# LemonATsu/DANBO-pytorch

Measured on AMD Instinct MI355X. Metric: ray-samples/sec at 512x512x64 samples, higher is better.
Workload: dtype f32 (fp16x2-split MFMA products, fp32 accumulate); 1 GPU; H36M danbo_base network, 512x512 rays x (48 coarse + 16 importance) samples, 1 pose / 1 camera per rank, cylinder near/far, exact in-volume culling; rays=262144, samples_per_ray=64, parallelism=rays-dp1

## Files before the change

### danbo-pytorch_amd/core/hip_ops.py

```python
import contextlib
import ctypes
import gc

import torch

from . import _hip
from ._hip import call as _call, ptr as _p, stream as _stream
from .utils.skeleton_utils import SMPLSkeleton

J = _hip.C.DANBO_J
VOL = _hip.C.DANBO_VOL
FEAT = _hip.C.DANBO_FEAT
RAY_FLAT_VMAX = _hip.C.DANBO_RAY_FLAT_VMAX
H_STRIDE = _hip.C.DANBO_H_STRIDE
MLP_PACKED_FLOATS = _hip.C.DANBO_MLP_PACKED_FLOATS
ASSIGN16_PACKED_BYTES = _hip.C.DANBO_ASSIGN16_PACKED_BYTES
MLP16_PACKED_BYTES = _hip.C.DANBO_MLP16_PACKED_BYTES
ANERF_ENC_FLOATS = _hip.C.DANBO_ANERF_ENC_FLOATS
LINEAR16_ENC_K = _hip.C.DANBO_LINEAR16_ENC_K
TRUNK_PACKED_BYTES = _hip.C.DANBO_TRUNK_PACKED_BYTES
TRUNK_PE_WIDTH = _hip.C.DANBO_TRUNK_PE_WIDTH
VIEW_W = 128


def _on_device(*named, f32=False, dim=None, required=False):
    for t, name in named:
        ok = not required if t is None else t.is_cuda and (not f32 or t.dtype == torch.float32) and (dim is None or t.dim() == dim)
        if not ok:
            what = ("%d-D " % dim if dim else "") + ("float32 " if f32 else "")
            raise RuntimeError(f"{name}: expected a {what}CUDA/HIP tensor -- libdanbo_hip has no CPU fallback")


def _f32(t, name):
    if t is None:
        return None
    _on_device((t, name))
    if t.dtype != torch.float32:
        t = t.float()
    return t.contiguous()


def cam_index(cam_idx):
    return None if cam_idx is None else cam_idx.reshape(-1).to(torch.int64).contiguous()


def _ptr_array(tensors):
    arr = (ctypes.c_void_p * len(tensors))()
    for i, t in enumerate(tensors):
        arr[i] = t.data_ptr()
    return arr


def pose_volumes(bones, gw, L_graph=5):
    bones = _f32(bones, "bones")
    G = bones.shape[0]
    W = gw["w1"].shape[-1]
    scratch = torch.empty(3 * G * J * W, device=bones.device, dtype=torch.float32)
    vol = torch.empty(G, J, VOL, device=bones.device, dtype=torch.float32)
    _call("danbo_pose_volumes_fwd", _p(bones), G, L_graph, W,
          _p(gw["w0"]), _p(gw["adjw0"]), _p(gw["b0"]), _p(gw["w1"]), _p(gw["adjw1"]), _p(gw["b1"]),
          _p(gw["w2"]), _p(gw["b2"]), _p(gw["w3"]), _p(gw["b3"]), _p(scratch), _p(vol), _stream())
    return vol


def near_far_cylinder(rays_o, rays_d, cyl, near0=0.0, far0=1.0, chunk=4096, near_in=None, far_in=None):
    rays_o, rays_d, cyl = _f32(rays_o, "rays_o"), _f32(rays_d, "rays_d"), _f32(cyl, "cyl")
    near_in, far_in = _f32(near_in, "near_in"), _f32(far_in, "far_in")
    R, G = rays_o.shape[0], cyl.shape[0]
    nchunk = (R + chunk - 1) // chunk
    scratch = torch.empty(nchunk * 8, device=rays_o.device, dtype=torch.float32)
    near = torch.empty(R, device=rays_o.device, dtype=torch.float32)
    far = torch.empty_like(near)
    _call("danbo_near_far_cylinder", _p(rays_o), _p(rays_d), _p(cyl), R, G, float(near0), float(far0),
          _p(near_in), _p(far_in), int(chunk), _p(scratch), _p(near), _p(far), _stream())
    return near, far


def near_far_boxes(rays_o, rays_d, skts, align, axis_scale, near, far):
    R, G = rays_o.shape[0], skts.shape[0]
    _call("danbo_near_far_boxes", _p(_f32(rays_o, "rays_o")), _p(_f32(rays_d, "rays_d")), _p(_f32(skts, "skts")),
          _p(_f32(align, "align")), _p(_f32(axis_scale, "axis_scale")), R, G, _p(near), _p(far), _stream())
    return near, far


def coarse_samples(near, far, S, t_rand=None):
    R = near.shape[0]
    z = torch.empty(R, S, device=near.device, dtype=torch.float32)
    _call("danbo_coarse_samples", _p(near), _p(far), R, S, _p(_f32(t_rand, "t_rand")), _p(z), _stream())
    return z


@contextlib.contextmanager
def capture(graph):
    gc.collect()
    was_on = gc.isenabled()
    gc.disable()
    try:
        with torch.cuda.graph(graph):
            yield
    finally:
        if was_on:
            gc.enable()


def per_pose(x, G):
    return x if x.shape[0] == G else x[::max(x.shape[0] // G, 1)].contiguous()


def dw16(layers, M, device, count=None, slices=8):
    L = (_hip.DanboDwLayer * len(layers))(*layers)
    scratch = torch.empty(_hip.lib().danbo_dw16_scratch_floats(L, len(layers), slices), device=device)
    _call("danbo_dw16", L, len(layers), M, _p(count), slices, _p(scratch), _stream())


class Geometry:

    def __init__(self, rays_o, rays_d, skts, align, axis_scale, z=None, pts=None, ray_mask=None):
        self.rays_o = _f32(rays_o, "rays_o")
        self.rays_d = _f32(rays_d, "rays_d")
        self.skts = _f32(skts, "skts")
        self.align = _f32(align, "align")
        self.axis_scale = _f32(axis_scale, "axis_scale")
        self.z = _f32(z, "z")
        self.pts = _f32(pts, "pts")
        assert (self.z is None) != (self.pts is None)
        self.R = self.rays_o.shape[0]
        self.G = self.skts.shape[0]
        self.S = self.z.shape[1] if self.z is not None else self.pts.shape[1]
        self.M = self.R * self.S
        self.device = self.rays_o.device
        self.ray_mask = ray_mask if self.z is not None else None

    def head(self):
        return (_p(self.rays_o), _p(self.rays_d), _p(self.z), _p(self.pts), self.R, self.S, self.G,
                _p(self.skts), _p(self.align), _p(self.axis_scale))


def bone_cull(geo, compact=True, cnt=None):
    bits = torch.empty(geo.M, device=geo.device, dtype=torch.int32)
    lst = None
    if compact:
        lst = torch.empty(geo.M, device=geo.device, dtype=torch.int32)
        if cnt is None:
            cnt = torch.zeros(1, device=geo.device, dtype=torch.int32)
        assert cnt.dtype == torch.int32 and cnt.numel() == 1 and cnt.is_contiguous()
    else:
        cnt = None
    rm = tuple(geo.ray_mask) if geo.ray_mask is not None else (None, None, None)
    flat = rm[3] if len(rm) > 3 else None
    _call("danbo_bone_cull", *geo.head(), _p(rm[0]), _p(rm[1]), _p(rm[2]), _p(flat), _p(bits), _p(lst), _p(cnt), _stream())
    return bits, lst, cnt


def bone_cull_rays(geo, flat, bounds=None, cnt=None, rays_per_wg=0):
    assert geo.z is not None and geo.ray_mask is not None and geo.z.is_contiguous()
    bits = torch.empty(geo.M, device=geo.device, dtype=torch.int32)
    lst = torch.empty(geo.M, device=geo.device, dtype=torch.int32)
    if cnt is None:
        cnt = torch.zeros(1, device=geo.device, dtype=torch.int32)
    assert cnt.dtype == torch.int32 and cnt.numel() == 1 and cnt.is_contiguous()
    near, far = (None, None) if bounds is None else (_f32(b, "bounds").reshape(-1) for b in bounds)
    assert near is None or (near.shape[0] == geo.R and far.shape[0] == geo.R)
    rm = tuple(geo.ray_mask)
    _call("danbo_bone_cull_rays", *_ray_list(flat), _p(rm[0]), _p(rm[1]), _p(rm[2]), _p(geo.rays_o), _p(geo.rays_d), geo.R, geo.S,
          geo.G, _p(geo.skts), _p(geo.align), _p(geo.axis_scale), _p(near), _p(far), _p(geo.z), int(rays_per_wg), _p(bits), _p(lst),
          _p(cnt), _stream())
    return bits, lst, cnt


def ray_bone_mask(rays_o, rays_d, skts, align, axis_scale, t_lo, t_hi, want_flat=False):
    rays_o, rays_d, skts = _f32(rays_o, "rays_o"), _f32(rays_d, "rays_d"), _f32(skts, "skts")
    t_lo, t_hi = _f32(t_lo, "t_lo").reshape(-1), _f32(t_hi, "t_hi").reshape(-1)
    R, G = rays_o.shape[0], skts.shape[0]
    assert t_lo.shape[0] == R and t_hi.shape[0] == R
    mask = torch.empty(R, device=rays_o.device, dtype=torch.int32)
    flat = torch.empty(R, device=rays_o.device, dtype=torch.int32) if want_flat else None
    _call("danbo_ray_bone_mask", _p(rays_o), _p(rays_d), _p(t_lo), _p(t_hi), R, G, _p(skts), _p(_f32(align, "align")),
          _p(_f32(axis_scale, "axis_scale")), _p(mask), _p(flat), _stream())
    return (mask, t_lo, t_hi, flat) if want_flat else (mask, t_lo, t_hi)


def group_rows(bits, lst, cnt):
    _call("danbo_group_rows", _p(bits), _p(lst), _p(cnt), lst.shape[0], _stream())
    return lst


def bone_gather(geo, volumes, lst=None, cnt=None, n=None):
    n = geo.M if n is None else n
    out = torch.empty(n, J, FEAT, device=geo.device, dtype=torch.float32)
    _call("danbo_bone_gather_fwd", *geo.head(), _p(volumes), _p(lst), _p(cnt), n, _p(out), _stream())
    return out


def assign_blend(part_feat, bits, aw, lst=None, cnt=None, n=None, want_confd=False):
    n = part_feat.shape[0] if n is None else n
    h = torch.empty(n, H_STRIDE, device=part_feat.device, dtype=torch.float32)
    confd = torch.empty(n, J, device=part_feat.device, dtype=torch.float32) if want_confd else None
    _call("danbo_assign_blend_fwd", _p(part_feat), _p(bits), _p(lst), _p(cnt), n,
          _p(aw["w0"]), _p(aw["adjw"]), _p(aw["b0"]), _p(aw["w1"]), _p(aw["b1"]), _p(aw["w2"]), _p(aw["b2"]),
          _p(h), _p(confd), _stream())
    return h, confd


def gather_assign_blend(geo, volumes, bits, aw, lst=None, cnt=None, n=None, want_confd=False):
    n = geo.M if n is None else n
    h = torch.empty(n, H_STRIDE, device=geo.device, dtype=torch.float32)
    confd = torch.empty(n, J, device=geo.device, dtype=torch.float32) if want_confd else None
    _call("danbo_gather_assign_blend_fwd", *geo.head(), _p(volumes), _p(bits), _p(lst), _p(cnt), n,
          _p(aw["w0"]), _p(aw["adjw"]), _p(aw["b0"]), _p(aw["w1"]), _p(aw["b1"]), _p(aw["w2"]), _p(aw["b2"]),
          _p(h), _p(confd), _stream())
    return h, confd


_ADJ_CHECKED = set()


def check_smpl_adjacency(adj):
    key = (adj.data_ptr(), adj._version)
    if key in _ADJ_CHECKED:
        return
    want = torch.eye(J)
    for i, p_ in enumerate(SMPLSkeleton.joint_trees.tolist()):
        if i != p_:
            want[i, p_] = want[p_, i] = 1.0
    if not torch.equal((adj.detach().reshape(J, J) != 0).cpu(), want != 0):
        raise NotImplementedError("the assignment net's adjacency is not the SMPL tree: the fast K2 kernel (k_assign16) has that "
                                  "tree compiled in -- use mlp_mode='fp32' (k_assign_blend reads the adjacency it is given)")
    _ADJ_CHECKED.add(key)


def assign16_pack(aw):
    packed = torch.empty(ASSIGN16_PACKED_BYTES, device=aw["w0"].device, dtype=torch.uint8)
    _call("danbo_assign16_pack", _p(aw["w0"]), _p(aw["adjw"]), _p(aw["w1"]), _p(packed), _stream())
    return packed


_TICKETS = {}


def _ticket(device):
    if torch.cuda.is_current_stream_capturing():
        return torch.zeros(1, device=device, dtype=torch.int32)
    key = (device, torch.cuda.current_stream(device).cuda_stream)
    t = _TICKETS.get(key)
    if t is None:
        t = _TICKETS[key] = torch.zeros(1, device=device, dtype=torch.int32)
    return t


def gather_assign_blend16(geo, volumes, bits, aw, packed16, lst=None, cnt=None, n=None, want_confd=False):
    n = geo.M if n is None else n
    h = torch.empty(n, H_STRIDE, device=geo.device, dtype=torch.float32)
    confd = torch.empty(n, J, device=geo.device, dtype=torch.float32) if want_confd else None
    _call("danbo_gather_assign_blend16_fwd", *geo.head(), _p(volumes), _p(bits), _p(lst), _p(cnt), n, _p(packed16),
          _p(aw["b0"]), _p(aw["b1"]), _p(aw["w2"]), _p(aw["b2"]), _p(h), _p(confd), _p(_ticket(geo.device)), _stream())
    return h, confd


def mlp_pack(pts_w, feature_w, views_w):
    dev = feature_w.device
    Cv = views_w.shape[1] - 256
    packed = torch.empty(MLP_PACKED_FLOATS, device=dev, dtype=torch.float32)
    wrt = torch.empty(max(Cv, 1), VIEW_W, device=dev, dtype=torch.float32)
    pts_w = [_f32(w, "pts_w") for w in pts_w]
    _call("danbo_mlp_pack", _ptr_array(pts_w), _p(_f32(feature_w, "feature_w")), _p(_f32(views_w, "views_w")), Cv,
          _p(packed), _p(wrt), _stream())
    return packed, wrt


def view_consts(rays_d, skts, ray_mode, normalise, L_view, framecodes, mean_code, cam_idx, wrt, views_b,
                rgb_w, rgb_b, empty_consts=None, rgb_order=0, code_table=None, ray_list=None, ray_count=None):
    rays_d = _f32(rays_d, "rays_d")
    R, G = rays_d.shape[0], skts.shape[0]
    Cf = 0 if mean_code is None else mean_code.shape[0]
    n_codes = 0 if framecodes is None else framecodes.shape[0]
    cview = torch.empty(R, VIEW_W, device=rays_d.device, dtype=torch.float32)
    raw_empty = torch.empty(R, 4, device=rays_d.device, dtype=torch.float32) if empty_consts is not None else None
    cam_idx = cam_index(cam_idx)
    _call("danbo_view_consts", _p(rays_d), _p(_f32(skts, "skts")), R, G, int(ray_mode), int(normalise), int(L_view),
          _p(framecodes), n_codes, Cf, _p(mean_code), _p(cam_idx), _p(wrt), _p(views_b), _p(rgb_w), _p(rgb_b),
          _p(empty_consts), int(rgb_order), _p(code_table), _p(ray_list), _p(ray_count), _p(cview), _p(raw_empty), _stream())
    return cview, raw_empty


def view_code_table(framecodes, mean_code, L_view, wrt, views_b):
    n_codes, Cf = framecodes.shape
    table = torch.empty(n_codes + 1, VIEW_W, device=framecodes.device, dtype=torch.float32)
    _call("danbo_view_code_table", _p(framecodes), _p(mean_code), n_codes, Cf, int(L_view), _p(wrt), _p(views_b),
          _p(table), _stream())
    return table


def pe_mlp(h, S, packed, pts_b, alpha_w, alpha_b, feature_b, cview, rgb_w, rgb_b, raw_out,
           lst=None, cnt=None, n=None, aux=False):
    n = h.shape[0] if n is None else n
    aux_out = torch.empty(n, VIEW_W + 1, device=h.device, dtype=torch.float32) if aux else None
    _call("danbo_pe_mlp_fwd", _p(h), _p(lst), _p(cnt), n, S, _p(packed), _ptr_array(pts_b), _p(alpha_w), _p(alpha_b),
          _p(feature_b), _p(cview), _p(rgb_w), _p(rgb_b), _p(raw_out), _p(aux_out), _stream())
    return aux_out


def mlp16_pack(pts_w, feature_w, feature_b, views_w, views_b, form=16):
    dev = feature_w.device
    Cv = views_w.shape[1] - 256
    packed = torch.empty(MLP16_PACKED_BYTES, device=dev, dtype=torch.uint8)
    vb = torch.empty(VIEW_W, device=dev, dtype=torch.float32)
    pts_w = [_f32(w, "pts_w") for w in pts_w]
    _call({16: "danbo_mlp16_pack", 32: "danbo_mlp32_pack"}[form], _ptr_array(pts_w), _p(_f32(feature_w, "feature_w")), _p(_f32(feature_b, "feature_b")),
          _p(_f32(views_w, "views_w")), _p(_f32(views_b, "views_b")), Cv, _p(packed), _p(vb), _stream())
    return packed, vb


def pe_mlp16(h, S, packed16, pts_b, alpha_w, alpha_b, cview, rgb_w, rgb_b, raw_out,
             lst=None, cnt=None, n=None, aux=False, form=16):
    n = h.shape[0] if n is None else n
    aux_out = torch.empty(n, VIEW_W + 1, device=h.device, dtype=torch.float32) if aux else None
    _call({16: "danbo_pe_mlp16_fwd", 32: "danbo_pe_mlp32_fwd"}[form], _p(h), _p(lst), _p(cnt), n, S, _p(packed16), _ptr_array(pts_b), _p(alpha_w),
          _p(alpha_b), _p(cview), _p(rgb_w), _p(rgb_b), _p(raw_out), _p(aux_out), _stream())
    return aux_out


def fill_raw(raw_empty, S):
    R = raw_empty.shape[0]
    raw = torch.empty(R, S, 4, device=raw_empty.device, dtype=torch.float32)
    _call("danbo_fill_raw", _p(raw_empty), R, S, _p(raw), _stream())
    return raw


RELU = ("relu", 0.0)
_ACT_TYPES = {"relu": _hip.C.DANBO_DENSITY_RELU, "softplus": _hip.C.DANBO_DENSITY_SOFTPLUS}


def density_act(fn):
    if fn is None:
        return RELU
    if isinstance(fn, tuple) and len(fn) == 2 and fn[0] in _ACT_TYPES:
        return (fn[0], float(fn[1]) if fn[0] == "softplus" else 0.0)
    kind = getattr(fn, "density_kind", None)
    if kind == "softplus":
        return ("softplus", float(fn.softplus_shift))
    if kind == "relu" or fn is torch.nn.functional.relu or fn is torch.relu or getattr(fn, "__name__", "") == "relu":
        return RELU
    raise NotImplementedError("density activation: only relu and softplus (raycasters.get_density_fn) are implemented in the "
                              "composite kernels")


def _act_args(act):
    kind, shift = density_act(act)
    return _ACT_TYPES[kind], float(shift)


def _ray_outputs(R, S, Sf, dev, flat=None, want_weights=True, merged=False):
    n = S + Sf if merged else S
    if flat is not None:
        out = dict(flat["out" if merged else "out0"])
        assert out["alpha"].shape == (R, n)
        return out
    f = lambda *shape: torch.empty(*shape, device=dev, dtype=torch.float32)
    return dict(rgb_map=f(R, 3), disp_map=f(R), acc_map=f(R), weights=f(R, n) if want_weights else None, alpha=f(R, n))


def _ray_list(flat):
    return (None, None) if flat is None else (_p(flat["ray_list"]), _p(flat["ray_count"]))


def composite(raw, z, rays_d, B=1.0, noise=None, bits=None, raw_empty=None, flat=None, act=None):
    a_type, a_shift = _act_args(act)
    assert a_type == 0 or flat is None, "rays of constants (flat=) do not exist under softplus"
    raw, z, rays_d = _f32(raw, "raw"), _f32(z, "z"), _f32(rays_d, "rays_d")
    R, S = z.shape
    out = _ray_outputs(R, S, 0, raw.device, flat)
    assert out["weights"] is not None and out["weights"].shape == (R, S)
    _call("danbo_composite_rays_fwd_act", _p(raw), _p(_f32(raw_empty, "raw_empty")), _p(bits), _p(z), _p(rays_d), R, S, float(B),
          _p(_f32(noise, "noise")), _p(out["rgb_map"]), _p(out["disp_map"]), _p(out["acc_map"]), _p(out["weights"]), _p(out["alpha"]),
          *_ray_list(flat), a_type, a_shift, _stream())
    return out


def importance_samples(z, weights, Sf, u=None, flat=None, two_net=False):
    R, S = z.shape
    dev = z.device
    zs = torch.empty(R, S + Sf, device=dev, dtype=torch.float32)
    idx = torch.empty(R, S + Sf, device=dev, dtype=torch.int32)
    zf = flat["z_fine"] if flat is not None else torch.empty(R, Sf, device=dev, dtype=torch.float32)
    assert zf.shape == (R, Sf)
    _call("danbo_importance_samples_pdf", _p(_f32(z, "z")), _p(_f32(weights, "weights")), R, S, Sf, _p(_f32(u, "u")),
          int(bool(two_net)), _p(zf), _p(zs), _p(idx), *_ray_list(flat), _stream())
    return zs, zf, idx


def flat_rays(t_lo, ray_flat, S, Sf, want_weights=False, rows_later=False, cnt=None):
    t_lo = _f32(t_lo, "t_lo").reshape(-1)
    R, dev = t_lo.shape[0], t_lo.device
    assert ray_flat.dtype == torch.int32 and ray_flat.shape[0] == R
    out0 = _ray_outputs(R, S, Sf, dev, want_weights=want_weights)
    out = _ray_outputs(R, S, Sf, dev, merged=True)
    zf = torch.empty(R, Sf, device=dev, dtype=torch.float32)
    lst = torch.empty(R, device=dev, dtype=torch.int32)
    if cnt is None:
        cnt = torch.zeros(1, device=dev, dtype=torch.int32)
    assert cnt.dtype == torch.int32 and cnt.numel() == 1
    def launch(parts):
        _call("danbo_flat_rays", _p(t_lo), _p(ray_flat), R, int(S), int(Sf), _p(out0["rgb_map"]), _p(out0["disp_map"]),
              _p(out0["acc_map"]), _p(out0["weights"]), _p(out0["alpha"]), _p(zf), _p(out["rgb_map"]), _p(out["disp_map"]),
              _p(out["acc_map"]), _p(out["weights"]), _p(out["alpha"]), _p(lst), _p(cnt), parts, _stream())
    launch(1 if rows_later else 3)
    res = dict(out0=out0, out=out, z_fine=zf, ray_list=lst, ray_count=cnt)
    if rows_later:
        res["rows"] = lambda: launch(2)
    return res


def composite_importance(raw, z, rays_d, Sf, B=1.0, noise=None, u=None, bits=None, raw_empty=None, want_weights=True,
                         flat=None, two_net=False, act=None):
    a_type, a_shift = _act_args(act)
    assert a_type == 0 or flat is None, "rays of constants (flat=) do not exist under softplus"
    raw, z, rays_d = _f32(raw, "raw"), _f32(z, "z"), _f32(rays_d, "rays_d")
    R, S = z.shape
    dev = raw.device
    out0 = _ray_outputs(R, S, Sf, dev, flat, want_weights)
    zf = flat["z_fine"] if flat is not None else torch.empty(R, Sf, device=dev, dtype=torch.float32)
    assert zf.shape == (R, Sf)
    zs = torch.empty(R, S + Sf, device=dev, dtype=torch.float32)
    idx = torch.empty(R, S + Sf, device=dev, dtype=torch.int32)
    _call("danbo_composite_importance_pdf_fwd_act", _p(raw), _p(_f32(raw_empty, "raw_empty")), _p(bits), _p(z), _p(rays_d), R, S,
          int(Sf), float(B), _p(_f32(noise, "noise")), _p(_f32(u, "u")), int(bool(two_net)), _p(out0["rgb_map"]), _p(out0["disp_map"]),
          _p(out0["acc_map"]), _p(out0["weights"]), _p(out0["alpha"]), _p(zf), _p(zs), _p(idx), *_ray_list(flat), a_type, a_shift,
          _stream())
    return out0, zs, zf, idx


def composite_merged(raw_a, raw_b, idx, z_sorted, rays_d, B=1.0, noise=None, bits_a=None, bits_b=None, raw_empty=None,
                     want_raw=False, flat=None, act=None):
    a_type, a_shift = _act_args(act)
    assert a_type == 0 or flat is None, "rays of constants (flat=) do not exist under softplus"
    raw_a, raw_b, rays_d = _f32(raw_a, "raw_a"), _f32(raw_b, "raw_b"), _f32(rays_d, "rays_d")
    R, S = raw_a.shape[:2]
    Sf = raw_b.shape[1]
    assert flat is None or not want_raw
    out = _ray_outputs(R, S, Sf, raw_a.device, flat, merged=True)
    rs = torch.empty(R, S + Sf, 4, device=raw_a.device, dtype=torch.float32) if want_raw else None
    _call("danbo_composite_merged_fwd_act", _p(raw_a), _p(raw_b), _p(_f32(raw_empty, "raw_empty")), _p(bits_a), _p(bits_b),
          _p(idx), _p(_f32(z_sorted, "z_sorted")), _p(rays_d), R, S, Sf, float(B), _p(_f32(noise, "noise")), _p(out["rgb_map"]),
          _p(out["disp_map"]), _p(out["acc_map"]), _p(out["weights"]), _p(out["alpha"]), _p(rs), *_ray_list(flat), a_type, a_shift,
          _stream())
    if want_raw:
        out["raw_sorted"] = rs
    return out


def random_draws(state, n_uniform, n_normal, normal_std=1.0):
    assert state.dtype == torch.int64 and state.numel() == 3 and state.is_cuda
    dev = state.device
    u = torch.empty(n_uniform, device=dev, dtype=torch.float32) if n_uniform else None
    nz = torch.empty(n_normal, device=dev, dtype=torch.float32) if n_normal else None
    _call("danbo_random_draws", _p(state), int(n_uniform), _p(u), int(n_normal), float(normal_std), _p(nz), _stream())
    return u, nz


def row_span(t):
    assert t.element_size() in (4, 8)
    k = t.element_size() // 4
    if t.dim() == 0:
        t = t.reshape(1)
    inner = t[0] if t.shape[0] > 0 else t
    if not (t.shape[0] > 0 and inner.is_contiguous() and t.stride(0) >= 0):
        t = t.contiguous()
        inner = t[0]
    return t, t.shape[0], inner.numel() * k, t.stride(0) * k


def gather_rows(dst, items):
    assert dst.is_contiguous() and dst.element_size() == 4 and len(items) <= _hip.MAX_ROW_SPANS
    spans = (_hip.DanboRowSpan * len(items))()
    keep = []
    for i, (t, off) in enumerate(items):
        t, rows, words, stride = row_span(t)
        assert off + rows * words <= dst.numel()
        keep.append(t)
        spans[i] = _hip.DanboRowSpan(src=t.data_ptr(), dst_word=int(off), src_row_stride_words=int(stride), rows=int(rows),
                                     row_words=int(words))
    _call("danbo_gather_rows", spans, len(items), _p(dst), _stream())
    return dst


def merge_samples(a, b, idx):
    R, S = a.shape[:2]
    Sf = b.shape[1]
    C = a[0, 0].numel()
    out = torch.empty((R, S + Sf) + tuple(a.shape[2:]), device=a.device, dtype=torch.float32)
    _call("danbo_merge_samples", _p(_f32(a, "a")), _p(_f32(b, "b")), _p(idx), R, S, Sf, C, _p(out), _stream())
    return out


PART_MODES = {"confd": 0, "entropy": 1}
_PALETTES = {}


def part_palette(device):
    device = torch.device(device)
    t = _PALETTES.get(device)
    if t is None:
        from .networks.misc import joint_colours
        t = joint_colours(device).contiguous()
        if device.type != "cuda" or not torch.cuda.is_current_stream_capturing():
            _PALETTES[device] = t
    return t


def part_colors(confd, mode, rgb, lst=None, cnt=None, n=None, bits=None, valid_only=False):
    if mode not in PART_MODES:
        raise ValueError(f"part_colors: mode must be one of {sorted(PART_MODES)}, not {mode!r}")
    _on_device((confd, "confd"), (rgb, "rgb"), (lst, "list"), (cnt, "count"), (bits, "valid_bits"))
    if confd.dtype != torch.float32 or confd.dim() != 2 or confd.shape[1] != J or not confd.is_contiguous():
        raise ValueError("part_colors: confd must be a contiguous [rows, 24] float32 tensor")
    if rgb.dtype != torch.float32 or not rgb.is_contiguous() or rgb.shape[-1] != 3:
        raise ValueError("part_colors: rgb must be a contiguous [..., 3] float32 tensor")
    if valid_only and bits is None:
        raise ValueError("part_colors: valid_only needs the in-volume words")
    n = confd.shape[0] if n is None else int(n)
    if n > confd.shape[0] or (lst is None and n > rgb.numel() // 3) or (lst is not None and n > lst.numel()):
        raise ValueError("part_colors: more rows than confd / list / rgb hold")
    pal = part_palette(confd.device) if mode == "confd" else None
    _call("danbo_part_colors_fwd", _p(confd), _p(bits), _p(lst), _p(cnt), n, PART_MODES[mode], 1 if valid_only else 0, _p(pal),
          _p(rgb), _stream())
    return rgb


def composite_colors(rgb_a, weights, rgb_b=None, idx=None, bits_a=None, bits_b=None, flat=None, out=None):
    _on_device((rgb_a, "rgb_a"), (weights, "weights"), (rgb_b, "rgb_b"), (idx, "sorted_idx"), (out, "out"))
    rgb_a, rgb_b, weights = _f32(rgb_a, "rgb_a"), _f32(rgb_b, "rgb_b"), _f32(weights, "weights")
    R, S = rgb_a.shape[:2]
    Sf = 0 if rgb_b is None else rgb_b.shape[1]
    if tuple(weights.shape) != (R, S + Sf) or (idx is None) != (rgb_b is None) or (idx is not None and tuple(idx.shape) != (R, S + Sf)):
        raise ValueError("composite_colors: weights / sorted_idx must be [R, S + Sf]; sorted_idx and rgb_b come together")
    if out is None:
        out = torch.empty(R, 3, device=rgb_a.device, dtype=torch.float32)
    assert out.dtype == torch.float32 and tuple(out.shape) == (R, 3) and out.is_contiguous()
    _call("danbo_composite_colors_fwd", _p(rgb_a), _p(rgb_b), _p(bits_a), _p(bits_b), _p(idx), _p(weights), R, S, Sf,
          *_ray_list(flat), _p(out), _stream())
    return out


def _anerf_grid(rays_o, rays_d, skts, z, pts, nrows, width, out):
    skts = _f32(skts, "skts")
    if pts is not None:
        geo = (None, None, None, _f32(pts, "pts"))
    else:
        geo = (_f32(rays_o, "rays_o"), _f32(rays_d, "rays_d"), _f32(z, "z"), None)
    grid = geo[3] if pts is not None else geo[2]
    if out is None:
        out = (torch.empty(nrows, width, device=grid.device, dtype=torch.float32),
               torch.empty(nrows, J, device=grid.device, dtype=torch.float32))
    return geo, skts, grid.shape[0], grid.shape[1], out[0][:nrows], out[1][:nrows]


def anerf_encode(rays_o, rays_d, skts, align, cutoff, tau, L, row0, nrows, z=None, pts=None, out=None):
    geo, skts, R, S, x0, w = _anerf_grid(rays_o, rays_d, skts, z, pts, nrows, (1 + 2 * L) * J + 3 * J, out)
    _call("danbo_anerf_encode_fwd", *map(_p, geo), R, S, skts.shape[0], _p(skts), _p(_f32(align, "align")),
          _p(_f32(cutoff, "cutoff")), float(tau), int(L), int(row0), int(nrows), _p(x0), _p(w), _stream())
    return x0, w


def anerf_encode_compact(rays_o, rays_d, skts, align, cutoff, tau, row0, nrows, z=None, pts=None, out=None):
    geo, skts, R, S, table, w = _anerf_grid(rays_o, rays_d, skts, z, pts, nrows, ANERF_ENC_FLOATS, out)
    _call("danbo_anerf_encode_compact", *map(_p, geo), R, S, skts.shape[0], _p(skts), _p(_f32(align, "align")),
          _p(_f32(cutoff, "cutoff")), float(tau), int(row0), int(nrows), _p(table), _p(w), _stream())
    return table, w


def anerf_view_pe(rays_d, skts, L):
    rays_d, skts = _f32(rays_d, "rays_d"), _f32(skts, "skts")
    R, G = rays_d.shape[0], skts.shape[0]
    E = torch.empty(R, (1 + 2 * L) * 3 * J, device=rays_d.device, dtype=torch.float32)
    _call("danbo_anerf_view_pe_fwd", _p(rays_d), _p(skts), R, G, int(L), _p(E), _stream())
    return E


def transform_batch(vecs, skt, rot_only=False):
    _on_device((vecs, "transform_batch pts"), (skt, "transform_batch skt"), f32=True)
    N, S = vecs.shape[:2]
    G, J = skt.shape[0], skt.shape[-3]
    if vecs.shape[-1] != 3 or skt.shape[-2:] != (4, 4) or G < 1 or N % G:
        raise ValueError(f"transform_batch: pts {tuple(vecs.shape)}, skt {tuple(skt.shape)}")
    vecs, skt = vecs.contiguous(), skt.contiguous()
    out = torch.empty(N, S, J, 3, device=vecs.device, dtype=torch.float32)
    _call("danbo_transform_batch_pts", _p(vecs), _p(skt), N, S, J, N // G, 1 if rot_only else 0, _p(out), _stream())
    return out


def optcodes(codes, idx, mode):
    _on_device((codes, "optcodes codes"), f32=True)
    _on_device((idx, "optcodes idx"))
    idx = idx.reshape(idx.shape[0], -1).to(torch.float32).contiguous()
    codes = codes.contiguous()
    out = torch.empty(idx.shape[0], codes.shape[1], device=codes.device, dtype=torch.float32)
    _call("danbo_optcodes_fwd", _p(codes), codes.shape[0], codes.shape[1], _p(idx), idx.shape[1], idx.shape[0], int(mode), _p(out), _stream())
    return out


def small_matmul(a, b, bias=None, out=None):
    _on_device((a, "small_matmul a"), (b, "small_matmul b"), f32=True, dim=2)
    M, K = a.shape
    K2, N = b.shape
    if K != K2:
        raise ValueError(f"small_matmul: {tuple(a.shape)} @ {tuple(b.shape)}")
    if out is None:
        out = torch.empty(M, N, device=a.device, dtype=torch.float32)
    if bias is not None:
        bias = _f32(bias, "bias")
    _call("danbo_small_matmul", _p(a), a.stride(0), a.stride(1), _p(b), b.stride(0), b.stride(1), _p(bias), M, N, K, _p(out), out.stride(0),
          _stream())
    return out


def anerf_view_wj(views_w, col0, L):
    views_w = _f32(views_w, "views_w")
    VW, ld = views_w.shape
    wj = torch.empty(J, 3 * (1 + 2 * L), VW, device=views_w.device, dtype=torch.float32)
    _call("danbo_anerf_view_wj_pack", _p(views_w), ld, int(col0), VW, int(L), _p(wj), _stream())
    return wj


def anerf_view_consts(rays_d, skts, L, wj, out=None):
    rays_d, skts, wj = _f32(rays_d, "rays_d"), _f32(skts, "skts"), _f32(wj, "wj")
    R, G, VW = rays_d.shape[0], skts.shape[0], wj.shape[2]
    if wj.shape[0] != J or wj.shape[1] != 3 * (1 + 2 * L):
        raise ValueError(f"wj {tuple(wj.shape)} for L = {L}")
    C = out if out is not None else torch.empty(J, R, VW, device=rays_d.device, dtype=torch.float32)
    _call("danbo_anerf_view_consts_fwd", _p(rays_d), _p(skts), R, G, int(L), _p(wj), VW, _p(C), _stream())
    return C


def anerf_view_consts_bwd(rays_d, skts, L, dC, g_views_w, col0):
    rays_d, skts, dC = _f32(rays_d, "rays_d"), _f32(skts, "skts"), _f32(dC, "dC")
    R, G, VW = rays_d.shape[0], skts.shape[0], dC.shape[2]
    g_views_w = _f32(g_views_w, "g_views_w")
    n = _hip.lib().danbo_anerf_view_consts_bwd_scratch_floats(R, int(L), VW)
    scratch = torch.empty(n, device=rays_d.device, dtype=torch.float32)
    _call("danbo_anerf_view_consts_bwd", _p(rays_d), _p(skts), R, G, int(L), _p(dC), VW, _p(g_views_w), g_views_w.shape[1], int(col0),
          _p(scratch), _stream())
    return g_views_w


def _rows(t, name):
    _on_device((t, name), f32=True)
    if t.dim() == 1:
        t = t.unsqueeze(1)
    if t.stride(1) != 1:
        t = t.contiguous()
    return t, t.stride(0)


def anerf_color(featv, w, C, table, cam_idx, ray0, nrays, S, rgb_w, rgb_b, alpha, raw_out):
    VW = featv.shape[1]
    R_total = C.shape[1]
    cam_idx = cam_index(cam_idx)
    if cam_idx is not None and not cam_idx.is_cuda:
        raise RuntimeError("cam_idx: expected a CUDA/HIP tensor")
    featv, ldf = _rows(featv, "featv")
    alpha, lda = _rows(alpha, "alpha")
    _call("danbo_anerf_color_fwd", _p(featv), ldf, _p(_f32(w, "w")), _p(_f32(C, "C")), _p(_f32(table, "table")),
          _p(cam_idx), table.shape[0] - 1, R_total, int(ray0), int(nrays), int(S), VW, _p(_f32(rgb_w, "rgb_w")),
          _p(_f32(rgb_b, "rgb_b")), _p(alpha), lda, _p(raw_out), _stream())
    return raw_out


def linear16_color(h, packed, shape, bias, w, C, table, cam_idx, ray0, S, rgb_w, rgb_b, raw_out):
    N, K1, K2 = shape
    if not isinstance(h, FragBuffer) or h.C != K1 or K2:
        raise ValueError("linear16_color: h must be the FragBuffer the layer was packed for")
    VW, M = N - 1, h.M
    cam_idx = cam_index(cam_idx)
    _call("danbo_linear16_fwd_color", _p(h.data), K1, _p(packed), _p(_f32(bias, "bias")), VW, M, _p(_f32(w, "w")), _p(_f32(C, "C")),
          _p(_f32(table, "table")), _p(cam_idx), table.shape[0] - 1, C.shape[1], int(ray0), int(S), _p(_f32(rgb_w, "rgb_w")),
          _p(_f32(rgb_b, "rgb_b")), _p(raw_out), _stream())
    return raw_out


def linear16_pack(weight, K1=None, transposed=False, frag_in=(False, False)):
    w = _f32(weight, "weight")
    N, K = (w.shape[1], w.shape[0]) if transposed else w.shape
    K1 = K if K1 is None else int(K1)
    nbytes = _hip.lib().danbo_linear16_packed_bytes(N, K1, K - K1)
    if nbytes < 0:
        raise ValueError(f"linear16: unsupported layer shape N={N}, K={K}")
    packed = torch.empty(nbytes, dtype=torch.uint8, device=w.device)
    sn, sk = (1, w.stride(0)) if transposed else (w.stride(0), 1)
    fr = (1 if frag_in[0] else 0) | (2 if frag_in[1] else 0)
    _call("danbo_linear16_pack_frag", _p(w), sn, sk, N, K1, K - K1, fr, _p(packed), _stream())
    return packed, (N, K1, K - K1)


def linear16_pack_enc(weight, L, frag_second=True):
    w = _f32(weight, "weight")
    N, K = w.shape
    K2 = K - (24 * (1 + 2 * L) + 72)
    if K2 < 0 or K2 % 32:
        raise ValueError(f"linear16_pack_enc: {K} columns do not hold the {24 * (1 + 2 * L) + 72} density inputs (+ a multiple of 32)")
    nbytes = _hip.lib().danbo_linear16_packed_bytes(N, LINEAR16_ENC_K, K2)
    if nbytes < 0:
        raise ValueError(f"linear16: unsupported layer shape N={N}, K={K}")
    packed = torch.empty(nbytes, dtype=torch.uint8, device=w.device)
    _call("danbo_linear16_pack_enc", _p(w), w.stride(0), 1, N, int(L), K2, 2 if (K2 > 0 and frag_second) else 0, _p(packed), _stream())
    return packed, (N, LINEAR16_ENC_K, K2)


def linear16_enc(table, packed, shape, L, bias=None, relu=False, x2=None, out=None, count=None):
    N, K1, K2 = shape
    M = table.shape[0]
    if K1 != LINEAR16_ENC_K or table.shape[1] != ANERF_ENC_FLOATS or not table.is_contiguous() or not isinstance(out, FragBuffer):
        raise ValueError("linear16_enc: table must be [M, 144] contiguous, out a FragBuffer, the layer packed by linear16_pack_enc")
    if (K2 > 0) != (x2 is not None) or (x2 is not None and (not isinstance(x2, FragBuffer) or x2.M != M or x2.C != K2)):
        raise ValueError("linear16_enc: x2 must be the FragBuffer the layer was packed for")
    if out.M != M or out.C != N:
        raise ValueError("linear16_enc: out shape")
    _call("danbo_linear16_fwd_enc", _p(table), int(L), _p(x2.data) if x2 is not None else None, K2, _p(packed), _p(_f32(bias, "bias")), N,
          1 if relu else 0, _p(out.data), M, _p(count), _stream())
    return out


class FragBuffer:

    def __init__(self, rows, C, device, storage=None):
        if C % 32:
            raise ValueError("FragBuffer: the width must be a multiple of 32")
        self.M, self.C = int(rows), int(C)
        n = (self.M + 127) // 128 * 128 * self.C
        if storage is not None and storage.numel() < n:
            raise ValueError("FragBuffer: storage too small")
        self.data = torch.empty(n, device=device, dtype=torch.float32) if storage is None else storage

    def rows(self):
        G = (self.M + 127) // 128 * 8
        t = self.data[:G * 16 * self.C].view(G, self.C // 32, 2, 4, 16, 4).permute(0, 4, 1, 2, 3, 5)
        return t.reshape(G * 16, self.C)[:self.M]

    @staticmethod
    def from_rows(x):
        M, C = x.shape
        fb = FragBuffer(M, C, x.device)
        G = (M + 127) // 128 * 8
        pad = torch.zeros(G * 16, C, device=x.device, dtype=torch.float32)
        pad[:M] = x
        fb.data[:G * 16 * C] = pad.view(G, 16, C // 32, 2, 4, 4).permute(0, 2, 3, 4, 1, 5).reshape(-1)
        return fb


def _aligned_rows(t, name):
    t, ld = _rows(t, name)
    K = t.shape[1]
    if ld % 4 == 0 and ld >= (K + 3) // 4 * 4 and t.data_ptr() % 16 == 0:
        return t, ld
    buf = torch.zeros(t.shape[0], (K + 3) // 4 * 4, device=t.device, dtype=torch.float32)
    buf[:, :K] = t
    return buf[:, :K], buf.stride(0)


def _linear16_out(out, M, N, device):
    if out is None:
        out = torch.empty(M, (N + 3) // 4 * 4, device=device, dtype=torch.float32)[:, :N]
    y, ldy = _rows(out, "out")
    if y.data_ptr() != out.data_ptr() or tuple(y.shape) != (M, N) or ldy % 4 or y.data_ptr() % 16:
        raise ValueError("linear16: out must be a [M, N] float32 matrix, unit column stride, rows 16-byte aligned")
    return out, y, ldy


def linear16(x1, packed, shape, bias=None, relu=False, x2=None, out=None, count=None):
    N, K1, K2 = shape
    fr = (1 if isinstance(x1, FragBuffer) else 0) | (2 if isinstance(x2, FragBuffer) else 0) | (4 if isinstance(out, FragBuffer) else 0)
    if fr:
        return _linear16_frag(x1, packed, shape, bias, relu, x2, out, count, fr)
    if x1.shape[1] != K1 or (K2 > 0) != (x2 is not None):
        raise ValueError(f"linear16: inputs do not match the packed layer ({K1} + {K2} columns)")
    x1, ld1 = _aligned_rows(x1, "x1")
    M = x1.shape[0]
    ld2 = 0
    if x2 is not None:
        if tuple(x2.shape) != (M, K2):
            raise ValueError("linear16: x2 shape")
        x2, ld2 = _aligned_rows(x2, "x2")
    out, y, ldy = _linear16_out(out, M, N, x1.device)
    _call("danbo_linear16_fwd", _p(x1), ld1, K1, _p(x2), ld2, K2, _p(packed), _p(_f32(bias, "bias")), N, 1 if relu else 0,
          _p(y), ldy, M, _p(count), _stream())
    return out


def _linear16_frag(x1, packed, shape, bias, relu, x2, out, count, fr):
    N, K1, K2 = shape
    if fr not in (1, 4, 5, 6) or (fr == 1 and N > 256):
        raise ValueError("linear16: unsupported combination of fragment-order inputs / output")
    if (K2 > 0) != (x2 is not None):
        raise ValueError(f"linear16: inputs do not match the packed layer ({K1} + {K2} columns)")

    def operand(x, K, name):
        if isinstance(x, FragBuffer):
            if x.C != K:
                raise ValueError(f"linear16: {name} has {x.C} columns, the packed layer wants {K}")
            return x.data, 0, x.M
        if x.shape[1] != K:
            raise ValueError(f"linear16: {name} has {x.shape[1]} columns, the packed layer wants {K}")
        t, ld = _aligned_rows(x, name)
        return t, ld, t.shape[0]
    a1, ld1, M = operand(x1, K1, "x1")
    a2, ld2 = None, 0
    if x2 is not None:
        a2, ld2, M2 = operand(x2, K2, "x2")
        if M2 != M:
            raise ValueError("linear16: x2 rows")
    if isinstance(out, FragBuffer):
        if out.C != N or out.M != M:
            raise ValueError("linear16: fragment-order out does not match [rows, N]")
        y, ldy = out.data, 0
    else:
        out, y, ldy = _linear16_out(out, M, N, a1.device)
    _call("danbo_linear16_fwd_frag", _p(a1), ld1, K1, _p(a2), ld2, K2, _p(packed), _p(_f32(bias, "bias")), N, 1 if relu else 0,
          _p(y), ldy, M, _p(count), fr, _stream())
    return out


def marching_cubes(sigma, iso, floor=float("-inf"), scale=1.0, offset=(0.0, 0.0, 0.0), normals=False):
    _on_device((sigma, "sigma"))
    if sigma.dtype != torch.float32 or sigma.dim() != 3:
        raise ValueError("marching_cubes: sigma must be a [nx, ny, nz] float32 grid")
    if sigma.stride(2) != 1:
        raise ValueError("marching_cubes: the innermost stride of sigma must be 1")
    nx, ny, nz = sigma.shape
    grid = (_p(sigma), nx, ny, nz, sigma.stride(0), sigma.stride(1), float(floor), float(iso))
    n_bytes = _hip.lib().danbo_mesh_workspace_bytes(nx, ny, nz)
    if n_bytes == 0:
        raise _hip.HipError(f"marching_cubes: unsupported grid {nx} x {ny} x {nz} (each dimension 2 .. 1024, fewer than 2^31 points)")
    ws = torch.empty(n_bytes, device=sigma.device, dtype=torch.uint8)
    counts = torch.empty(2, device=sigma.device, dtype=torch.int32)
    _call("danbo_mesh_count", *grid, _p(ws), _p(counts), _stream())
    V, T = counts.tolist()
    if max(V, T) >= 2 ** 31 - 1:
        raise _hip.HipError("marching_cubes: the surface has 2^31 or more vertices or triangles")
    verts = torch.empty(V, 3, device=sigma.device, dtype=torch.float32)
    faces = torch.empty(T, 3, device=sigma.device, dtype=torch.int32)
    if V > 0:
        ox, oy, oz = (float(x) for x in offset)
        _call("danbo_mesh_extract", *grid, _p(ws), float(scale), ox, oy, oz, _p(verts), V, _p(faces), T, _stream())
    if not normals:
        return verts, faces
    nrm = torch.empty(V, 3, device=sigma.device, dtype=torch.float32)
    if V > 0:
        _call("danbo_mesh_normals", *grid, _p(ws), _p(nrm), V, _stream())
    return verts, faces, nrm


_rc = _hip.header("danbo_raster.h").C
RASTER_MODES = {"color": _rc.DANBO_RASTER_COLOR, "normal": _rc.DANBO_RASTER_NORMAL, "flat": _rc.DANBO_RASTER_FLAT}


def rasterize_mesh(verts, faces, attr=None, mode="normal", views=None, half_extent=0.6, size=(512, 512), background=(1.0, 1.0, 1.0),
                   want=("rgb",)):
    _on_device((verts, "verts"), (faces, "faces"), (views, "views"), required=True)
    if mode not in RASTER_MODES:
        raise ValueError(f"rasterize_mesh: mode must be one of {sorted(RASTER_MODES)}, not {mode!r}")
    if verts.dim() != 2 or verts.shape[1] != 3 or verts.dtype != torch.float32:
        raise ValueError("rasterize_mesh: verts must be a [V, 3] float32 tensor")
    if faces.dim() != 2 or faces.shape[1] != 3 or faces.dtype != torch.int32:
        raise ValueError("rasterize_mesh: faces must be a [T, 3] int32 tensor")
    if views.dtype != torch.float32 or views.numel() == 0 or views.numel() % 12 or tuple(views.shape[1:]) not in ((3, 4), (12,)):
        raise ValueError("rasterize_mesh: views must be a [n, 3, 4] or [n, 12] float32 tensor, n >= 1")
    want = tuple(want)
    if not want or any(w not in ("rgb", "depth", "tri_id") for w in want):
        raise ValueError("rasterize_mesh: want names at least one of 'rgb', 'depth', 'tri_id'")
    V, n = verts.shape[0], views.shape[0]
    H, W = (int(x) for x in size)
    if mode == "flat":
        attr = None
    else:
        if attr is None:
            raise ValueError(f"rasterize_mesh: mode {mode!r} needs attr [V, 3]")
        _on_device((attr, "attr"))
        if attr.dtype != torch.float32 or tuple(attr.shape) != (V, 3):
            raise ValueError(f"rasterize_mesh: attr must be a [{V}, 3] float32 tensor")
        attr = attr.contiguous() if V else attr.new_zeros(1, 3)
    n_bytes = _hip.lib().danbo_raster_workspace_bytes(V, H, W)
    if n_bytes == 0:
        raise _hip.HipError(f"rasterize_mesh: unsupported size {H} x {W} (height and width 1 .. 4096)")
    dev = verts.device
    verts, faces, views = verts.contiguous(), faces.contiguous(), views.contiguous()
    ws = torch.empty(n_bytes, device=dev, dtype=torch.uint8)
    bg = torch.tensor([float(x) for x in background], device=dev, dtype=torch.float32)
    if bg.numel() != 3:
        raise ValueError("rasterize_mesh: background is three numbers")
    out = {}
    if "rgb" in want:
        out["rgb"] = torch.empty(n, H, W, 3, device=dev, dtype=torch.float32)
    if "depth" in want:
        out["depth"] = torch.empty(n, H, W, device=dev, dtype=torch.float32)
    if "tri_id" in want:
        out["tri_id"] = torch.empty(n, H, W, device=dev, dtype=torch.int32)
    _call("danbo_raster_mesh", _p(verts) if V else None, V, _p(faces) if faces.shape[0] else None, faces.shape[0], _p(attr),
          RASTER_MODES[mode], _p(views), n, float(half_extent), H, W, _p(bg), _p(ws), _p(out.get("rgb")), _p(out.get("depth")),
          _p(out.get("tri_id")), _stream())
    return out


METRICS_WIN = 11
_METRIC_WINDOWS = {}
_METRIC_WORKSPACES = {}


def metrics_window(device):
    key = str(device)
    if key not in _METRIC_WINDOWS:
        from .utils.evaluation_helpers import _gauss
        _METRIC_WINDOWS[key] = _gauss(METRICS_WIN).to(device=device, dtype=torch.float32).contiguous()
    return _METRIC_WINDOWS[key]


def image_metrics(pred, gt, mask_a=None, mask_b=None, boxes=None, want_map=False):
    _on_device((pred, "pred"), (gt, "gt"), (mask_a, "mask_a"), (mask_b, "mask_b"), (boxes, "boxes"))
    if pred.dim() != 4 or pred.shape[-1] != 3 or pred.shape != gt.shape:
        raise ValueError("image_metrics: pred and gt must be [N, H, W, 3] tensors of one shape")
    pred, gt = _f32(pred, "pred"), _f32(gt, "gt")
    pred, gt = (t.clone() if t.data_ptr() % 16 else t for t in (pred, gt))
    N, H, W = pred.shape[:3]
    dev = pred.device

    def mask(m, name):
        if m is None:
            return None
        if m.numel() != N * H * W:
            raise ValueError(f"image_metrics: {name} must be [N, H, W] (or [N, H, W, 1])")
        return _f32(m, name).reshape(N, H, W)
    mask_a, mask_b = mask(mask_a, "mask_a"), mask(mask_b, "mask_b")
    if boxes is not None:
        if boxes.dtype != torch.int32 or tuple(boxes.shape) != (N, 4):
            raise ValueError("image_metrics: boxes must be an [N, 4] int32 tensor")
        boxes = boxes.contiguous()
    n_bytes = _hip.lib().danbo_image_metrics_workspace_bytes(N, H, W)
    if n_bytes == 0:
        raise _hip.HipError(f"image_metrics: unsupported size {N} x {H} x {W} (height and width 1 .. 4096)")
    key = (str(dev), n_bytes, torch.cuda.current_stream().cuda_stream)
    if key not in _METRIC_WORKSPACES:
        _METRIC_WORKSPACES[key] = torch.empty(n_bytes, device=dev, dtype=torch.uint8)
    sums = torch.empty(N, 8, device=dev, dtype=torch.float32)
    ssim = torch.zeros(N, H, W, 3, device=dev, dtype=torch.float32) if want_map else None
    _call("danbo_image_metrics", _p(pred), _p(gt), _p(mask_a), _p(mask_b), _p(boxes), N, H, W, _p(metrics_window(dev)), METRICS_WIN,
          _p(_METRIC_WORKSPACES[key]), _p(sums), _p(ssim), _stream())
    return dict(sums=sums, ssim_map=ssim)
```

### danbo-pytorch_amd/core/render_engine.py

```python
import ctypes

import torch

from . import _hip
from . import hip_ops as ops


class RenderEngine:
    fuse_resample = False

    def _key(self):
        return tuple((k, v.data_ptr(), v._version) for k, v in sorted(self.p.items()))

    def _sampling(self, N_samples, N_importance):
        cfg = self.cfg
        return (N_samples or cfg["N_samples"], N_importance or cfg["N_importance"], cfg["density_scale"],
                ops.density_act(cfg.get("density_act")))

    @staticmethod
    def frame_result(out, out0):
        return dict(rgb_map=out["rgb_map"], disp_map=out["disp_map"], acc_map=out["acc_map"], alpha=out["alpha"],
                    T_i=out["weights"], rgb0=out0["rgb_map"], disp0=out0["disp_map"], acc0=out0["acc_map"],
                    alpha0=out0["alpha"])

    def _network_pass(self, rays_o, rays_d, skts, bones, cam_idx, z, bounds, dense, lazy, tag):
        raise NotImplementedError

    @staticmethod
    def _part_mode(part_map):
        if part_map not in (None, "confd", "entropy"):
            raise ValueError(f"part_map must be None, 'confd' or 'entropy', not {part_map!r}")
        return part_map

    def _part_exact_culled(self, act):
        return act[0] == "relu" and bool(getattr(self, "empty_density_le0", False))

    @staticmethod
    def _part_colors(ex, n_samples, mode, valid_only, dense):
        confd = ex["confd_rows"]
        R = ex["valid_bits"].numel() // n_samples
        rgb = torch.empty(R, n_samples, 3, device=confd.device, dtype=torch.float32)
        ops.part_colors(confd, mode, rgb, ex["list"], ex["count"], bits=ex["valid_bits"], valid_only=valid_only)
        return rgb, (None if dense else ex["valid_bits"])

    def render_two_net(self, fine, rays_o, rays_d, skts, bones, cyls, cam_idx=None, N_samples=None, N_importance=None,
                       chunk=4096, near_far=None, dense=False, keep=False, part_map=None, part_valid_only=False):
        S, Sf, B, act = self._sampling(N_samples, N_importance)
        self.refresh()
        fine.refresh()
        part = self._part_mode(part_map)
        if part and not (self._part_exact_culled(act) and fine._part_exact_culled(act)):
            dense = True
        lazy = not dense and not keep
        pkw = dict(want_confd=True) if part else {}
        near, far = self.near_far(rays_o, rays_d, cyls, skts, 0.0, 1.0, chunk) if near_far is None else near_far
        z = ops.coarse_samples(near, far, S)
        raw, bits, empty, ex = self._network_pass(rays_o, rays_d, skts, bones, cam_idx, z, (near, far), dense, lazy, "coarse", **pkw)
        if self.fuse_resample and S <= 64 and Sf <= 64:
            out0, z_all, z_fine, order = ops.composite_importance(raw, z, rays_d, Sf, B, bits=bits, raw_empty=empty,
                                                                  want_weights=keep or bool(part), two_net=True, act=act)
        else:
            out0 = ops.composite(raw, z, rays_d, B, bits=bits, raw_empty=empty, act=act)
            z_all, z_fine, order = ops.importance_samples(z, out0["weights"], Sf, two_net=True)
        raw_f, bits_f, empty_f, ex_f = fine._network_pass(rays_o, rays_d, skts, bones, cam_idx, z_all, (near, far), dense, lazy, "fine",
                                                          **pkw)
        out = ops.composite(raw_f, z_all, rays_d, B, bits=bits_f, raw_empty=empty_f, act=act)
        pex, pex_f = ex.pop("part", None), ex_f.pop("part", None)
        if part:
            col, cb = self._part_colors(pex, S, part, part_valid_only, dense)
            ops.composite_colors(col, out0["weights"], bits_a=cb, out=out0["rgb_map"])
            col_f, cb_f = self._part_colors(pex_f, S + Sf, part, part_valid_only, dense)
            ops.composite_colors(col_f, out["weights"], bits_a=cb_f, out=out["rgb_map"])
        ret = self.frame_result(out, out0)
        if keep and part:
            ret.update(confd_coarse=pex["confd_rows"], confd_fine=pex_f["confd_rows"], list_coarse=pex["list"],
                       list_fine=pex_f["list"])
        if keep:
            ret.update(near=near, far=far, z_coarse=z, raw_coarse=raw, weights_coarse=out0["weights"], z_fine=z_fine,
                       z_sorted=z_all, sorted_idxs=order, raw_fine=raw_f, **ex, **ex_f)
        return ret


class DanboEngine(RenderEngine):
    fuse_resample = True

    def __init__(self, cfg, params, align, buffers=None, mlp_mode="f16split"):
        self.cfg = cfg
        self.p = params
        self.align = align.float().contiguous()
        self._packed_key = None
        self.packed = self.wrt = self.empty_consts = None
        self.mean_code = None
        self.profile = None
        self.skip_flat_rays = True
        self.mlp_form = 32
        assert mlp_mode in ("f16split", "fp32")
        self.mlp_mode = mlp_mode
        self.group_rows = False
        self.cull_listed_rays = True

    def refresh(self):
        key = self._key()
        if key == self._packed_key and getattr(self, "_built_mode", None) == (self.mlp_mode, self.mlp_form):
            return
        p = self.p
        dev = p["alpha_linear.weight"].device
        q = self._equalized(p) if self.mlp_mode == "f16split" else p
        self.pts_w = [q[f"pts_linears.{i}.weight"] for i in range(8)]
        self.pts_b = [q[f"pts_linears.{i}.bias"].contiguous() for i in range(8)]
        self.packed, self.wrt = ops.mlp_pack(self.pts_w, q["feature_linear.weight"], q["views_linears.0.weight"])
        self.packed16, self.views_b16 = ops.mlp16_pack(self.pts_w, q["feature_linear.weight"],
                                                       q["feature_linear.bias"], q["views_linears.0.weight"],
                                                       q["views_linears.0.bias"], form=self.mlp_form)
        self.alpha_w = q["alpha_linear.weight"].reshape(-1).contiguous()
        self.alpha_b = q["alpha_linear.bias"].contiguous()
        self.feature_b = q["feature_linear.bias"].contiguous()
        self.views_b = q["views_linears.0.bias"].contiguous()
        self.rgb_w = q["rgb_linear.weight"].contiguous()
        self.rgb_b = q["rgb_linear.bias"].contiguous()
        self.view_scale = q.get("_view_scale", torch.ones((), device=dev))
        g = "graph_net.layers."
        self.gw = dict(
            w0=p[g + "0.lin.weight"].contiguous(), adjw0=(p[g + "0.adj_w"] * p[g + "0.adj"])[0].contiguous(),
            b0=p[g + "0.bias"].contiguous(),
            w1=p[g + "1.lin.weight"].contiguous(), adjw1=(p[g + "1.adj_w"] * p[g + "1.adj"])[0].contiguous(),
            b1=p[g + "1.bias"].contiguous(),
            w2=p[g + "2.weight"].contiguous(), b2=p[g + "2.bias"].reshape(24, -1).contiguous(),
            w3=p[g + "3.weight"].contiguous(), b3=p[g + "3.bias"].reshape(24, -1).contiguous())
        a = "prob_linears.layers."
        self.aw = dict(
            w0=p[a + "0.lin.weight"].contiguous(), adjw=(p[a + "0.adj_w"] * p[a + "0.adj"])[0].contiguous(),
            b0=p[a + "0.bias"].contiguous(), w1=p[a + "1.weight"].contiguous(),
            b1=p[a + "1.bias"].reshape(24, -1).contiguous(), w2=p[a + "2.weight"].reshape(24, -1).contiguous(),
            b2=p[a + "2.bias"].reshape(-1).contiguous())
        if self.mlp_mode == "f16split":
            ops.check_smpl_adjacency(p[a + "0.adj"])
        self.assign16 = ops.assign16_pack(self.aw)
        self.axis_scale = p["graph_net.axis_scale"].contiguous()
        if self.cfg["use_framecode"]:
            self.framecodes = p["framecodes.codes.weight"].contiguous()
            self.mean_code = self.framecodes.mean(0).contiguous()
            vb = self.views_b16 if self.mlp_mode == "f16split" else self.views_b
            self.code_table = ops.view_code_table(self.framecodes, self.mean_code, self.cfg["multires_views"],
                                                  self.wrt, vb)
        else:
            self.framecodes = self.mean_code = self.code_table = None
        h0 = torch.zeros(1, ops.H_STRIDE, device=dev)
        scratch_raw = torch.empty(1, 4, device=dev)
        self.empty_consts = self._mlp(h0, 1, None, scratch_raw, aux=True).reshape(-1).contiguous()
        self.flat_rays_ok = self._flat_rays_ok()
        self._built_mode = (self.mlp_mode, self.mlp_form)
        self._packed_key = key

    def _flat_rays_ok(self):
        cfg = self.cfg
        ec = self.empty_consts
        if self.mlp_mode != "f16split":
            self.empty_density_le0 = bool((ec[128] / float(cfg["density_scale"]) <= 0).item())
            return False
        Cpe = 3 * (1 + 2 * cfg["multires_views"])
        vmax = 1.0 if cfg["view_type"] == "relray" else ops.RAY_FLAT_VMAX
        a_max = self.wrt[:Cpe].abs().sum(0) * vmax
        if self.code_table is not None:
            a_max = a_max + self.code_table.abs().max(0).values
        elif self.wrt.shape[0] > Cpe:
            self.empty_density_le0 = bool((ec[128] / float(cfg["density_scale"]) <= 0).item())
            return False
        else:
            a_max = a_max + self.views_b16.abs()
        hidden = ec[:128].abs() + a_max
        logit = ((self.rgb_w.abs() * hidden[None, :]).sum(-1) + self.rgb_b.abs()).max()
        le0 = ec[128] / float(cfg["density_scale"]) <= 0
        self.empty_density_le0, ok = torch.stack([le0, le0 & (logit < 1e30)]).tolist()
        return ok

    @staticmethod
    def _equalized(p):
        q = dict(p)
        one = torch.ones((), device=p["alpha_linear.weight"].device)
        tiny = torch.finfo(torch.float32).tiny

        def pow2(x):
            return torch.exp2(torch.clamp(torch.round(torch.log2(torch.clamp(x, min=tiny))), -100, 100))

        def factor(w_eff, b):
            gain = torch.sqrt((w_eff.double() ** 2).sum(1).mean()).float() * 0.7
            r = pow2(1.0 / torch.clamp(gain, min=tiny))
            cap = torch.exp2(torch.clamp(torch.floor(torch.log2(1024.0 / torch.clamp(b.abs().max(), min=tiny))), -100, 100))
            return torch.minimum(r, cap)

        r_prev = one
        n_in = p["pts_linears.0.weight"].shape[1]
        for l in range(8):
            w, b = p[f"pts_linears.{l}.weight"], p[f"pts_linears.{l}.bias"]
            if l == 0:
                w_eff = w
            elif w.shape[1] > p["pts_linears.1.weight"].shape[1]:
                w_eff = torch.cat([w[:, :n_in], w[:, n_in:] / r_prev], 1)
            else:
                w_eff = w / r_prev
            r = factor(w_eff, b)
            q[f"pts_linears.{l}.weight"], q[f"pts_linears.{l}.bias"] = (w_eff * r).contiguous(), (b * r).contiguous()
            r_prev = r
        q["alpha_linear.weight"] = (p["alpha_linear.weight"] / r_prev).contiguous()
        q["feature_linear.weight"] = (p["feature_linear.weight"] / r_prev).contiguous()
        wv, bv = p["views_linears.0.weight"], p["views_linears.0.bias"]
        rv = factor(wv, bv)
        q["views_linears.0.weight"], q["views_linears.0.bias"] = (wv * rv).contiguous(), (bv * rv).contiguous()
        q["rgb_linear.weight"] = (p["rgb_linear.weight"] / rv).contiguous()
        q["_view_scale"] = rv
        return q

    def _mlp(self, h, S, cview, raw, lst=None, cnt=None, n=None, aux=False):
        if self.mlp_mode == "f16split":
            return ops.pe_mlp16(h, S, self.packed16, self.pts_b, self.alpha_w, self.alpha_b, cview,
                                self.rgb_w, self.rgb_b, raw, lst, cnt, n, aux, form=self.mlp_form)
        return ops.pe_mlp(h, S, self.packed, self.pts_b, self.alpha_w, self.alpha_b, self.feature_b, cview,
                          self.rgb_w, self.rgb_b, raw, lst, cnt, n, aux)

    def volumes(self, bones):
        self.refresh()
        return ops.pose_volumes(bones, self.gw, self.cfg["multires_graph"])

    def view_constants(self, rays_d, skts, cam_idx, ray_list=None, ray_count=None):
        self.refresh()
        cfg = self.cfg
        ray_mode = {"world": 0, "root_local": 1}[cfg["ray_tr_type"]]
        normalise = 1 if cfg["view_type"] == "relray" else 0
        return ops.view_consts(rays_d, skts, ray_mode, normalise, cfg["multires_views"], self.framecodes,
                               self.mean_code, cam_idx, self.wrt,
                               self.views_b16 if self.mlp_mode == "f16split" else self.views_b, self.rgb_w,
                               self.rgb_b, self.empty_consts, {16: 1, 32: 2}[self.mlp_form] if self.mlp_mode == "f16split" else 0,
                               self.code_table, ray_list, ray_count)

    def forward_samples(self, rays_o, rays_d, skts, bones, cam_idx=None, z=None, pts=None, dense=False,
                        want_confd=False, volumes=None, view=None, fill=True, ray_mask=None, count=None, listed=None):
        self.refresh()
        geo = ops.Geometry(rays_o, rays_d, skts, self.align, self.axis_scale, z=z, pts=pts, ray_mask=ray_mask)
        vols = self.volumes(bones) if volumes is None else volumes
        cview, raw_empty = self.view_constants(geo.rays_d, geo.skts, cam_idx) if view is None else view
        S = geo.S
        if listed is not None:
            assert not dense and pts is None
            bits, lst, cnt = ops.bone_cull_rays(geo, listed[0], listed[1], cnt=count)
        else:
            bits, lst, cnt = ops.bone_cull(geo, compact=not dense, cnt=count)
        if lst is not None and self.mlp_mode == "f16split" and self.group_rows:
            ops.group_rows(bits, lst, cnt)
        if self.mlp_mode == "f16split":
            h, confd = ops.gather_assign_blend16(geo, vols, bits, self.aw, self.assign16, lst, cnt, geo.M, want_confd)
        else:
            h, confd = ops.gather_assign_blend(geo, vols, bits, self.aw, lst, cnt, geo.M, want_confd)
        raw = ops.fill_raw(raw_empty, S) if fill or dense else torch.empty(geo.R, S, 4, device=raw_empty.device)
        if self.profile is not None:
            e0, e1 = torch.cuda.Event(enable_timing=True), torch.cuda.Event(enable_timing=True)
            e0.record()
        self._mlp(h, S, cview, raw, lst, cnt, geo.M)
        if self.profile is not None:
            e1.record()
            self.profile.setdefault("k_pe_mlp", []).append((e0, e1, cnt if cnt is not None else geo.M))
        extras = dict(valid_bits=bits, list=lst, count=cnt, confd_rows=confd, h_rows=h, volumes=vols)
        return raw, extras

    def density(self, pts, skts, bones, netchunk=1024 * 64):
        self.refresh()
        M = pts.shape[0]
        out = torch.empty(M, 1, device=pts.device, dtype=torch.float32)
        vols = self.volumes(bones)
        for a in range(0, M, netchunk):
            p = pts[a:a + netchunk].contiguous()
            n = p.shape[0]
            dummy = torch.zeros(n, 3, device=pts.device)
            raw_empty = torch.zeros(n, 4, device=pts.device)
            raw_empty[:, 3] = self.empty_consts[128]
            cview = torch.zeros(n, ops.VIEW_W, device=pts.device)
            raw, _ = self.forward_samples(dummy, dummy, skts, bones, pts=p, volumes=vols, view=(cview, raw_empty))
            out[a:a + n] = raw[..., 3:4].reshape(n, 1)
        return out

    def colors(self, pts, dirs, skts, bones, cam_idx=None, netchunk=1024 * 64):
        self.refresh()
        pts, dirs = pts.reshape(-1, 1, 3), dirs.reshape(-1, 3)
        M = pts.shape[0]
        out = torch.empty(M, 3, device=pts.device, dtype=torch.float32)
        vols = self.volumes(bones)
        cam = ops.cam_index(cam_idx)
        for a in range(0, M, netchunk):
            p, d = pts[a:a + netchunk].contiguous(), dirs[a:a + netchunk].contiguous()
            raw, _ = self.forward_samples(torch.zeros_like(d), d, skts, bones, None if cam is None else cam[a:a + netchunk], pts=p,
                                          volumes=vols)
            out[a:a + p.shape[0]] = torch.sigmoid(raw[:, 0, :3])
        return out

    def render_frame_c(self, rays_o, rays_d, skts, bones, cyls, cam_idx=None, N_samples=None, N_importance=None, chunk=4096):
        assert self.mlp_mode == "f16split" and self.mlp_form == 32
        self.refresh()
        cfg = self.cfg
        S, Sf, _, act = self._sampling(N_samples, N_importance)
        f32 = lambda t: None if t is None else t.float().contiguous()
        rays_o, rays_d, skts, bones, cyls = (f32(t) for t in (rays_o, rays_d, skts, bones, cyls))
        cam = ops.cam_index(cam_idx) if cfg["use_framecode"] else None
        R, G, dev = rays_o.shape[0], skts.shape[0], rays_o.device
        gw, aw = self.gw, self.aw
        m = _hip.DanboModel()
        for k in ("w0", "adjw0", "b0", "w1", "adjw1", "b1", "w2", "b2", "w3", "b3"):
            setattr(m, "g_" + k, gw[k].data_ptr())
        m.L_graph, m.graph_width = cfg["multires_graph"], gw["w1"].shape[-1]
        m.align, m.axis_scale, m.assign16 = self.align.data_ptr(), self.axis_scale.data_ptr(), self.assign16.data_ptr()
        m.a_b0, m.a_b1, m.a_w2, m.a_b2 = (aw[k].data_ptr() for k in ("b0", "b1", "w2", "b2"))
        m.mlp16 = self.packed16.data_ptr()
        for i in range(8):
            m.pts_b[i] = self.pts_b[i].data_ptr()
        m.alpha_w, m.alpha_b, m.rgb_w, m.rgb_b = (t.data_ptr() for t in (self.alpha_w, self.alpha_b, self.rgb_w, self.rgb_b))
        m.views_w_ray_t, m.views_b_eff, m.empty_consts = self.wrt.data_ptr(), self.views_b16.data_ptr(), self.empty_consts.data_ptr()
        if self.framecodes is not None:
            m.framecodes, m.mean_code, m.code_table = (t.data_ptr() for t in (self.framecodes, self.mean_code, self.code_table))
            m.n_codes, m.code_size = self.framecodes.shape
        m.L_view = cfg["multires_views"]
        m.ray_mode, m.normalise = {"world": 0, "root_local": 1}[cfg["ray_tr_type"]], 1 if cfg["view_type"] == "relray" else 0
        m.density_scale, m.use_volume_near_far = float(cfg["density_scale"]), int(bool(cfg["use_volume_near_far"]))
        m.flat_rays_ok = int(self.flat_rays_ok and self.skip_flat_rays)
        r = _hip.DanboRays(rays_o=rays_o.data_ptr(), rays_d=rays_d.data_ptr(), skts=skts.data_ptr(), bones=bones.data_ptr(),
                           cyls=cyls.data_ptr(), cam_idx=None if cam is None else cam.data_ptr(), near_in=None, far_in=None,
                           R=R, G=G, chunk=int(chunk))
        shapes = dict(rgb_map=(R, 3), disp_map=(R,), acc_map=(R,), alpha=(R, S + Sf), weights=(R, S + Sf), rgb0=(R, 3),
                      disp0=(R,), acc0=(R,), alpha0=(R, S))
        out = {k: torch.empty(v, device=dev, dtype=torch.float32) for k, v in shapes.items()}
        o = _hip.DanboFrameOut(**{k: v.data_ptr() for k, v in out.items()})
        nbytes = _hip.lib().danbo_render_frame_workspace(R, G, S, Sf, int(chunk), m.graph_width)
        ws = torch.empty(nbytes, device=dev, dtype=torch.uint8)
        ops._call("danbo_render_frame_act", ctypes.byref(m), ctypes.byref(r), S, Sf, ctypes.byref(o), _hip.ptr(ws), nbytes,
                  *ops._act_args(act), ops._stream())
        out["T_i"] = out.pop("weights")
        return out

    def near_far(self, rays_o, rays_d, cyls, skts, near0=0.0, far0=1.0, chunk=4096):
        self.refresh()
        near, far = ops.near_far_cylinder(rays_o, rays_d, cyls, near0, far0, chunk)
        if self.cfg["use_volume_near_far"]:
            ops.near_far_boxes(rays_o, rays_d, skts, self.align, self.axis_scale, near, far)
        return near, far

    def render(self, rays_o, rays_d, skts, bones, cyls, cam_idx=None, N_samples=None, N_importance=None,
               chunk=4096, near_far=None, dense=False, keep=False, part_map=None, part_valid_only=False):
        S, Sf, B, act = self._sampling(N_samples, N_importance)
        self.refresh()
        part = self._part_mode(part_map)
        if part and not self._part_exact_culled(act):
            dense = True
        fused = S <= 64 and Sf <= 64
        lazy = not dense and not keep
        flat_mode = (lazy and (fused or (S <= 256 and Sf <= 64)) and self.skip_flat_rays and self.flat_rays_ok
                     and act[0] == "relu")
        near, far = self.near_far(rays_o, rays_d, cyls, skts, 0.0, 1.0, chunk) if near_far is None else near_far
        listed_cull = flat_mode and self.cull_listed_rays and not part and skts.shape[0] == 1
        z = torch.empty(rays_o.shape[0], S, device=rays_o.device, dtype=torch.float32) if listed_cull else ops.coarse_samples(near, far, S)
        ray_mask = None if dense else ops.ray_bone_mask(rays_o, rays_d, skts, self.align, self.axis_scale, near, far,
                                                        want_flat=flat_mode)
        counts = torch.zeros(3, device=rays_o.device, dtype=torch.int32)
        flat = None
        vols = self.volumes(bones)
        if flat_mode:
            flat = ops.flat_rays(ray_mask[1], ray_mask[3], S, Sf, want_weights=not fused or bool(part), cnt=counts[2:3])
            view = self.view_constants(rays_d, skts, cam_idx, flat["ray_list"], flat["ray_count"])
        else:
            view = self.view_constants(rays_d, skts, cam_idx)
        if ray_mask is not None:
            ray_mask = ray_mask[:3]
        raw, ex = self.forward_samples(rays_o, rays_d, skts, bones, cam_idx, z=z, dense=dense, volumes=vols, view=view,
                                       fill=not lazy, ray_mask=ray_mask, count=counts[0:1], want_confd=bool(part),
                                       listed=(flat, (near, far)) if listed_cull else None)
        if fused:
            out0, z_all, z_fine, order = ops.composite_importance(
                raw, z, rays_d, Sf, B, bits=ex["valid_bits"] if lazy else None, raw_empty=view[1] if lazy else None,
                want_weights=keep or bool(part), flat=flat, act=act)
        else:
            out0 = ops.composite(raw, z, rays_d, B, bits=ex["valid_bits"] if lazy else None, raw_empty=view[1] if lazy else None,
                                 flat=flat, act=act)
            z_all, z_fine, order = ops.importance_samples(z, out0["weights"], Sf, flat=flat)
        raw_f, ex_f = self.forward_samples(rays_o, rays_d, skts, bones, cam_idx, z=z_fine, dense=dense,
                                           volumes=vols, view=view, fill=not lazy,
                                           ray_mask=ray_mask, count=counts[1:2], want_confd=bool(part),
                                           listed=(flat, None) if listed_cull else None)
        out = ops.composite_merged(raw, raw_f, order, z_all, rays_d, B, bits_a=ex["valid_bits"] if lazy else None,
                                   bits_b=ex_f["valid_bits"] if lazy else None, raw_empty=view[1] if lazy else None,
                                   want_raw=keep, flat=flat, act=act)
        if part:
            col, cb = self._part_colors(ex, S, part, part_valid_only, dense)
            col_f, cb_f = self._part_colors(ex_f, Sf, part, part_valid_only, dense)
            ops.composite_colors(col, out0["weights"], bits_a=cb, flat=flat, out=out0["rgb_map"])
            ops.composite_colors(col, out["weights"], col_f, order, cb, cb_f, flat=flat, out=out["rgb_map"])
        ret = self.frame_result(out, out0)
        if keep:
            ret.update(near=near, far=far, z_coarse=z, raw_coarse=raw, weights_coarse=out0["weights"], z_fine=z_fine,
                       z_sorted=z_all, sorted_idxs=order, raw_fine=raw_f, raw_sorted=out.get("raw_sorted"),
                       count_coarse=ex["count"], count_fine=ex_f["count"], valid_bits=ex["valid_bits"])
            if part:
                ret.update(confd_coarse=ex["confd_rows"], confd_fine=ex_f["confd_rows"], list_coarse=ex["list"],
                           list_fine=ex_f["list"], valid_bits_fine=ex_f["valid_bits"])
        return ret

    def _network_pass(self, rays_o, rays_d, skts, bones, cam_idx, z, bounds, dense, lazy, tag, want_confd=False):
        mask = None if dense else ops.ray_bone_mask(rays_o, rays_d, skts, self.align, self.axis_scale, *bounds)
        view = self.view_constants(rays_d, skts, cam_idx)
        raw, ex = self.forward_samples(rays_o, rays_d, skts, bones, cam_idx, z=z, dense=dense, volumes=self.volumes(bones), view=view,
                                       fill=not lazy, ray_mask=mask, want_confd=want_confd)
        bits, empty = (ex["valid_bits"], view[1]) if lazy else (None, None)
        extras = {"count_" + tag: ex["count"], "valid_bits" + ("_fine" if tag == "fine" else ""): ex["valid_bits"]}
        if want_confd:
            extras["part"] = ex
        return raw, bits, empty, extras
```

### danbo-pytorch_amd/csrc/k_frame.hip

```cpp
#include "common.hpp"
#include "../../include/danbo_cull.h"

using namespace danbo;

namespace {
struct FrameBuffers {
    float *near, *far, *cyl_scratch, *z, *vol_scratch, *volumes, *cview, *raw_empty, *h, *raw_a, *raw_b, *z_fine, *z_sorted, *weights0;
    uint32_t *bits_a, *bits_b, *ray_mask, *ray_flat;
    int32_t *list, *count, *order, *ray_list;
};

FrameBuffers carve(Carver& c, int R, int G, int S, int Sf, int chunk, int Wg) {
    FrameBuffers b;
    const size_t M = (size_t)R * S, Mf = (size_t)R * Sf;
    b.near = c.take<float>(R);
    b.far = c.take<float>(R);
    b.cyl_scratch = c.take<float>(8 * (size_t)((R + chunk - 1) / chunk));
    b.z = c.take<float>(M);
    b.vol_scratch = c.take<float>(3 * (size_t)G * 24 * Wg);
    b.volumes = c.take<float>((size_t)G * 24 * 240);
    b.cview = c.take<float>((size_t)R * 128);
    b.raw_empty = c.take<float>((size_t)R * 4);
    b.ray_mask = c.take<uint32_t>(R);
    b.ray_flat = c.take<uint32_t>(R);
    b.ray_list = c.take<int32_t>(R);
    b.bits_a = c.take<uint32_t>(M);
    b.bits_b = c.take<uint32_t>(Mf);
    b.list = c.take<int32_t>(M);
    b.count = c.take<int32_t>(4);
    b.h = c.take<float>((M > Mf ? M : Mf) * 16);
    b.raw_a = c.take<float>(M * 4);
    b.raw_b = c.take<float>(Mf * 4);
    b.z_fine = c.take<float>(Mf);
    b.z_sorted = c.take<float>(M + Mf);
    b.order = c.take<int32_t>(M + Mf);
    if (Mf > M) b.list = c.take<int32_t>(Mf);
    b.weights0 = (S <= 64 && Sf <= 64) ? nullptr : c.take<float>(M);
    return b;
}
}

extern "C" size_t danbo_render_frame_workspace(int R, int G, int S, int Sf, int chunk, int graph_width) {
    if (R < 1 || G < 1 || S < 1 || Sf < 1 || chunk < 1 || graph_width < 1) return 0;
    Carver c;
    carve(c, R, G, S, Sf, chunk, graph_width);
    return c.used + 256;
}

static int render_frame_impl(const DanboModel* m, const DanboRays* r, int S, int Sf, const DanboFrameOut* o, void* workspace,
                             size_t workspace_bytes, int act, float shift, void* stream) {
    DANBO_CHECK_ARG(m && r && o && workspace && S >= 3 && S <= 256 && Sf >= 1 && Sf <= 64);
    DANBO_CHECK_ARG(r->R >= 1 && r->G >= 1 && r->R % r->G == 0 && r->chunk >= 1);
    DANBO_CHECK_ARG(r->rays_o && r->rays_d && r->skts && r->bones && r->cyls);
    DANBO_CHECK_ARG(o->rgb_map && o->disp_map && o->acc_map && o->alpha && o->weights && o->rgb0 && o->disp0 && o->acc0 && o->alpha0);
    const int R = r->R, G = r->G;
    const bool flat_rays = m->flat_rays_ok != 0 && act == DANBO_DENSITY_RELU;
    DANBO_CHECK_ARG(workspace_bytes >= danbo_render_frame_workspace(R, G, S, Sf, r->chunk, m->graph_width));
    Carver c(workspace);
    const FrameBuffers b = carve(c, R, G, S, Sf, r->chunk, m->graph_width);
    hipStream_t st = (hipStream_t)stream;

    DANBO_TRY(danbo_near_far_cylinder(r->rays_o, r->rays_d, r->cyls, R, G, 0.f, 1.f, r->near_in, r->far_in, r->chunk, b.cyl_scratch,
                                      b.near, b.far, stream));
    if (m->use_volume_near_far)
        DANBO_TRY(danbo_near_far_boxes(r->rays_o, r->rays_d, r->skts, m->align, m->axis_scale, R, G, b.near, b.far, stream));
    const bool listed_cull = flat_rays && G == 1;
    if (!listed_cull) DANBO_TRY(danbo_coarse_samples(b.near, b.far, R, S, nullptr, b.z, stream));
    DANBO_TRY(danbo_ray_bone_mask(r->rays_o, r->rays_d, b.near, b.far, R, G, r->skts, m->align, m->axis_scale, b.ray_mask,
                                  flat_rays ? b.ray_flat : nullptr, stream));
    DANBO_TRY(danbo_pose_volumes_fwd(r->bones, G, m->L_graph, m->graph_width, m->g_w0, m->g_adjw0, m->g_b0, m->g_w1, m->g_adjw1, m->g_b1,
                                     m->g_w2, m->g_b2, m->g_w3, m->g_b3, b.vol_scratch, b.volumes, stream));
    zero_words(b.count, 4, nullptr, 0, st);
    auto view_consts = [&](const int32_t* ray_list, const int32_t* ray_count) -> int {
        return danbo_view_consts(r->rays_d, r->skts, R, G, m->ray_mode, m->normalise, m->L_view, m->framecodes, m->n_codes, m->code_size,
                                 m->mean_code, r->cam_idx, m->views_w_ray_t, m->views_b_eff, m->rgb_w, m->rgb_b, m->empty_consts, 2,
                                 m->code_table, ray_list, ray_count, b.cview, b.raw_empty, stream);
    };
    const int32_t *ray_list = nullptr, *ray_count = nullptr;
    if (flat_rays) {
        DANBO_TRY(danbo_flat_rays(b.near, b.ray_flat, R, S, Sf, o->rgb0, o->disp0, o->acc0, b.weights0, o->alpha0, b.z_fine, o->rgb_map,
                                  o->disp_map, o->acc_map, o->weights, o->alpha, b.ray_list, b.count + 3, 3, stream));
        ray_list = b.ray_list;
        ray_count = b.count + 3;
    }
    DANBO_TRY(view_consts(ray_list, ray_count));
    auto cull = [&](float* zz, int s, uint32_t* bits, int32_t* count) -> int {
        if (listed_cull) {
            const bool coarse = zz == b.z;
            return danbo_bone_cull_rays(ray_list, ray_count, b.ray_mask, b.near, b.far, r->rays_o, r->rays_d, R, s, G, r->skts, m->align,
                                        m->axis_scale, coarse ? b.near : nullptr, coarse ? b.far : nullptr, zz, 0, bits, b.list, count,
                                        stream);
        }
        DANBO_TRY(danbo_bone_cull(r->rays_o, r->rays_d, zz, nullptr, R, s, G, r->skts, m->align, m->axis_scale, b.ray_mask, b.near, b.far,
                                  nullptr, bits, b.list, count, stream));
        return 0;
    };
    auto network = [&](const float* zz, int s, uint32_t* bits, int32_t* count, float* raw) -> int {
        DANBO_TRY(danbo_gather_assign_blend16_fwd(r->rays_o, r->rays_d, zz, nullptr, R, s, G, r->skts, m->align, m->axis_scale, b.volumes,
                                                  bits, b.list, count, R * s, m->assign16, m->a_b0, m->a_b1, m->a_w2, m->a_b2, b.h,
                                                  nullptr, reinterpret_cast<uint32_t*>(b.count + 2), stream));
        return danbo_pe_mlp32_fwd(b.h, b.list, count, R * s, s, m->mlp16, m->pts_b, m->alpha_w, m->alpha_b, b.cview, m->rgb_w,
                                  m->rgb_b, raw, nullptr, stream);
    };
    DANBO_TRY(cull(b.z, S, b.bits_a, b.count));
    DANBO_TRY(network(b.z, S, b.bits_a, b.count, b.raw_a));
    if (S <= 64) {
        DANBO_TRY(danbo_composite_importance_pdf_fwd_act(b.raw_a, b.raw_empty, b.bits_a, b.z, r->rays_d, R, S, Sf, m->density_scale, nullptr,
                                                         nullptr, 0, o->rgb0, o->disp0, o->acc0, nullptr, o->alpha0, b.z_fine, b.z_sorted,
                                                         b.order, ray_list, ray_count, act, shift, stream));
    } else {
        DANBO_TRY(danbo_composite_rays_fwd_act(b.raw_a, b.raw_empty, b.bits_a, b.z, r->rays_d, R, S, m->density_scale, nullptr, o->rgb0,
                                               o->disp0, o->acc0, b.weights0, o->alpha0, ray_list, ray_count, act, shift, stream));
        DANBO_TRY(danbo_importance_samples_rays(b.z, b.weights0, R, S, Sf, nullptr, b.z_fine, b.z_sorted, b.order, ray_list, ray_count,
                                                stream));
    }
    DANBO_TRY(cull(b.z_fine, Sf, b.bits_b, b.count + 1));
    DANBO_TRY(network(b.z_fine, Sf, b.bits_b, b.count + 1, b.raw_b));
    return danbo_composite_merged_fwd_act(b.raw_a, b.raw_b, b.raw_empty, b.bits_a, b.bits_b, b.order, b.z_sorted, r->rays_d, R, S, Sf,
                                          m->density_scale, nullptr, o->rgb_map, o->disp_map, o->acc_map, o->weights, o->alpha, nullptr,
                                          ray_list, ray_count, act, shift, stream);
}

extern "C" int danbo_render_frame(const DanboModel* m, const DanboRays* r, int S, int Sf, const DanboFrameOut* o, void* workspace,
                                  size_t workspace_bytes, void* stream) {
    return render_frame_impl(m, r, S, Sf, o, workspace, workspace_bytes, DANBO_DENSITY_RELU, 0.f, stream);
}

extern "C" int danbo_render_frame_act(const DanboModel* m, const DanboRays* r, int S, int Sf, const DanboFrameOut* o, void* workspace,
                                      size_t workspace_bytes, int act, float shift, void* stream) {
    DANBO_CHECK_DENSITY_ACT(act, shift);
    return render_frame_impl(m, r, S, Sf, o, workspace, workspace_bytes, act, act == DANBO_DENSITY_SOFTPLUS ? shift : 0.f, stream);
}
```

### danbo-pytorch_amd/csrc/k_sample.hip

```cpp
#include "common.hpp"
#include "cull_math.hpp"

namespace danbo {

__global__ __launch_bounds__(256) DANBO_NO_PK_F32 void k_cylinder_pass1(const float* __restrict__ rays_o,
                                                        const float* __restrict__ rays_d,
                                                        const float* __restrict__ cyl, int R, int G,
                                                        float near0, float far0,
                                                        const float* __restrict__ near_in,
                                                        const float* __restrict__ far_in, int chunk,
                                                        double* __restrict__ acc,
                                                        float* __restrict__ near_out,
                                                        float* __restrict__ far_out) {
    const int rays_per_pose = R / G;
    for (int r0 = blockIdx.x * blockDim.x; r0 < R; r0 += gridDim.x * blockDim.x) {
        const int r = r0 + threadIdx.x;
        const bool act = r < R;
        const int rc = act ? r : R - 1;
        const int g = min(rc / rays_per_pose, G - 1);
        float o[3] = {rays_o[3 * rc], rays_o[3 * rc + 1], rays_o[3 * rc + 2]};
        float d[3] = {rays_d[3 * rc], rays_d[3 * rc + 1], rays_d[3 * rc + 2]};
        float c[3] = {cyl[5 * g], cyl[5 * g + 1], cyl[5 * g + 2]};
        float nr, fr;
        const bool hit = cylinder_bounds(o, d, c, near_in ? near_in[rc] : near0, far_in ? far_in[rc] : far0, &nr, &fr) && act;
        if (act) {
            near_out[r] = nr;
            far_out[r] = fr;
        }
        const int ck = rc / chunk;
        const int ck0 = __shfl(ck, 0, 64);
        const bool uniform = __all(ck == ck0);
        double sn = hit ? (double)nr : 0.0, sf = hit ? (double)fr : 0.0, sc = hit ? 1.0 : 0.0;
        if (uniform) {
#pragma unroll
            for (int off = 32; off > 0; off >>= 1) {
                sn += __shfl_xor(sn, off, 64);
                sf += __shfl_xor(sf, off, 64);
                sc += __shfl_xor(sc, off, 64);
            }
            if ((threadIdx.x & 63) == 0 && sc > 0.0) {
                double* a = acc + 4 * ck;
                atomicAdd(a + 0, sn);
                atomicAdd(a + 1, sf);
                atomicAdd(a + 2, sc);
            }
        } else if (hit) {
            double* a = acc + 4 * ck;
            atomicAdd(a + 0, sn);
            atomicAdd(a + 1, sf);
            atomicAdd(a + 2, 1.0);
        }
    }
}

__global__ __launch_bounds__(256) void k_cylinder_pass2(int R, float near0, float far0,
                                                        const float* __restrict__ near_in,
                                                        const float* __restrict__ far_in, int chunk,
                                                        const double* __restrict__ acc,
                                                        float* __restrict__ near_out,
                                                        float* __restrict__ far_out) {
    for (int r = blockIdx.x * blockDim.x + threadIdx.x; r < R; r += gridDim.x * blockDim.x) {
        const float nr = near_out[r];
        if (nr != nr) {
            const double* a = acc + 4 * (r / chunk);
            const double cnt = a[2];
            near_out[r] = cnt > 0.0 ? (float)(a[0] / cnt) : (near_in ? near_in[r] : near0);
            far_out[r] = cnt > 0.0 ? (float)(a[1] / cnt) : (far_in ? far_in[r] : far0);
        }
    }
}

constexpr int CYL_BLOCK = 1024, CYL_FUSED_MAX = 16 * CYL_BLOCK;
__global__ __launch_bounds__(CYL_BLOCK) DANBO_NO_PK_F32 void k_cylinder_chunk(const float* __restrict__ rays_o, const float* __restrict__ rays_d,
                                                              const float* __restrict__ cyl, int R, int G, float near0, float far0,
                                                              const float* __restrict__ near_in, const float* __restrict__ far_in,
                                                              int chunk, float* __restrict__ near_out, float* __restrict__ far_out) {
    __shared__ double s_part[CYL_BLOCK / 64][3];
    __shared__ double s_sum[3];
    const int rays_per_pose = R / G;
    const int r_begin = blockIdx.x * chunk, r_end = min(r_begin + chunk, R);
    constexpr int PER = CYL_FUSED_MAX / CYL_BLOCK;
    float nr[PER], fr[PER];
    double sn = 0.0, sf = 0.0, sc = 0.0;
#pragma unroll
    for (int k = 0; k < PER; ++k) {
        const int r = r_begin + k * CYL_BLOCK + (int)threadIdx.x;
        nr[k] = 0.f; fr[k] = 0.f;
        if (r < r_end) {
            const int g = min(r / rays_per_pose, G - 1);
            const float o[3] = {rays_o[3 * r], rays_o[3 * r + 1], rays_o[3 * r + 2]};
            const float d[3] = {rays_d[3 * r], rays_d[3 * r + 1], rays_d[3 * r + 2]};
            const float c[3] = {cyl[5 * g], cyl[5 * g + 1], cyl[5 * g + 2]};
            if (cylinder_bounds(o, d, c, near_in ? near_in[r] : near0, far_in ? far_in[r] : far0, &nr[k], &fr[k])) {
                sn += (double)nr[k]; sf += (double)fr[k]; sc += 1.0;
            }
        }
    }
#pragma unroll
    for (int off = 32; off > 0; off >>= 1) {
        sn += __shfl_xor(sn, off, 64);
        sf += __shfl_xor(sf, off, 64);
        sc += __shfl_xor(sc, off, 64);
    }
    if ((threadIdx.x & 63) == 0) { s_part[threadIdx.x >> 6][0] = sn; s_part[threadIdx.x >> 6][1] = sf; s_part[threadIdx.x >> 6][2] = sc; }
    __syncthreads();
    if (threadIdx.x < 3) {
        double t = 0.0;
        for (int w = 0; w < CYL_BLOCK / 64; ++w) t += s_part[w][threadIdx.x];
        s_sum[threadIdx.x] = t;
    }
    __syncthreads();
    const double cnt = s_sum[2];
#pragma unroll
    for (int k = 0; k < PER; ++k) {
        const int r = r_begin + k * CYL_BLOCK + (int)threadIdx.x;
        if (r < r_end) {
            float n = nr[k], f = fr[k];
            if (n != n) {
                n = cnt > 0.0 ? (float)(s_sum[0] / cnt) : (near_in ? near_in[r] : near0);
                f = cnt > 0.0 ? (float)(s_sum[1] / cnt) : (far_in ? far_in[r] : far0);
            }
            near_out[r] = n;
            far_out[r] = f;
        }
    }
}

__global__ __launch_bounds__(256) void k_box_bounds(const float* __restrict__ rays_o,
                                                    const float* __restrict__ rays_d,
                                                    const float* __restrict__ skts,
                                                    const float* __restrict__ align,
                                                    const float* __restrict__ axis_scale, int R, int G,
                                                    float* __restrict__ near_io, float* __restrict__ far_io) {
    __shared__ float s_align[J * 16];
    __shared__ float s_scale[J * 3];
    for (int i = threadIdx.x; i < J * 16; i += blockDim.x) s_align[i] = align[i];
    for (int i = threadIdx.x; i < J * 3; i += blockDim.x) s_scale[i] = fabsf(axis_scale[i]);
    __syncthreads();
    const int rays_per_pose = R / G;
    const int j = threadIdx.x & 31;
    const long slots = ((long)gridDim.x * blockDim.x) >> 5;
    for (long r0 = ((long)blockIdx.x * blockDim.x + threadIdx.x) >> 5; r0 < ((R + 1) & ~1L); r0 += slots) {
        const int r = (int)(r0 < R ? r0 : R - 1);
        const int g = min(r / rays_per_pose, G - 1);
        float lo = 100000.0f, hi = -100000.0f;
        bool ok = false;
        if (j < J && r0 < R) {
            const float o[3] = {rays_o[3 * r], rays_o[3 * r + 1], rays_o[3 * r + 2]};
            const float d[3] = {rays_d[3 * r], rays_d[3 * r + 1], rays_d[3 * r + 2]};
            float sk[12];
            const float* src = skts + ((size_t)g * J + j) * 16;
#pragma unroll
            for (int i = 0; i < 12; ++i) sk[i] = src[i];
            float l_, h_;
            ok = bone_box_steps(sk, s_align + 16 * j, s_scale + 3 * j, o, d, &l_, &h_);
            if (ok) { lo = l_; hi = h_; }
        }
        int any = ok ? 1 : 0;
#pragma unroll
        for (int off = 16; off > 0; off >>= 1) {
            lo = fminf(lo, __shfl_xor(lo, off, 64));
            hi = fmaxf(hi, __shfl_xor(hi, off, 64));
            any |= __shfl_xor(any, off, 64);
        }
        if (j == 0 && r0 < R && any) {
            near_io[r] = lo;
            far_io[r] = hi;
        }
    }
}

__global__ __launch_bounds__(256) void k_coarse_samples4(const float* __restrict__ nr, const float* __restrict__ fr,
                                                         int R, int S, const float* __restrict__ t_rand,
                                                         float4* __restrict__ z) {
    const unsigned S4 = (unsigned)S / 4u;
    const unsigned M4 = (unsigned)R * S4;
    for (unsigned q = blockIdx.x * blockDim.x + threadIdx.x; q < M4; q += gridDim.x * blockDim.x) {
        const unsigned r = q / S4;
        const int s0 = 4 * (int)(q - r * S4);
        const float n_ = nr[r], f_ = fr[r];
        const long m = 4L * q;
        float4 v;
        v.x = coarse_sample(n_, f_, s0, S, t_rand, m);
        v.y = coarse_sample(n_, f_, s0 + 1, S, t_rand, m + 1);
        v.z = coarse_sample(n_, f_, s0 + 2, S, t_rand, m + 2);
        v.w = coarse_sample(n_, f_, s0 + 3, S, t_rand, m + 3);
        z[q] = v;
    }
}

__global__ __launch_bounds__(256) void k_coarse_samples(const float* __restrict__ nr, const float* __restrict__ fr,
                                                        int R, int S, const float* __restrict__ t_rand,
                                                        float* __restrict__ z) {
    const long M = (long)R * S;
    const bool small = M <= 0x7fffffffL;
    for (long m = (long)blockIdx.x * blockDim.x + threadIdx.x; m < M; m += (long)gridDim.x * blockDim.x) {
        int r, s;
        if (small) {
            r = (int)((unsigned)m / (unsigned)S);
            s = (int)((unsigned)m - (unsigned)r * (unsigned)S);
        } else {
            r = (int)(m / S);
            s = (int)(m % S);
        }
        z[m] = coarse_sample(nr[r], fr[r], s, S, t_rand, m);
    }
}


__device__ __forceinline__ bool segment_misses_bone(const float* sk, const float* al, const float* sc ,
                                                    const float* o, const float* d, float zl, float zh) {
    float ol[3], dl[3], t[3];
    bone_local(sk, al, o, ol);
    for (int k = 0; k < 3; ++k) t[k] = sk[4 * k] * d[0] + sk[4 * k + 1] * d[1] + sk[4 * k + 2] * d[2];
    for (int k = 0; k < 3; ++k) dl[k] = al[4 * k] * t[0] + al[4 * k + 1] * t[1] + al[4 * k + 2] * t[2];
    const float pad = 1e-4f * fmaxf(fabsf(zl), fabsf(zh)) + 1e-5f;
    float tmin = zl - pad, tmax = zh + pad;
    bool miss = false;
    for (int k = 0; k < 3; ++k) {
        const float s = sc[k] * 1.001f + 1e-4f;
        if (fabsf(dl[k]) < 1e-12f) {
            miss = miss || fabsf(ol[k]) > s;
        } else {
            const float inv = 1.0f / dl[k];
            const float t1 = (-s - ol[k]) * inv, t2 = (s - ol[k]) * inv;
            tmin = fmaxf(tmin, fminf(t1, t2));
            tmax = fminf(tmax, fmaxf(t1, t2));
        }
    }
    return miss || tmin > tmax;
}

constexpr float RAY_FLAT_VMAX = DANBO_RAY_FLAT_VMAX;

template <bool POSES_IN_LDS>
__global__ __launch_bounds__(256) void k_ray_bone_mask(const float* __restrict__ rays_o, const float* __restrict__ rays_d,
                                                       const float* __restrict__ t_lo, const float* __restrict__ t_hi,
                                                       const float* __restrict__ skts, const float* __restrict__ align,
                                                       const float* __restrict__ axis_scale, int R, int G,
                                                       uint32_t* __restrict__ ray_mask, uint32_t* __restrict__ ray_flat) {
    extern __shared__ __attribute__((aligned(16))) float smem[];
    float* s_align = smem;
    float* s_scale = smem + J * 16;
    float* s_skt = smem + J * 16 + J * 4;
    const int rays_per_pose = R / G;
    const int r_a = blockIdx.x * 256, r_b = min(r_a + 255, R - 1);
    const int g0 = min(r_a / rays_per_pose, G - 1), g1 = min(r_b / rays_per_pose, G - 1);
    const int r = min(r_a + (int)threadIdx.x, R - 1);
    const float o[3] = {rays_o[3 * r], rays_o[3 * r + 1], rays_o[3 * r + 2]};
    const float d[3] = {rays_d[3 * r], rays_d[3 * r + 1], rays_d[3 * r + 2]};
    const float zl = t_lo[r], zh = t_hi[r];
    stage_bone_tables<256>(align, axis_scale, s_align, s_scale, 0.f);
    if (POSES_IN_LDS)
        for (int i = threadIdx.x; i < (g1 - g0 + 1) * J * 16; i += 256) s_skt[i] = skts[(size_t)g0 * J * 16 + i];
    __syncthreads();
    const int g = min(r / rays_per_pose, G - 1);
    uint32_t bits = 0u;
    if (POSES_IN_LDS) {
        const float* sk = s_skt + (size_t)(g - g0) * J * 16;
#pragma unroll 2
        for (int j = 0; j < J; ++j)
            bits |= segment_misses_bone(sk + 16 * j, s_align + 16 * j, s_scale + 4 * j, o, d, zl, zh) ? 0u : 1u << j;
    } else {
        for (int j = 0; j < J; ++j) {
            float sk[12];
            const float* src = skts + ((size_t)g * J + j) * 16;
#pragma unroll
            for (int i = 0; i < 12; ++i) sk[i] = src[i];
            bits |= segment_misses_bone(sk, s_align + 16 * j, s_scale + 4 * j, o, d, zl, zh) ? 0u : 1u << j;
        }
    }
    if (r_a + (int)threadIdx.x < R) {
        ray_mask[r] = bits;
        if (ray_flat != nullptr) {
            const float dn = norm3_torch(d[0], d[1], d[2]);
            const float span = mul_rn(add_rn(sub_rn(zh, zl), mul_rn(1e-3f, fmaxf(fabsf(zl), fabsf(zh)))), dn);
            const float tail = mul_rn(1e10f, dn);
            const float* m0 = POSES_IN_LDS ? s_skt + (size_t)(g - g0) * J * 16 : skts + (size_t)g * J * 16;
            float msum = 0.f;
            for (int a = 0; a < 3; ++a)
                for (int k = 0; k < 3; ++k) msum = add_rn(msum, fabsf(m0[4 * a + k]));
            const float vin = mul_rn(dn, fmaxf(1.0f, msum));
            const bool fin = zl <= zh && sub_rn(span, span) == 0.f && sub_rn(tail, tail) == 0.f && vin <= RAY_FLAT_VMAX;
            ray_flat[r] = (bits == 0u && fin) ? 1u : 0u;
        }
    }
}

constexpr int CULL_BLOCK = 256;
constexpr int CULL_SPT = 4;
constexpr int CULL_MAX_RAYS = 130;

__global__ __launch_bounds__(CULL_BLOCK) void k_bone_cull(const float* __restrict__ rays_o,
                                                          const float* __restrict__ rays_d,
                                                          const float* __restrict__ z,
                                                          const float* __restrict__ pts, int R, int S, int G,
                                                          const float* __restrict__ skts,
                                                          const float* __restrict__ align,
                                                          const float* __restrict__ axis_scale, int np_lds,
                                                          const uint32_t* __restrict__ ray_mask,
                                                          const float* __restrict__ t_lo, const float* __restrict__ t_hi,
                                                          uint32_t* __restrict__ ray_flat,
                                                          uint32_t* __restrict__ valid_bits,
                                                          int32_t* __restrict__ list, int32_t* __restrict__ count) {
    extern __shared__ __attribute__((aligned(16))) float smem[];
    float* s_align = smem;
    float* s_scale = smem + J * 16;
    float* s_skt = smem + J * 16 + J * 4;
    __shared__ float s_zlo[CULL_MAX_RAYS], s_zhi[CULL_MAX_RAYS];
    __shared__ uint32_t s_mask[CULL_MAX_RAYS];

    const long M = (long)R * S;
    const long spp = (long)(R / G) * S;
    const long base = (long)blockIdx.x * (CULL_BLOCK * CULL_SPT);
    const long last = min(base + CULL_BLOCK * CULL_SPT, M) - 1;
    const int g0 = pose_of_sample(base, spp, G), g1 = pose_of_sample(last, spp, G);

    const int lane = threadIdx.x & 63;
    const int r_first = (int)(base / S), r_last = (int)(last / S);
    const int off0 = (int)(base - (long)r_first * S);
    const int rays_per_pose = R / G;
    const float inv_S = 1.0f / (float)S;
    auto pose_of = [&](int r) { return G == 1 ? 0 : min(r / rays_per_pose, G - 1); };
    const int nrays = r_last - r_first + 1;
    const bool prefilter = pts == nullptr && ray_mask == nullptr && nrays <= CULL_MAX_RAYS;
    float zreg[CULL_SPT];
    if (pts == nullptr) {
#pragma unroll
        for (int k = 0; k < CULL_SPT; ++k) zreg[k] = z[min(base + k * CULL_BLOCK + threadIdx.x, M - 1)];
    }
    uint32_t pre[CULL_SPT];
    if (ray_mask != nullptr) {
        bool any = false;
#pragma unroll
        for (int k = 0; k < CULL_SPT; ++k) {
            pre[k] = 0u;
            if (base + k * CULL_BLOCK + threadIdx.x < M) {
                const int r = r_first + ray_of_local(off0 + k * CULL_BLOCK + threadIdx.x, S, inv_S);
                const float lo = t_lo[r], hi = t_hi[r];
                const float slack = mask_slack(lo, hi);
                const bool inside = zreg[k] >= lo - slack && zreg[k] <= hi + slack;
                pre[k] = inside ? ray_mask[r] : (1u << J) - 1u;
                if (!inside && ray_flat != nullptr) ray_flat[r] = 0u;
            }
            any = any || pre[k] != 0u;
        }
        if (!__syncthreads_or(any ? 1 : 0)) {
#pragma unroll
            for (int k = 0; k < CULL_SPT; ++k)
                if (base + k * CULL_BLOCK + threadIdx.x < M) valid_bits[base + k * CULL_BLOCK + threadIdx.x] = 0u;
            return;
        }
    }
    stage_bone_tables<CULL_BLOCK>(align, axis_scale, s_align, s_scale, 0.f);
    const int npose = g1 - g0 + 1;
    for (int i = threadIdx.x; i < npose * J * 16; i += CULL_BLOCK) s_skt[i] = skts[(size_t)g0 * J * 16 + i];
    __syncthreads();

    if (prefilter) {
        int* s_lo = reinterpret_cast<int*>(s_zlo);
        int* s_hi = reinterpret_cast<int*>(s_zhi);
        for (int i = threadIdx.x; i < nrays; i += CULL_BLOCK) { s_lo[i] = INT_MAX; s_hi[i] = INT_MIN; s_mask[i] = 0u; }
        __syncthreads();
        auto ordered = [](float f) { const int b = __builtin_bit_cast(int, f); return b >= 0 ? b : (int)(0x80000000u - (unsigned)b); };
        auto unordered = [](int o) { return __builtin_bit_cast(float, o >= 0 ? o : (int)(0x80000000u - (unsigned)o)); };
#pragma unroll
        for (int k = 0; k < CULL_SPT; ++k) {
            if (base + k * CULL_BLOCK + threadIdx.x < M) {
                const int i = ray_of_local(off0 + k * CULL_BLOCK + threadIdx.x, S, inv_S);
                const int oz = ordered(zreg[k]);
                atomicMin(&s_lo[i], oz);
                atomicMax(&s_hi[i], oz);
            }
        }
        __syncthreads();
        for (int i = threadIdx.x; i < nrays; i += CULL_BLOCK) {
            const float lo = unordered(s_lo[i]), hi = unordered(s_hi[i]);
            s_zlo[i] = lo; s_zhi[i] = hi;
        }
        __syncthreads();
        for (int q = threadIdx.x; q < nrays * J; q += CULL_BLOCK) {
            const int i = q / J, j = q % J, r = r_first + i;
            const int g = pose_of(r);
            const float* sk = s_skt + (g - g0) * J * 16 + 16 * j;
            const float* al = s_align + 16 * j;
            const float o[3] = {rays_o[3 * r], rays_o[3 * r + 1], rays_o[3 * r + 2]};
            const float d[3] = {rays_d[3 * r], rays_d[3 * r + 1], rays_d[3 * r + 2]};
            const bool miss = segment_misses_bone(sk, al, s_scale + 4 * j, o, d, s_zlo[i], s_zhi[i]);
            if (!miss) atomicOr(&s_mask[i], 1u << j);
        }
        __syncthreads();
    }
    uint32_t bits4[CULL_SPT];
#pragma unroll
    for (int pr = 0; pr < CULL_SPT / 2; ++pr) {
        const long ma = base + (2 * pr) * CULL_BLOCK + threadIdx.x;
        const long mb = ma + CULL_BLOCK;
        const long mac = min(ma, M - 1), mbc = min(mb, M - 1);
        const int lia = (int)(mac - base) + off0, lib = (int)(mbc - base) + off0;
        const int ra = r_first + ray_of_local(lia, S, inv_S), rb = r_first + ray_of_local(lib, S, inv_S);
        float pa[3], pb[3];
        if (pts != nullptr) {
            pa[0] = pts[3 * mac]; pa[1] = pts[3 * mac + 1]; pa[2] = pts[3 * mac + 2];
            pb[0] = pts[3 * mbc]; pb[1] = pts[3 * mbc + 1]; pb[2] = pts[3 * mbc + 2];
        } else {
            const float oa[3] = {rays_o[3 * ra], rays_o[3 * ra + 1], rays_o[3 * ra + 2]};
            const float da[3] = {rays_d[3 * ra], rays_d[3 * ra + 1], rays_d[3 * ra + 2]};
            const float ob[3] = {rays_o[3 * rb], rays_o[3 * rb + 1], rays_o[3 * rb + 2]};
            const float db[3] = {rays_d[3 * rb], rays_d[3 * rb + 1], rays_d[3 * rb + 2]};
            sample_point(oa, da, ma < M ? zreg[2 * pr] : z[M - 1], pa);
            sample_point(ob, db, mb < M ? zreg[2 * pr + 1] : z[M - 1], pb);
        }
        const int ga = pose_of(ra), gb = pose_of(rb);
        uint32_t ba = 0, bb = 0;
        uint32_t need = (1u << J) - 1u;
        if (ray_mask != nullptr) {
            need = wave_or(pre[2 * pr] | pre[2 * pr + 1]);
        } else if (prefilter) {
            uint32_t mine = s_mask[ra - r_first] | s_mask[rb - r_first];
            need = wave_or(mine);
        }
        if (__builtin_amdgcn_readfirstlane((int)__all(ga == gb))) {
            const v2f px = {pa[0], pb[0]}, py = {pa[1], pb[1]}, pz = {pa[2], pb[2]};
            const float* sk = s_skt + (ga - g0) * J * 16;
            in_volume_pk(sk, s_align, s_scale, need, px, py, pz, ba, bb);
        } else {
            const float* ska = s_skt + (ga - g0) * J * 16;
            const float* skb = s_skt + (gb - g0) * J * 16;
            for (int j = 0; j < J; ++j) {
                float pt[3];
                bone_local(ska + 16 * j, s_align + 16 * j, pa, pt);
                ba |= (in_volume(pt, s_scale + 4 * j) ? 1u : 0u) << j;
                bone_local(skb + 16 * j, s_align + 16 * j, pb, pt);
                bb |= (in_volume(pt, s_scale + 4 * j) ? 1u : 0u) << j;
            }
        }
        bits4[2 * pr] = ma < M ? ba : 0u;
        bits4[2 * pr + 1] = mb < M ? bb : 0u;
        if (ma < M) valid_bits[ma] = ba;
        if (mb < M) valid_bits[mb] = bb;
    }
    if (list != nullptr) {
        __shared__ int s_cnt[CULL_SPT * (CULL_BLOCK / 64)];
        __shared__ int s_base;
        const int wave = threadIdx.x >> 6;
        unsigned long long ball[CULL_SPT];
#pragma unroll
        for (int it = 0; it < CULL_SPT; ++it) {
            ball[it] = __ballot(bits4[it] != 0);
            if (lane == 0) s_cnt[it * (CULL_BLOCK / 64) + wave] = __popcll(ball[it]);
        }
        __syncthreads();
        if (threadIdx.x == 0) {
            int run = 0;
            for (int i = 0; i < CULL_SPT * (CULL_BLOCK / 64); ++i) { const int c = s_cnt[i]; s_cnt[i] = run; run += c; }
            s_base = run > 0 ? atomicAdd(count, run) : 0;
        }
        __syncthreads();
#pragma unroll
        for (int it = 0; it < CULL_SPT; ++it) {
            if (bits4[it] != 0) {
                const long m = base + it * CULL_BLOCK + threadIdx.x;
                list[s_base + s_cnt[it * (CULL_BLOCK / 64) + wave] + __popcll(ball[it] & ((1ull << lane) - 1ull))] = (int32_t)m;
            }
        }
    }
}

constexpr int GATHER_TS = 16;
constexpr int GATHER_BLOCK = GATHER_TS * J;

__global__ __launch_bounds__(GATHER_BLOCK) void k_bone_gather(const float* __restrict__ rays_o,
                                                              const float* __restrict__ rays_d,
                                                              const float* __restrict__ z,
                                                              const float* __restrict__ pts, int R, int S, int G,
                                                              const float* __restrict__ skts,
                                                              const float* __restrict__ align,
                                                              const float* __restrict__ axis_scale,
                                                              const float* __restrict__ volumes,
                                                              const int32_t* __restrict__ list,
                                                              const int32_t* __restrict__ count, int n_cap,
                                                              float* __restrict__ part_feat) {
    __shared__ __attribute__((aligned(16))) float s_vol[J * VOL];
    __shared__ __attribute__((aligned(16))) float s_out[GATHER_TS * J * FEAT];
    __shared__ __attribute__((aligned(16))) float s_skt[J * 16];
    __shared__ __attribute__((aligned(16))) float s_align[J * 16];
    __shared__ float s_scale[J * 4];

    const int n = resolve_count(count, n_cap);
    const int ntiles = (n + GATHER_TS - 1) / GATHER_TS;
    const long spp = (long)(R / G) * S;
    const int tid = threadIdx.x;
    const int sl = tid / J, j = tid % J;

    stage_bone_tables<GATHER_BLOCK>(align, axis_scale, s_align, s_scale, 1.f);
    int g_lds = -1;

    for (int tile = blockIdx.x; tile < ntiles; tile += gridDim.x) {
        const int row0 = tile * GATHER_TS;
        const int first = list ? list[row0] : row0;
        const int g_tile = pose_of_sample(first, spp, G);
        __syncthreads();
        if (g_tile != g_lds) {
            const float4* src = reinterpret_cast<const float4*>(volumes + (size_t)g_tile * J * VOL);
            float4* dst = reinterpret_cast<float4*>(s_vol);
            for (int i = tid; i < J * VOL / 4; i += GATHER_BLOCK) dst[i] = src[i];
            for (int i = tid; i < J * 16; i += GATHER_BLOCK) s_skt[i] = skts[(size_t)g_tile * J * 16 + i];
            g_lds = g_tile;
        }
        __syncthreads();
        const int row = row0 + sl;
        float* o_ = s_out + (sl * J + j) * FEAT;
        if (row < n) {
            const long m = list ? list[row] : row;
            const int g = pose_of_sample(m, spp, G);
            float p[3], pt[3], f[FEAT];
            point_of_sample(rays_o, rays_d, z, pts, m, S, p);
            if (g == g_lds) {
                bone_local(s_skt + 16 * j, s_align + 16 * j, p, pt);
                gather_bone_features(s_vol + j * VOL, pt, s_scale + 4 * j, f);
            } else {
                float sk[12];
                const float* src = skts + ((size_t)g * J + j) * 16;
#pragma unroll
                for (int i = 0; i < 12; ++i) sk[i] = src[i];
                bone_local(sk, s_align + 16 * j, p, pt);
                gather_bone_features(volumes + ((size_t)g * J + j) * VOL, pt, s_scale + 4 * j, f);
            }
#pragma unroll
            for (int k = 0; k < FEAT; ++k) o_[k] = f[k];
        } else {
#pragma unroll
            for (int k = 0; k < FEAT; ++k) o_[k] = 0.f;
        }
        __syncthreads();
        const int rows_here = min(GATHER_TS, n - row0);
        const int nvec = rows_here * (J * FEAT / 4);
        f32x4* dst = reinterpret_cast<f32x4*>(part_feat + (size_t)row0 * J * FEAT);
        const f32x4* src = reinterpret_cast<const f32x4*>(s_out);
        for (int i = tid; i < nvec; i += GATHER_BLOCK) __builtin_nontemporal_store(src[i], dst + i);
    }
}

__global__ __launch_bounds__(256) void k_fill_raw(const float4* __restrict__ raw_empty, int R, int S,
                                                  float4* __restrict__ raw) {
    const long M = (long)R * S;
    for (long m = (long)blockIdx.x * blockDim.x + threadIdx.x; m < M; m += (long)gridDim.x * blockDim.x)
        raw[m] = raw_empty[m / S];
}

__global__ __launch_bounds__(256) void k_merge_samples(const float* __restrict__ a, const float* __restrict__ b,
                                                       const int32_t* __restrict__ idx, int R, int S, int Sf, int C,
                                                       float* __restrict__ out) {
    const int St = S + Sf;
    const long N = (long)R * St;
    for (long i = (long)blockIdx.x * blockDim.x + threadIdx.x; i < N; i += (long)gridDim.x * blockDim.x) {
        const int r = (int)(i / St);
        const int src = min(max(idx[i], 0), St - 1);
        const float* s = src < S ? a + ((size_t)r * S + src) * C : b + ((size_t)r * Sf + (src - S)) * C;
        float* o = out + (size_t)i * C;
        if (C == 4) {
            *reinterpret_cast<float4*>(o) = *reinterpret_cast<const float4*>(s);
        } else {
            for (int c = 0; c < C; ++c) o[c] = s[c];
        }
    }
}

struct CompositeState {
    float carry, sr, sg, sb, sd, sa;
};

__device__ __forceinline__ int scattered_ray(long g, unsigned scatter, int R) {
    return (int)((unsigned long long)g * scatter % (unsigned)R);
}

template <int DA>
__device__ __forceinline__ float composite_chunk(CompositeState& st, const float4 rw, float zs, float gap, float dn,
                                                 float B, bool has_noise, float nz, bool act, int lane, float& al, float shift) {
    const float dist = mul_rn(gap, dn);
    float sig = div_rn(rw.w, B);
    if (has_noise) sig = add_rn(sig, nz);
    sig = density_act<DA>(sig, shift);
    al = sub_rn(1.0f, expf(-mul_rn(sig, dist)));
    if (!act) al = 0.f;
    const float t = act ? add_rn(sub_rn(1.0f, al), 1e-10f) : 1.0f;
    const float p = wave_scan_mul(t);
    float excl = __shfl_up(p, 1, 64);
    if (lane == 0) excl = 1.0f;
    const float T = mul_rn(st.carry, excl);
    st.carry = mul_rn(st.carry, __builtin_bit_cast(float, __builtin_amdgcn_readlane(__builtin_bit_cast(int, p), 63)));
    const float w = mul_rn(al, T);
    const float cr = rgb_of_logit(rw.x);
    const float cg = rgb_of_logit(rw.y);
    const float cb = rgb_of_logit(rw.z);
    st.sr += wave_total(w * cr);
    st.sg += wave_total(w * cg);
    st.sb += wave_total(w * cb);
    st.sd += wave_total(w * zs);
    st.sa += wave_total(w);
    return w;
}

__device__ __forceinline__ void composite_finish(const CompositeState& st, int r, float* __restrict__ rgb_map,
                                                 float* __restrict__ disp, float* __restrict__ acc_out) {
    rgb_map[3 * r] = st.sr;
    rgb_map[3 * r + 1] = st.sg;
    rgb_map[3 * r + 2] = st.sb;
    disp[r] = disp_of(st.sd, st.sa);
    acc_out[r] = fminf(st.sa, 1.0f);
}

__device__ __forceinline__ float ray_norm(const float* __restrict__ rays_d, int r) {
    const float dx = rays_d[3 * r], dy = rays_d[3 * r + 1], dz_ = rays_d[3 * r + 2];
    return norm3_torch(dx, dy, dz_);
}

template <int DA>
__global__ __launch_bounds__(256) void k_composite(const float4* __restrict__ raw, const float4* __restrict__ raw_empty,
                                                   const uint32_t* __restrict__ bits, const float* __restrict__ z,
                                                   const float* __restrict__ rays_d, int R, int S, float B, float shift,
                                                   const float* __restrict__ noise, float* __restrict__ rgb_map,
                                                   float* __restrict__ disp, float* __restrict__ acc_out,
                                                   float* __restrict__ weights, float* __restrict__ alpha_out,
                                                   const int32_t* __restrict__ ray_list, const int32_t* __restrict__ ray_count) {
    const int lane = threadIdx.x & 63;
    const int wave = (blockIdx.x * blockDim.x + threadIdx.x) >> 6;
    const int nwaves = (gridDim.x * blockDim.x) >> 6;
    const int n = ray_list ? min(max(*ray_count, 0), R) : R;
    for (int i = wave; i < n; i += nwaves) {
        const int r = ray_list ? min(max(ray_list[i], 0), R - 1) : i;
        const float dn = ray_norm(rays_d, r);
        const float4 re = bits ? raw_empty[r] : float4{0.f, 0.f, 0.f, 0.f};
        CompositeState st = {1.0f, 0.f, 0.f, 0.f, 0.f, 0.f};
        for (int c0 = 0; c0 < S; c0 += 64) {
            const int s = c0 + lane;
            const bool act = s < S;
            const size_t m = (size_t)r * S + (act ? s : S - 1);
            const float zs = z[m];
            const float gap = (s + 1 < S) ? sub_rn(z[m + 1], zs) : 1e10f;
            float4 rw = re;
            if (bits == nullptr || bits[m] != 0u) rw = raw[m];
            float al;
            const float w = composite_chunk<DA>(st, rw, zs, gap, dn, B, noise != nullptr, noise ? noise[m] : 0.f, act, lane, al, shift);
            if (act) {
                if (weights) weights[m] = w;
                if (alpha_out) alpha_out[m] = al;
            }
        }
        if (lane == 0) composite_finish(st, r, rgb_map, disp, acc_out);
    }
}

#define DANBO_MERGED_PARAMS                                                                                                      \
    const float4 *__restrict__ raw_a, const float4 *__restrict__ raw_b, const float4 *__restrict__ raw_empty,                    \
        const uint32_t *__restrict__ bits_a, const uint32_t *__restrict__ bits_b, const int32_t *__restrict__ sorted_idx,        \
        const float *__restrict__ z, const float *__restrict__ rays_d, int R, int S, int Sf, float B,                            \
        const float *__restrict__ noise, float *__restrict__ rgb_map, float *__restrict__ disp, float *__restrict__ acc_out,     \
        float *__restrict__ weights, float *__restrict__ alpha_out, float4 *__restrict__ raw_sorted,                             \
        const int32_t *__restrict__ ray_list, const int32_t *__restrict__ ray_count, unsigned scatter
__global__ __launch_bounds__(256) __attribute__((amdgpu_waves_per_eu(8, 8))) void k_composite_merged(DANBO_MERGED_PARAMS) {
    constexpr int DA = DENSITY_RELU;
    const float shift = 0.f;
#include "composite_merged_body.inc"
}
__global__ __launch_bounds__(256) __attribute__((amdgpu_waves_per_eu(8, 8))) void k_composite_merged_softplus(DANBO_MERGED_PARAMS,
                                                                                                              float shift) {
    constexpr int DA = DENSITY_SOFTPLUS;
#include "composite_merged_body.inc"
}
#undef DANBO_MERGED_PARAMS

template <bool TWO>
__global__ __launch_bounds__(64) void k_importance(const float* __restrict__ z, const float* __restrict__ weights,
                                                   int R, int S, int Sf, const float* __restrict__ u,
                                                   float* __restrict__ z_fine, float* __restrict__ z_sorted,
                                                   int32_t* __restrict__ sorted_idx) {
    for (int r = blockIdx.x * blockDim.x + threadIdx.x; r < R; r += gridDim.x * blockDim.x) {
        float* cdf = reinterpret_cast<float*>(sorted_idx + (size_t)r * (S + Sf));
        const float* zr = z + (size_t)r * S;
        float* zf = z_fine + (size_t)r * Sf;
        float* zs = z_sorted + (size_t)r * (S + Sf);
        int32_t* si = sorted_idx + (size_t)r * (S + Sf);
        importance_ray<TWO>(zr, weights + (size_t)r * S, S, Sf, u ? u + (size_t)r * Sf : nullptr, cdf, zf, zs, si);
        bool ascending = true;
        for (int i = 0; i + 1 < S; ++i) ascending = ascending && zr[i + 1] >= zr[i];
        if (u != nullptr || !ascending) {
            for (int i = 0; i < S; ++i) {
                int rank = 0;
                for (int k = 0; k < Sf; ++k) rank += zf[k] < zr[i];
                for (int q = 0; q < S; ++q) rank += sorts_before(zr[q], q, zr[i], i);
                zs[rank] = zr[i];
                si[rank] = i;
            }
            for (int k = 0; k < Sf; ++k) {
                int rank = 0;
                for (int i = 0; i < S; ++i) rank += zr[i] <= zf[k];
                for (int q = 0; q < Sf; ++q) rank += sorts_before(zf[q], q, zf[k], k);
                zs[rank] = zf[k];
                si[rank] = S + k;
            }
        }
    }
}

template <bool DET, bool TWO = false>
__device__ __forceinline__ void importance_wave(float zi, float wi, int r, int S, int Sf, const float* __restrict__ u,
                                                int lane, float* __restrict__ z_fine, float* __restrict__ z_sorted,
                                                int32_t* __restrict__ sorted_idx) {
    const int nb = S - 2, ncdf = S - 1;
    const bool cact = lane < S;
    const float w1 = __shfl_down(wi, 1, 64), w2 = __shfl_down(wi, 2, 64);
    const float z1 = __shfl_down(zi, 1, 64);
    float dw = 0.f;
    if (lane < nb) dw = pdf_weight<TWO>(wi, w1, w2);
    const float sum = wave_total(dw);
    const float inc = wave_scan_add(div_rn(dw, sum));
    float cdf = __shfl_up(inc, 1, 64);
    if (lane == 0) cdf = 0.f;
    const float bin = mul_rn(0.5f, add_rn(z1, zi));
    const bool fact = lane < Sf;
    const float uk = DET ? linspace01(fact ? lane : 0, Sf) : (fact ? u[(size_t)r * Sf + lane] : 0.f);
    int lo = 0, hi = ncdf;
#pragma unroll
    for (int it = 0; it < 7; ++it) {
        const int mid = (lo + hi) >> 1;
        const float cm = __shfl(cdf, mid < ncdf ? mid : ncdf - 1, 64);
        if (lo < hi) {
            if (cm > uk) hi = mid; else lo = mid + 1;
        }
    }
    const int below = cdf_below(lo), above = cdf_above(lo, ncdf);
    const float c0 = __shfl(cdf, below, 64), c1 = __shfl(cdf, above, 64);
    const float b0 = __shfl(bin, below, 64), b1 = __shfl(bin, above, 64);
    float denom = sub_rn(c1, c0);
    if (denom < 1e-5f) denom = 1.0f;
    const float t = div_rn(sub_rn(uk, c0), denom);
    const float zf = fact ? add_rn(b0, mul_rn(t, sub_rn(b1, b0))) : INFINITY;
    if (fact) z_fine[(size_t)r * Sf + lane] = zf;
    int rank_c = lane, rank_f = lane;
    const bool ascending = __all(!(lane < S - 1) || z1 >= zi);
    if (DET && ascending) {
        int l0 = 0, h0 = Sf, l1 = 0, h1 = S;
#pragma unroll
        for (int it = 0; it < 7; ++it) {
            const int m0 = (l0 + h0) >> 1, m1 = (l1 + h1) >> 1;
            const float f = __shfl(zf, m0 < 63 ? m0 : 63, 64);
            const float c = __shfl(zi, m1 < 63 ? m1 : 63, 64);
            if (l0 < h0) { if (f < zi) l0 = m0 + 1; else h0 = m0; }
            if (l1 < h1) { if (c <= zf) l1 = m1 + 1; else h1 = m1; }
        }
        rank_c += l0;
        rank_f += l1;
    } else {
        rank_c = 0;
        rank_f = 0;
        for (int k = 0; k < Sf; ++k) {
            const float zk = __shfl(zf, k, 64);
            rank_c += zk < zi;
            rank_f += sorts_before(zk, k, zf, lane);
        }
        if (ascending) rank_c += lane;
        for (int i = 0; i < S; ++i) {
            const float zc = __shfl(zi, i, 64);
            rank_f += zc <= zf;
            if (!ascending) rank_c += sorts_before(zc, i, zi, lane);
        }
    }
    const size_t o = (size_t)r * (S + Sf);
    if (cact) { z_sorted[o + rank_c] = zi; sorted_idx[o + rank_c] = lane; }
    if (fact) { z_sorted[o + rank_f] = zf; sorted_idx[o + rank_f] = S + lane; }
}

template <bool DET, bool TWO = false>
__global__ __launch_bounds__(256) void k_importance_wave(const float* __restrict__ z, const float* __restrict__ weights,
                                                         int R, int S, int Sf, const float* __restrict__ u,
                                                         float* __restrict__ z_fine, float* __restrict__ z_sorted,
                                                         int32_t* __restrict__ sorted_idx) {
    const int lane = threadIdx.x & 63;
    const int wave = (blockIdx.x * blockDim.x + threadIdx.x) >> 6;
    const int nwaves = (gridDim.x * blockDim.x) >> 6;
    for (int r = wave; r < R; r += nwaves) {
        const bool cact = lane < S;
        const float zi = cact ? z[(size_t)r * S + lane] : INFINITY;
        const float wi = cact ? weights[(size_t)r * S + lane] : 0.f;
        importance_wave<DET, TWO>(zi, wi, r, S, Sf, u, lane, z_fine, z_sorted, sorted_idx);
    }
}

constexpr int IMPB_MAX_S = 256;
template <bool DET, bool TWO = false>
__global__ __launch_bounds__(256) void k_importance_wave_long(const float* __restrict__ z, const float* __restrict__ weights,
                                                              int R, int S, int Sf, const float* __restrict__ u,
                                                              float* __restrict__ z_fine, float* __restrict__ z_sorted,
                                                              int32_t* __restrict__ sorted_idx, unsigned scatter,
                                                              const int32_t* __restrict__ ray_list,
                                                              const int32_t* __restrict__ ray_count) {
    __shared__ float s_all[4][3 * IMPB_MAX_S + 64];
    const int lane = threadIdx.x & 63, wv = threadIdx.x >> 6;
    float* s_z = s_all[wv];
    float* s_w = s_z + IMPB_MAX_S;
    float* s_b = s_w + IMPB_MAX_S;
    float* s_f = s_b + IMPB_MAX_S;
    const int wave = (blockIdx.x * blockDim.x + threadIdx.x) >> 6;
    const int nwaves = (gridDim.x * blockDim.x) >> 6;
    const int nb = S - 2, ncdf = S - 1;
    const int nchunk = (S + 63) >> 6;
    const int n = ray_list ? min(max(*ray_count, 0), R) : R;
    for (int i = wave; i < n; i += nwaves) {
        const int r = ray_list ? min(max(ray_list[i], 0), R - 1) : scattered_ray(i, scatter, R);
        const size_t o = (size_t)r * S;
        for (int c = 0; c < nchunk; ++c) {
            const int s0 = 64 * c + lane;
            if (s0 < S) { s_z[s0] = z[o + s0]; s_w[s0] = weights[o + s0]; }
        }
        float sum = 0.f;
        float dwv[IMPB_MAX_S / 64];
        bool asc = true;
#pragma unroll
        for (int c = 0; c < IMPB_MAX_S / 64; ++c) {
            const int s0 = 64 * c + lane;
            float dw = 0.f;
            if (c < nchunk && s0 < nb) {
                const float w0 = s_w[s0], w1 = s_w[s0 + 1], w2 = s_w[s0 + 2];
                dw = pdf_weight<TWO>(w0, w1, w2);
            }
            dwv[c] = dw;
            if (c < nchunk) {
                sum = add_rn(sum, wave_total(dw));
                if (s0 + 1 < S) {
                    const float z0 = s_z[s0], z1 = s_z[s0 + 1];
                    s_b[s0] = mul_rn(0.5f, add_rn(z1, z0));
                    asc = asc && z1 >= z0;
                }
            }
        }
        const bool ascending = __all(asc);
        float carry = 0.f;
#pragma unroll
        for (int c = 0; c < IMPB_MAX_S / 64; ++c) {
            if (c < nchunk) {
                const int s0 = 64 * c + lane;
                const float inc = add_rn(carry, wave_scan_add(div_rn(dwv[c], sum)));
                if (s0 < nb) s_w[s0 + 1] = inc;
                carry = __builtin_bit_cast(float, __builtin_amdgcn_readlane(__builtin_bit_cast(int, inc), 63));
            }
        }
        if (lane == 0) s_w[0] = 0.f;
        const bool fact = lane < Sf;
        const float uk = DET ? linspace01(fact ? lane : 0, Sf) : (fact ? u[(size_t)r * Sf + lane] : 0.f);
        int lo = 0, hi = ncdf;
#pragma unroll
        for (int it = 0; it < 9; ++it) {
            const int mid = (lo + hi) >> 1;
            const float cm = s_w[mid < ncdf ? mid : ncdf - 1];
            if (lo < hi) {
                if (cm > uk) hi = mid; else lo = mid + 1;
            }
        }
        const int below = cdf_below(lo), above = cdf_above(lo, ncdf);
        const float c0 = s_w[below], c1 = s_w[above];
        const float b0 = s_b[below], b1 = s_b[above];
        float denom = sub_rn(c1, c0);
        if (denom < 1e-5f) denom = 1.0f;
        const float t = div_rn(sub_rn(uk, c0), denom);
        const float zf = fact ? add_rn(b0, mul_rn(t, sub_rn(b1, b0))) : INFINITY;
        if (fact) z_fine[(size_t)r * Sf + lane] = zf;
        s_f[lane] = zf;
        const size_t oo = (size_t)r * (S + Sf);
        if (DET && ascending) {
            int l1 = 0, h1 = S;
#pragma unroll
            for (int it = 0; it < 9; ++it) {
                const int m1 = (l1 + h1) >> 1;
                const float cz = s_z[m1 < S ? m1 : S - 1];
                if (l1 < h1) { if (cz <= zf) l1 = m1 + 1; else h1 = m1; }
            }
            if (fact) { z_sorted[oo + lane + l1] = zf; sorted_idx[oo + lane + l1] = S + lane; }
            for (int c = 0; c < nchunk; ++c) {
                const int s0 = 64 * c + lane;
                const float zi = s_z[s0 < S ? s0 : S - 1];
                int l0 = 0, h0 = Sf;
#pragma unroll
                for (int it = 0; it < 7; ++it) {
                    const int m0 = (l0 + h0) >> 1;
                    const float fz = s_f[m0 < 63 ? m0 : 63];
                    if (l0 < h0) { if (fz < zi) l0 = m0 + 1; else h0 = m0; }
                }
                if (s0 < S) { z_sorted[oo + s0 + l0] = zi; sorted_idx[oo + s0 + l0] = s0; }
            }
        } else {
            int rank_f = 0;
            for (int k = 0; k < Sf; ++k) {
                const float zk = s_f[k];
                rank_f += (zk < zf) || (zk == zf && k < lane);
            }
            for (int q = 0; q < S; ++q) rank_f += s_z[q] <= zf;
            if (fact) { z_sorted[oo + rank_f] = zf; sorted_idx[oo + rank_f] = S + lane; }
            for (int c = 0; c < nchunk; ++c) {
                const int s0 = 64 * c + lane;
                const float zi = s_z[s0 < S ? s0 : S - 1];
                int rank_c = 0;
                for (int k = 0; k < Sf; ++k) rank_c += s_f[k] < zi;
                if (ascending) rank_c += s0;
                else
                    for (int q = 0; q < S; ++q) { const float zq = s_z[q]; rank_c += (zq < zi) || (zq == zi && q < s0); }
                if (s0 < S) { z_sorted[oo + rank_c] = zi; sorted_idx[oo + rank_c] = s0; }
            }
        }
    }
}

template <bool DET, bool TWO = false, int DA = DENSITY_RELU>
__global__ __launch_bounds__(256) __attribute__((amdgpu_waves_per_eu(8, 8))) void k_composite_importance(const float4* __restrict__ raw,
                                                              const float4* __restrict__ raw_empty,
                                                              const uint32_t* __restrict__ bits,
                                                              const float* __restrict__ z, const float* __restrict__ rays_d,
                                                              int R, int S, int Sf, float B, const float* __restrict__ noise,
                                                              const float* __restrict__ u, float* __restrict__ rgb_map,
                                                              float* __restrict__ disp, float* __restrict__ acc_out,
                                                              float* __restrict__ weights, float* __restrict__ alpha_out,
                                                              float* __restrict__ z_fine, float* __restrict__ z_sorted,
                                                              int32_t* __restrict__ sorted_idx,
                                                              const int32_t* __restrict__ ray_list,
                                                              const int32_t* __restrict__ ray_count, unsigned scatter, float shift) {
    const int lane = threadIdx.x & 63;
    const int wave = (blockIdx.x * blockDim.x + threadIdx.x) >> 6;
    const int nwaves = (gridDim.x * blockDim.x) >> 6;
    const bool act = lane < S;
    struct RayIn { uint32_t word; float zs, z1, dn; float4 re; };
    auto fetch = [&](int r) {
        RayIn in;
        const size_t m = (size_t)r * S + (act ? lane : S - 1);
        in.word = bits ? bits[m] : 1u;
        in.zs = z[m];
        in.z1 = (lane + 1 < S) ? z[m + 1] : 0.f;
        in.dn = ray_norm(rays_d, r);
        in.re = bits ? raw_empty[r] : float4{0.f, 0.f, 0.f, 0.f};
        return in;
    };
    const int n = ray_list ? min(max(*ray_count, 0), R) : R;
    auto ray_at = [&](int i) { return i < n ? (ray_list ? min(max(ray_list[i], 0), R - 1) : scattered_ray(i, scatter, R)) : -1; };
    int r = ray_at(wave), r_nxt = ray_at(wave + nwaves);
    if (r < 0) return;
    RayIn cur = fetch(r);
    for (int i = wave; i < n; i += nwaves) {
        CompositeState st = {1.0f, 0.f, 0.f, 0.f, 0.f, 0.f};
        const size_t m = (size_t)r * S + (act ? lane : S - 1);
        float4 rw = cur.re;
        if (cur.word != 0u) rw = raw[m];
        const int r_n = r_nxt >= 0 ? r_nxt : r;
        const RayIn nxt = fetch(r_n);
        const int r_nn = ray_at(i + 2 * nwaves);
        const float zs = cur.zs;
        const float gap = (lane + 1 < S) ? sub_rn(cur.z1, zs) : 1e10f;
        float al, w;
        bool flat = false;
        if constexpr (DA == DENSITY_RELU) {
            const float dist = mul_rn(gap, cur.dn);
            const float rgb_sum = add_rn(add_rn(cur.re.x, cur.re.y), cur.re.z);
            flat = bits != nullptr && noise == nullptr && !(div_rn(cur.re.w, B) > 0.f) && sub_rn(rgb_sum, rgb_sum) == 0.f &&
                   __all(cur.word == 0u && sub_rn(dist, dist) == 0.f);
        }
        if (flat) {
            al = 0.f;
            w = 0.f;
            st.sr = st.sg = st.sb = st.sd = st.sa = 0.f;
        } else {
            w = composite_chunk<DA>(st, rw, zs, gap, cur.dn, B, noise != nullptr, noise ? noise[m] : 0.f, act, lane, al, shift);
        }
        if (act) {
            if (weights) weights[m] = w;
            if (alpha_out) alpha_out[m] = al;
        }
        if (lane == 0) composite_finish(st, r, rgb_map, disp, acc_out);
        importance_wave<DET, TWO>(act ? zs : INFINITY, act ? w : 0.f, r, S, Sf, u, lane, z_fine, z_sorted, sorted_idx);
        cur = nxt; r = r_n; r_nxt = r_nn;
    }
}

constexpr int FLAT_BLOCK = 256;
__global__ __launch_bounds__(FLAT_BLOCK) void k_flat_rays(const float* __restrict__ t_lo,
                                                          const uint32_t* __restrict__ ray_flat, int R, int S, int Sf,
                                                          float* __restrict__ rgb0, float* __restrict__ disp0, float* __restrict__ acc0,
                                                          float* __restrict__ weights0, float* __restrict__ alpha0,
                                                          float* __restrict__ z_fine, float* __restrict__ rgb_map,
                                                          float* __restrict__ disp, float* __restrict__ acc_out,
                                                          float* __restrict__ weights, float* __restrict__ alpha_out,
                                                          int32_t* __restrict__ ray_list, int32_t* __restrict__ ray_count,
                                                          int parts) {
    __shared__ int s_cnt[FLAT_BLOCK / 64];
    __shared__ int s_base;
    const int lane = threadIdx.x & 63, wave = threadIdx.x >> 6;
    const int St = S + Sf;
    const int r = blockIdx.x * FLAT_BLOCK + threadIdx.x;
    const bool flat = r < R && ray_flat[r] != 0u;
    const float lo = flat ? t_lo[r] : 0.f;
    if (flat && (parts & 1)) {
        rgb0[3 * r] = 0.f; rgb0[3 * r + 1] = 0.f; rgb0[3 * r + 2] = 0.f;
        disp0[r] = 0.f;
        acc0[r] = 0.f;
        rgb_map[3 * r] = 0.f; rgb_map[3 * r + 1] = 0.f; rgb_map[3 * r + 2] = 0.f;
        disp[r] = 0.f;
        acc_out[r] = 0.f;
    }
    unsigned long long rows = (parts & 2) ? __ballot(flat) : 0ull;
    const unsigned long long listed = __ballot(r < R && !flat);
    while (rows != 0ull) {
        const int b = (int)__builtin_ctzll(rows);
        rows &= rows - 1ull;
        const size_t rr = (size_t)(blockIdx.x * FLAT_BLOCK + wave * 64 + b);
        for (int c = lane; c < S; c += 64) {
            if (weights0) weights0[rr * S + c] = 0.f;
            if (alpha0) alpha0[rr * S + c] = 0.f;
        }
        const float lo_b = __builtin_bit_cast(float, __builtin_amdgcn_readlane(__builtin_bit_cast(int, lo), b));
        for (int c = lane; c < Sf; c += 64) z_fine[rr * Sf + c] = lo_b;
        for (int c = lane; c < St; c += 64) {
            if (weights) weights[rr * St + c] = 0.f;
            if (alpha_out) alpha_out[rr * St + c] = 0.f;
        }
    }
    if (!(parts & 1)) return;
    if (lane == 0) s_cnt[wave] = (int)__popcll(listed);
    __syncthreads();
    if (threadIdx.x == 0) {
        int run = 0;
        for (int w = 0; w < FLAT_BLOCK / 64; ++w) { const int c = s_cnt[w]; s_cnt[w] = run; run += c; }
        s_base = run > 0 ? atomicAdd(ray_count, run) : 0;
    }
    __syncthreads();
    if (r < R && !flat) ray_list[s_base + s_cnt[wave] + (int)__popcll(listed & ((1ull << lane) - 1ull))] = r;
}

}

using namespace danbo;

static unsigned ray_scatter(int R) {
    static const unsigned primes[] = {40507u, 40519u, 40529u, 40531u, 40543u, 40559u};
    for (unsigned p : primes) {
        unsigned a = p, b = (unsigned)R;
        while (b != 0u) { const unsigned t = a % b; a = b; b = t; }
        if (a == 1u) return p;
    }
    return 1u;
}

extern "C" int danbo_near_far_cylinder(const float* rays_o, const float* rays_d, const float* cyl, int R, int G,
                                        float near0, float far0, const float* near_in, const float* far_in, int chunk,
                                        float* scratch, float* near_out, float* far_out, void* stream) {
    DANBO_CHECK_ARG(chunk > 0 && scratch != nullptr && poses_ok(R, G));
    hipStream_t st = (hipStream_t)stream;
    const int nchunk = ceil_div(R, chunk);
    if (chunk <= CYL_FUSED_MAX) {
        hipLaunchKernelGGL(k_cylinder_chunk, dim3(nchunk), dim3(CYL_BLOCK), 0, st, rays_o, rays_d, cyl, R, G, near0, far0, near_in,
                           far_in, chunk, near_out, far_out);
        DANBO_LAUNCH_RET();
    }
    zero_words(scratch, 8L * nchunk, nullptr, 0, st);
    const int grid = stream_grid(R, 256);
    hipLaunchKernelGGL(k_cylinder_pass1, dim3(grid), dim3(256), 0, st, rays_o, rays_d, cyl, R, G, near0, far0, near_in,
                       far_in, chunk, reinterpret_cast<double*>(scratch), near_out, far_out);
    hipLaunchKernelGGL(k_cylinder_pass2, dim3(grid), dim3(256), 0, st, R, near0, far0, near_in, far_in, chunk,
                       reinterpret_cast<const double*>(scratch), near_out, far_out);
    DANBO_LAUNCH_RET();
}

extern "C" int danbo_near_far_boxes(const float* rays_o, const float* rays_d, const float* skts, const float* align,
                                     const float* axis_scale, int R, int G, float* near_io, float* far_io,
                                     void* stream) {
    DANBO_CHECK_ARG(poses_ok(R, G));
    hipLaunchKernelGGL(k_box_bounds, dim3(stream_grid((long)R * 32, 256)), dim3(256), 0, (hipStream_t)stream, rays_o, rays_d, skts,
                       align, axis_scale, R, G, near_io, far_io);
    DANBO_LAUNCH_RET();
}

extern "C" int danbo_coarse_samples(const float* near, const float* far, int R, int S, const float* t_rand, float* z,
                                     void* stream) {
    DANBO_CHECK_ARG(R > 0 && S > 0);
    if (S % 4 == 0 && (long)R * S <= 0x7fffffffL && ((uintptr_t)z & 15) == 0)
        hipLaunchKernelGGL(k_coarse_samples4, dim3(stream_grid((long)R * S / 4, 256)), dim3(256), 0, (hipStream_t)stream, near, far, R, S,
                           t_rand, reinterpret_cast<float4*>(z));
    else
        hipLaunchKernelGGL(k_coarse_samples, dim3(stream_grid((long)R * S, 256)), dim3(256), 0, (hipStream_t)stream, near,
                           far, R, S, t_rand, z);
    DANBO_LAUNCH_RET();
}

extern "C" int danbo_bone_cull(const float* rays_o, const float* rays_d, const float* z, const float* pts, int R, int S, int G,
                                const float* skts, const float* align, const float* axis_scale, const uint32_t* ray_mask,
                                const float* t_lo, const float* t_hi, uint32_t* ray_flat, uint32_t* valid_bits, int32_t* list,
                                int32_t* count, void* stream) {
    DANBO_CHECK_ARG(shape_ok(R, S, G));
    DANBO_CHECK_ARG((list == nullptr) == (count == nullptr));
    DANBO_CHECK_ARG(one_of(z, pts));
    DANBO_CHECK_ARG(ray_mask == nullptr || (z != nullptr && t_lo != nullptr && t_hi != nullptr));
    DANBO_CHECK_ARG(ray_flat == nullptr || ray_mask != nullptr);
    const long M = (long)R * S;
    const long spp = (long)(R / G) * S;
    const int per_block = CULL_BLOCK * CULL_SPT;
    long np = per_block / spp + 2;
    if (np > G) np = G;
    const size_t lds = sizeof(float) * (J * 16 + J * 4 + np * J * 16);
    DANBO_CHECK_ARG(lds <= 64 * 1024);
    const int grid = ceil_div(M, per_block);
    hipLaunchKernelGGL(k_bone_cull, dim3(grid), dim3(CULL_BLOCK), lds, (hipStream_t)stream, rays_o, rays_d, z, pts, R, S,
                       G, skts, align, axis_scale, (int)np, ray_mask, t_lo, t_hi, ray_flat, valid_bits, list, count);
    DANBO_LAUNCH_RET();
}

extern "C" int danbo_ray_bone_mask(const float* rays_o, const float* rays_d, const float* t_lo, const float* t_hi, int R, int G,
                                    const float* skts, const float* align, const float* axis_scale, uint32_t* ray_mask,
                                    uint32_t* ray_flat, void* stream) {
    DANBO_CHECK_ARG(rays_o && rays_d && t_lo && t_hi && skts && align && axis_scale && ray_mask && poses_ok(R, G));
    const long np = 256 / (R / G) + 2 < G ? 256 / (R / G) + 2 : G;
    const bool in_lds = np <= 8;
    const size_t lds = sizeof(float) * (J * 16 + J * 4 + (in_lds ? np * J * 16 : 0));
    if (in_lds)
        hipLaunchKernelGGL(k_ray_bone_mask<true>, dim3(ceil_div(R, 256)), dim3(256), lds, (hipStream_t)stream, rays_o, rays_d, t_lo, t_hi,
                           skts, align, axis_scale, R, G, ray_mask, ray_flat);
    else
        hipLaunchKernelGGL(k_ray_bone_mask<false>, dim3(ceil_div(R, 256)), dim3(256), lds, (hipStream_t)stream, rays_o, rays_d, t_lo,
                           t_hi, skts, align, axis_scale, R, G, ray_mask, ray_flat);
    DANBO_LAUNCH_RET();
}

extern "C" int danbo_bone_gather_fwd(const float* rays_o, const float* rays_d, const float* z, const float* pts, int R, int S, int G,
                                      const float* skts, const float* align, const float* axis_scale,
                                      const float* volumes, const int32_t* list, const int32_t* count, int n,
                                      float* part_feat, void* stream) {
    DANBO_CHECK_ARG(n >= 0 && shape_ok(R, S, G) && one_of(z, pts));
    if (n == 0) return 0;
    const int ntiles = ceil_div(n, GATHER_TS);
    const int grid = ntiles < num_cu() * 3 ? ntiles : num_cu() * 3;
    hipLaunchKernelGGL(k_bone_gather, dim3(grid), dim3(GATHER_BLOCK), 0, (hipStream_t)stream, rays_o, rays_d, z, pts, R, S,
                       G, skts, align, axis_scale, volumes, list, count, n, part_feat);
    DANBO_LAUNCH_RET();
}

extern "C" int danbo_fill_raw(const float* raw_empty, int R, int S, float* raw, void* stream) {
    DANBO_CHECK_ARG(R > 0 && S > 0);
    hipLaunchKernelGGL(k_fill_raw, dim3(stream_grid((long)R * S, 256)), dim3(256), 0, (hipStream_t)stream,
                       reinterpret_cast<const float4*>(raw_empty), R, S, reinterpret_cast<float4*>(raw));
    DANBO_LAUNCH_RET();
}

extern "C" int danbo_merge_samples(const float* a, const float* b, const int32_t* sorted_idx, int R, int S, int Sf,
                                    int C, float* out, void* stream) {
    DANBO_CHECK_ARG(R > 0 && S > 0 && Sf >= 0 && C > 0);
    hipLaunchKernelGGL(k_merge_samples, dim3(stream_grid((long)R * (S + Sf), 256)), dim3(256), 0, (hipStream_t)stream, a,
                       b, sorted_idx, R, S, Sf, C, out);
    DANBO_LAUNCH_RET();
}

struct CompositeArgs {
    const float *raw, *raw_empty;
    const uint32_t* bits;
    const float *z, *rays_d;
    int R, S;
    float B;
    const float* noise;
    float *rgb_map, *disp, *acc, *weights, *alpha;
    const int32_t *ray_list, *ray_count;
};
template <int DA>
static int composite_launch(const CompositeArgs& a, float shift, void* stream) {
    static const int per_launch = resident_grid(k_composite<DA>, 1L << 40, 256);
    const int grid = (int)std::min<long>(ceil_div((long)a.R * 64, 256), per_launch);
    hipLaunchKernelGGL(k_composite<DA>, dim3(grid), dim3(256), 0, (hipStream_t)stream, reinterpret_cast<const float4*>(a.raw),
                       reinterpret_cast<const float4*>(a.raw_empty), a.bits, a.z, a.rays_d, a.R, a.S, a.B, shift, a.noise, a.rgb_map, a.disp,
                       a.acc, a.weights, a.alpha, a.ray_list, a.ray_count);
    DANBO_LAUNCH_RET();
}
extern "C" int danbo_composite_fwd(const float* raw, const float* z, const float* rays_d, int R, int S, float B,
                                    const float* noise, float* rgb_map, float* disp, float* acc, float* weights,
                                    float* alpha, void* stream) {
    return danbo_composite_rays_fwd(raw, nullptr, nullptr, z, rays_d, R, S, B, noise, rgb_map, disp, acc, weights, alpha, nullptr, nullptr, stream);
}
extern "C" int danbo_composite_rays_fwd(const float* raw, const float* raw_empty, const uint32_t* valid_bits, const float* z,
                                         const float* rays_d, int R, int S, float B, const float* noise, float* rgb_map,
                                         float* disp, float* acc, float* weights, float* alpha, const int32_t* ray_list,
                                         const int32_t* ray_count, void* stream) {
    return danbo_composite_rays_fwd_act(raw, raw_empty, valid_bits, z, rays_d, R, S, B, noise, rgb_map, disp, acc, weights, alpha, ray_list,
                                        ray_count, DENSITY_RELU, 0.f, stream);
}
extern "C" int danbo_composite_rays_fwd_act(const float* raw, const float* raw_empty, const uint32_t* valid_bits, const float* z,
                                             const float* rays_d, int R, int S, float B, const float* noise, float* rgb_map,
                                             float* disp, float* acc, float* weights, float* alpha, const int32_t* ray_list,
                                             const int32_t* ray_count, int act, float shift, void* stream) {
    DANBO_CHECK_DENSITY_ACT(act, shift);
    DANBO_CHECK_ARG(R > 0 && S > 0 && B > 0.f);
    DANBO_CHECK_ARG((ray_list == nullptr) == (ray_count == nullptr) && (valid_bits == nullptr || raw_empty != nullptr));
    const CompositeArgs a{raw, raw_empty, valid_bits, z, rays_d, R, S, B, noise, rgb_map, disp, acc, weights, alpha, ray_list, ray_count};
    return act == DENSITY_SOFTPLUS ? composite_launch<DENSITY_SOFTPLUS>(a, shift, stream) : composite_launch<DENSITY_RELU>(a, 0.f, stream);
}

struct ImportanceArgs {
    const float *z, *weights;
    int R, S, Sf;
    const float* u;
    float *z_fine, *z_sorted;
    int32_t* sorted_idx;
    const int32_t *ray_list, *ray_count;
};
template <bool TWO>
static int importance_launch(const ImportanceArgs& a, void* stream) {
    const int R = a.R, S = a.S, Sf = a.Sf;
    if (S <= 64 && Sf <= 64) {
        if (a.u)
            hipLaunchKernelGGL((k_importance_wave<false, TWO>), dim3(stream_grid((long)R * 64, 256)), dim3(256), 0,
                               (hipStream_t)stream, a.z, a.weights, R, S, Sf, a.u, a.z_fine, a.z_sorted, a.sorted_idx);
        else
            hipLaunchKernelGGL((k_importance_wave<true, TWO>), dim3(stream_grid((long)R * 64, 256)), dim3(256), 0,
                               (hipStream_t)stream, a.z, a.weights, R, S, Sf, a.u, a.z_fine, a.z_sorted, a.sorted_idx);
    } else if (S <= IMPB_MAX_S && Sf <= 64) {
        const dim3 grid(stream_grid((long)R * 64, 256));
        if (a.u)
            hipLaunchKernelGGL((k_importance_wave_long<false, TWO>), grid, dim3(256), 0, (hipStream_t)stream, a.z, a.weights, R, S, Sf, a.u,
                               a.z_fine, a.z_sorted, a.sorted_idx, ray_scatter(R), a.ray_list, a.ray_count);
        else
            hipLaunchKernelGGL((k_importance_wave_long<true, TWO>), grid, dim3(256), 0, (hipStream_t)stream, a.z, a.weights, R, S, Sf, a.u,
                               a.z_fine, a.z_sorted, a.sorted_idx, ray_scatter(R), a.ray_list, a.ray_count);
    } else {
        hipLaunchKernelGGL(k_importance<TWO>, dim3(stream_grid(R, 64)), dim3(64), 0, (hipStream_t)stream, a.z, a.weights, R, S, Sf,
                           a.u, a.z_fine, a.z_sorted, a.sorted_idx);
    }
    DANBO_LAUNCH_RET();
}
extern "C" int danbo_importance_samples(const float* z, const float* weights, int R, int S, int Sf, const float* u,
                                         float* z_fine, float* z_sorted, int32_t* sorted_idx, void* stream) {
    return danbo_importance_samples_rays(z, weights, R, S, Sf, u, z_fine, z_sorted, sorted_idx, nullptr, nullptr, stream);
}
extern "C" int danbo_importance_samples_rays(const float* z, const float* weights, int R, int S, int Sf, const float* u,
                                              float* z_fine, float* z_sorted, int32_t* sorted_idx, const int32_t* ray_list,
                                              const int32_t* ray_count, void* stream) {
    return danbo_importance_samples_pdf(z, weights, R, S, Sf, u, 0, z_fine, z_sorted, sorted_idx, ray_list, ray_count, stream);
}
extern "C" int danbo_importance_samples_pdf(const float* z, const float* weights, int R, int S, int Sf, const float* u, int pdf,
                                             float* z_fine, float* z_sorted, int32_t* sorted_idx, const int32_t* ray_list,
                                             const int32_t* ray_count, void* stream) {
    DANBO_CHECK_ARG(pdf == 0 || pdf == 1);
    DANBO_CHECK_ARG(R > 0 && S >= 3 && Sf > 0);
    DANBO_CHECK_ARG((ray_list == nullptr) == (ray_count == nullptr));
    DANBO_CHECK_ARG(ray_list == nullptr || (S > 64 && S <= IMPB_MAX_S && Sf <= 64));
    const ImportanceArgs a{z, weights, R, S, Sf, u, z_fine, z_sorted, sorted_idx, ray_list, ray_count};
    return pdf ? importance_launch<true>(a, stream) : importance_launch<false>(a, stream);
}

struct CompositeImportanceArgs {
    const float *raw, *raw_empty;
    const uint32_t* valid_bits;
    const float *z, *rays_d;
    int R, S, Sf;
    float B;
    const float *noise, *u;
    float *rgb_map, *disp, *acc, *weights, *alpha, *z_fine, *z_sorted;
    int32_t* sorted_idx;
    const int32_t *ray_list, *ray_count;
};
template <bool TWO, int DA>
static int composite_importance_launch(const CompositeImportanceArgs& a, float shift, void* stream) {
    static const int resident[2] = {resident_grid(k_composite_importance<false, TWO, DA>, 1L << 40, 256),
                                    resident_grid(k_composite_importance<true, TWO, DA>, 1L << 40, 256)};
    const dim3 grid((unsigned)std::min<long>(ceil_div((long)a.R * 64, 256), resident[a.u ? 0 : 1])), block(256);
    const float4* r4 = reinterpret_cast<const float4*>(a.raw);
    const float4* e4 = reinterpret_cast<const float4*>(a.raw_empty);
    if (a.u)
        hipLaunchKernelGGL((k_composite_importance<false, TWO, DA>), grid, block, 0, (hipStream_t)stream, r4, e4, a.valid_bits, a.z, a.rays_d,
                           a.R, a.S, a.Sf, a.B, a.noise, a.u, a.rgb_map, a.disp, a.acc, a.weights, a.alpha, a.z_fine, a.z_sorted, a.sorted_idx,
                           a.ray_list, a.ray_count, ray_scatter(a.R), shift);
    else
        hipLaunchKernelGGL((k_composite_importance<true, TWO, DA>), grid, block, 0, (hipStream_t)stream, r4, e4, a.valid_bits, a.z, a.rays_d,
                           a.R, a.S, a.Sf, a.B, a.noise, a.u, a.rgb_map, a.disp, a.acc, a.weights, a.alpha, a.z_fine, a.z_sorted, a.sorted_idx,
                           a.ray_list, a.ray_count, ray_scatter(a.R), shift);
    DANBO_LAUNCH_RET();
}
extern "C" int danbo_composite_importance_fwd(const float* raw, const float* raw_empty, const uint32_t* valid_bits,
                                               const float* z, const float* rays_d, int R, int S, int Sf, float B,
                                               const float* noise, const float* u, float* rgb_map, float* disp,
                                               float* acc, float* weights, float* alpha, float* z_fine, float* z_sorted,
                                               int32_t* sorted_idx, const int32_t* ray_list, const int32_t* ray_count,
                                               void* stream) {
    return danbo_composite_importance_pdf_fwd(raw, raw_empty, valid_bits, z, rays_d, R, S, Sf, B, noise, u, 0, rgb_map, disp, acc, weights,
                                              alpha, z_fine, z_sorted, sorted_idx, ray_list, ray_count, stream);
}
extern "C" int danbo_composite_importance_pdf_fwd(const float* raw, const float* raw_empty, const uint32_t* valid_bits,
                                                   const float* z, const float* rays_d, int R, int S, int Sf, float B,
                                                   const float* noise, const float* u, int pdf, float* rgb_map, float* disp,
                                                   float* acc, float* weights, float* alpha, float* z_fine, float* z_sorted,
                                                   int32_t* sorted_idx, const int32_t* ray_list, const int32_t* ray_count,
                                                   void* stream) {
    return danbo_composite_importance_pdf_fwd_act(raw, raw_empty, valid_bits, z, rays_d, R, S, Sf, B, noise, u, pdf, rgb_map, disp, acc,
                                                  weights, alpha, z_fine, z_sorted, sorted_idx, ray_list, ray_count, DENSITY_RELU, 0.f,
                                                  stream);
}
extern "C" int danbo_composite_importance_pdf_fwd_act(const float* raw, const float* raw_empty, const uint32_t* valid_bits,
                                                       const float* z, const float* rays_d, int R, int S, int Sf, float B,
                                                       const float* noise, const float* u, int pdf, float* rgb_map, float* disp,
                                                       float* acc, float* weights, float* alpha, float* z_fine, float* z_sorted,
                                                       int32_t* sorted_idx, const int32_t* ray_list, const int32_t* ray_count,
                                                       int act, float shift, void* stream) {
    DANBO_CHECK_ARG(pdf == 0 || pdf == 1);
    DANBO_CHECK_DENSITY_ACT(act, shift);
    DANBO_CHECK_ARG(R > 0 && S >= 3 && S <= 64 && Sf > 0 && Sf <= 64 && B > 0.f);
    DANBO_CHECK_ARG(raw && z && rays_d && rgb_map && disp && acc && z_fine && z_sorted && sorted_idx);
    DANBO_CHECK_ARG((valid_bits == nullptr) || (raw_empty != nullptr));
    DANBO_CHECK_ARG((ray_list == nullptr) == (ray_count == nullptr));
    const CompositeImportanceArgs a{raw, raw_empty, valid_bits, z, rays_d, R, S, Sf, B, noise, u, rgb_map, disp, acc, weights, alpha,
                                    z_fine, z_sorted, sorted_idx, ray_list, ray_count};
    if (act == DENSITY_SOFTPLUS)
        return pdf ? composite_importance_launch<true, DENSITY_SOFTPLUS>(a, shift, stream)
                   : composite_importance_launch<false, DENSITY_SOFTPLUS>(a, shift, stream);
    return pdf ? composite_importance_launch<true, DENSITY_RELU>(a, 0.f, stream) : composite_importance_launch<false, DENSITY_RELU>(a, 0.f, stream);
}

extern "C" int danbo_flat_rays(const float* t_lo, const uint32_t* ray_flat, int R, int S, int Sf, float* rgb0, float* disp0, float* acc0, float* weights0, float* alpha0, float* z_fine,
                                float* rgb_map, float* disp, float* acc, float* weights, float* alpha, int32_t* ray_list,
                                int32_t* ray_count, int parts, void* stream) {
    DANBO_CHECK_ARG(R > 0 && S >= 3 && Sf > 0);
    DANBO_CHECK_ARG(t_lo && ray_flat && rgb0 && disp0 && acc0 && z_fine && rgb_map && disp && acc && ray_list && ray_count);
    DANBO_CHECK_ARG(parts >= 1 && parts <= 3);
    hipLaunchKernelGGL(k_flat_rays, dim3(ceil_div(R, FLAT_BLOCK)), dim3(FLAT_BLOCK), 0, (hipStream_t)stream,
                       t_lo, ray_flat, R, S, Sf, rgb0, disp0, acc0, weights0, alpha0, z_fine,
                       rgb_map, disp, acc, weights, alpha, ray_list, ray_count, parts);
    DANBO_LAUNCH_RET();
}

extern "C" int danbo_composite_merged_fwd(const float* raw_a, const float* raw_b, const float* raw_empty,
                                           const uint32_t* bits_a, const uint32_t* bits_b, const int32_t* sorted_idx,
                                           const float* z_sorted, const float* rays_d, int R, int S, int Sf, float B,
                                           const float* noise, float* rgb_map, float* disp, float* acc, float* weights,
                                           float* alpha, float* raw_sorted, const int32_t* ray_list, const int32_t* ray_count,
                                           void* stream) {
    return danbo_composite_merged_fwd_act(raw_a, raw_b, raw_empty, bits_a, bits_b, sorted_idx, z_sorted, rays_d, R, S, Sf, B, noise, rgb_map,
                                          disp, acc, weights, alpha, raw_sorted, ray_list, ray_count, DENSITY_RELU, 0.f, stream);
}
extern "C" int danbo_composite_merged_fwd_act(const float* raw_a, const float* raw_b, const float* raw_empty,
                                               const uint32_t* bits_a, const uint32_t* bits_b, const int32_t* sorted_idx,
                                               const float* z_sorted, const float* rays_d, int R, int S, int Sf, float B,
                                               const float* noise, float* rgb_map, float* disp, float* acc, float* weights,
                                               float* alpha, float* raw_sorted, const int32_t* ray_list, const int32_t* ray_count,
                                               int act, float shift, void* stream) {
    DANBO_CHECK_DENSITY_ACT(act, shift);
    DANBO_CHECK_ARG(R > 0 && S > 0 && Sf > 0 && B > 0.f && raw_a && raw_b && sorted_idx && z_sorted && rays_d);
    DANBO_CHECK_ARG(rgb_map && disp && acc && ((bits_a == nullptr && bits_b == nullptr) || raw_empty != nullptr));
    DANBO_CHECK_ARG((ray_list == nullptr) == (ray_count == nullptr));
    const float4 *a4 = reinterpret_cast<const float4*>(raw_a), *b4 = reinterpret_cast<const float4*>(raw_b);
    const float4* e4 = reinterpret_cast<const float4*>(raw_empty);
    float4* rs4 = reinterpret_cast<float4*>(raw_sorted);
    if (act == DENSITY_SOFTPLUS) {
        static const int per_launch = resident_grid(k_composite_merged_softplus, 1L << 40, 256);
        hipLaunchKernelGGL(k_composite_merged_softplus, dim3((unsigned)std::min<long>(ceil_div((long)R * 64, 256), per_launch)), dim3(256), 0,
                           (hipStream_t)stream, a4, b4, e4, bits_a, bits_b, sorted_idx, z_sorted, rays_d, R, S, Sf, B, noise, rgb_map, disp, acc,
                           weights, alpha, rs4, ray_list, ray_count, ray_scatter(R), shift);
    } else {
        static const int per_launch = resident_grid(k_composite_merged, 1L << 40, 256);
        hipLaunchKernelGGL(k_composite_merged, dim3((unsigned)std::min<long>(ceil_div((long)R * 64, 256), per_launch)), dim3(256), 0,
                           (hipStream_t)stream, a4, b4, e4, bits_a, bits_b, sorted_idx, z_sorted, rays_d, R, S, Sf, B, noise, rgb_map, disp, acc,
                           weights, alpha, rs4, ray_list, ray_count, ray_scatter(R));
    }
    DANBO_LAUNCH_RET();
}
```

Before: 3.961 billion ray-samples/s.

## Fuse ray bone mask and flat-ray setup into one ray-front kernel

Adds a k_ray_front kernel that computes the per-ray bone mask, classifies flat rays, writes zeroed outputs for them and builds the ray list in a single launch, replacing the separate ray_bone_mask and flat_rays kernels. The counter zeroing is folded into the near/far cylinder kernel through a new clear-words argument, which removes a separate memset launch. It also replaces fixed-count unrolled binary searches with loops sized by the actual array length. The goal is fewer launches and less re-reading of per-ray data in the front end of the frame, in exchange for a larger fused kernel and a new dynamically bound entry point.

```diff
diff --git a/danbo-pytorch_amd/core/hip_ops.py b/danbo-pytorch_amd/core/hip_ops.py
--- a/danbo-pytorch_amd/core/hip_ops.py
+++ b/danbo-pytorch_amd/core/hip_ops.py
@@ -63,7 +63,7 @@
     return vol
 
 
-def near_far_cylinder(rays_o, rays_d, cyl, near0=0.0, far0=1.0, chunk=4096, near_in=None, far_in=None):
+def near_far_cylinder(rays_o, rays_d, cyl, near0=0.0, far0=1.0, chunk=4096, near_in=None, far_in=None, clear=None):
     rays_o, rays_d, cyl = _f32(rays_o, "rays_o"), _f32(rays_d, "rays_d"), _f32(cyl, "cyl")
     near_in, far_in = _f32(near_in, "near_in"), _f32(far_in, "far_in")
     R, G = rays_o.shape[0], cyl.shape[0]
@@ -71,8 +71,14 @@
     scratch = torch.empty(nchunk * 8, device=rays_o.device, dtype=torch.float32)
     near = torch.empty(R, device=rays_o.device, dtype=torch.float32)
     far = torch.empty_like(near)
-    _call("danbo_near_far_cylinder", _p(rays_o), _p(rays_d), _p(cyl), R, G, float(near0), float(far0),
-          _p(near_in), _p(far_in), int(chunk), _p(scratch), _p(near), _p(far), _stream())
+    if clear is None:
+        _call("danbo_near_far_cylinder", _p(rays_o), _p(rays_d), _p(cyl), R, G, float(near0), float(far0),
+              _p(near_in), _p(far_in), int(chunk), _p(scratch), _p(near), _p(far), _stream())
+    else:
+        assert clear.dtype == torch.int32 and clear.is_contiguous() and clear.numel() <= 1024
+        _hip.check(_ray_front_entry("danbo_near_far_cylinder_clear")(
+            _p(rays_o), _p(rays_d), _p(cyl), R, G, float(near0), float(far0), _p(near_in), _p(far_in), int(chunk), _p(scratch), _p(near),
+            _p(far), _p(clear), clear.numel(), _stream()), "danbo_near_far_cylinder_clear")
     return near, far
 
 
@@ -409,6 +415,46 @@
     if rows_later:
         res["rows"] = lambda: launch(2)
     return res
+
+
+_RAY_FRONT = None
+
+
+def _ray_front_entry(name="danbo_ray_front"):
+    global _RAY_FRONT
+    if _RAY_FRONT is None:
+        import os
+        h = _hip.bind_headers([_hip.HEADER_PATH, os.path.join(os.path.dirname(_hip.HEADER_PATH), "danbo_ray_front.h")])[1]
+        bound = {}
+        for fn_name, argtypes in h.signatures.items():
+            fn = getattr(_hip.lib(), fn_name)
+            fn.argtypes, fn.restype = argtypes, h.restypes[fn_name]
+            bound[fn_name] = fn
+        _RAY_FRONT = bound
+    return _RAY_FRONT[name]
+
+
+def ray_front(rays_o, rays_d, skts, align, axis_scale, t_lo, t_hi, S, Sf, want_weights=False, cnt=None, want_flat=False,
+              park_z_fine=True):
+    rays_o, rays_d, skts = _f32(rays_o, "rays_o"), _f32(rays_d, "rays_d"), _f32(skts, "skts")
+    t_lo, t_hi = _f32(t_lo, "t_lo").reshape(-1), _f32(t_hi, "t_hi").reshape(-1)
+    R, G, dev = rays_o.shape[0], skts.shape[0], rays_o.device
+    assert t_lo.shape[0] == R and t_hi.shape[0] == R
+    mask = torch.empty(R, device=dev, dtype=torch.int32)
+    flags = torch.empty(R, device=dev, dtype=torch.int32) if want_flat else None
+    out0 = _ray_outputs(R, S, Sf, dev, want_weights=want_weights)
+    out = _ray_outputs(R, S, Sf, dev, merged=True)
+    zf = torch.empty(R, Sf, device=dev, dtype=torch.float32)
+    lst = torch.empty(R, device=dev, dtype=torch.int32)
+    if cnt is None:
+        cnt = torch.zeros(1, device=dev, dtype=torch.int32)
+    assert cnt.dtype == torch.int32 and cnt.numel() == 1
+    _hip.check(_ray_front_entry()(
+        _p(rays_o), _p(rays_d), _p(t_lo), _p(t_hi), R, G, _p(skts), _p(_f32(align, "align")), _p(_f32(axis_scale, "axis_scale")),
+        int(S), int(Sf), _p(mask), _p(flags), _p(out0["rgb_map"]), _p(out0["disp_map"]), _p(out0["acc_map"]), _p(out0["weights"]),
+        _p(out0["alpha"]), _p(zf if park_z_fine else None), _p(out["rgb_map"]), _p(out["disp_map"]), _p(out["acc_map"]),
+        _p(out["weights"]), _p(out["alpha"]), _p(lst), _p(cnt), _stream()), "danbo_ray_front")
+    return (mask, t_lo, t_hi, flags), dict(out0=out0, out=out, z_fine=zf, ray_list=lst, ray_count=cnt)
 
 
 def composite_importance(raw, z, rays_d, Sf, B=1.0, noise=None, u=None, bits=None, raw_empty=None, want_weights=True,
diff --git a/danbo-pytorch_amd/core/render_engine.py b/danbo-pytorch_amd/core/render_engine.py
--- a/danbo-pytorch_amd/core/render_engine.py
+++ b/danbo-pytorch_amd/core/render_engine.py
@@ -53,7 +53,12 @@
             dense = True
         lazy = not dense and not keep
         pkw = dict(want_confd=True) if part else {}
-        near, far = self.near_far(rays_o, rays_d, cyls, skts, 0.0, 1.0, chunk) if near_far is None else near_far
+        if near_far is None:
+            counts = torch.empty(3, device=rays_o.device, dtype=torch.int32)
+            near, far = self.near_far(rays_o, rays_d, cyls, skts, 0.0, 1.0, chunk, clear=counts)
+        else:
+            counts = torch.zeros(3, device=rays_o.device, dtype=torch.int32)
+            near, far = near_far
         z = ops.coarse_samples(near, far, S)
         raw, bits, empty, ex = self._network_pass(rays_o, rays_d, skts, bones, cam_idx, z, (near, far), dense, lazy, "coarse", **pkw)
         if self.fuse_resample and S <= 64 and Sf <= 64:
@@ -98,6 +103,7 @@
         self.mlp_mode = mlp_mode
         self.group_rows = False
         self.cull_listed_rays = True
+        self.ray_front = True
 
     def refresh(self):
         key = self._key()
@@ -334,9 +340,9 @@
         out["T_i"] = out.pop("weights")
         return out
 
-    def near_far(self, rays_o, rays_d, cyls, skts, near0=0.0, far0=1.0, chunk=4096):
-        self.refresh()
-        near, far = ops.near_far_cylinder(rays_o, rays_d, cyls, near0, far0, chunk)
+    def near_far(self, rays_o, rays_d, cyls, skts, near0=0.0, far0=1.0, chunk=4096, clear=None):
+        self.refresh()
+        near, far = ops.near_far_cylinder(rays_o, rays_d, cyls, near0, far0, chunk, clear=clear)
         if self.cfg["use_volume_near_far"]:
             ops.near_far_boxes(rays_o, rays_d, skts, self.align, self.axis_scale, near, far)
         return near, far
@@ -352,16 +358,26 @@
         lazy = not dense and not keep
         flat_mode = (lazy and (fused or (S <= 256 and Sf <= 64)) and self.skip_flat_rays and self.flat_rays_ok
                      and act[0] == "relu")
-        near, far = self.near_far(rays_o, rays_d, cyls, skts, 0.0, 1.0, chunk) if near_far is None else near_far
+        if near_far is None:
+            counts = torch.empty(3, device=rays_o.device, dtype=torch.int32)
+            near, far = self.near_far(rays_o, rays_d, cyls, skts, 0.0, 1.0, chunk, clear=counts)
+        else:
+            counts = torch.zeros(3, device=rays_o.device, dtype=torch.int32)
+            near, far = near_far
         listed_cull = flat_mode and self.cull_listed_rays and not part and skts.shape[0] == 1
         z = torch.empty(rays_o.shape[0], S, device=rays_o.device, dtype=torch.float32) if listed_cull else ops.coarse_samples(near, far, S)
-        ray_mask = None if dense else ops.ray_bone_mask(rays_o, rays_d, skts, self.align, self.axis_scale, near, far,
-                                                        want_flat=flat_mode)
-        counts = torch.zeros(3, device=rays_o.device, dtype=torch.int32)
         flat = None
+        front = flat_mode and self.ray_front
+        if front:
+            ray_mask, flat = ops.ray_front(rays_o, rays_d, skts, self.align, self.axis_scale, near, far, S, Sf,
+                                           want_weights=not fused or bool(part), cnt=counts[2:3], park_z_fine=not listed_cull)
+        else:
+            ray_mask = None if dense else ops.ray_bone_mask(rays_o, rays_d, skts, self.align, self.axis_scale, near, far,
+                                                            want_flat=flat_mode)
         vols = self.volumes(bones)
         if flat_mode:
-            flat = ops.flat_rays(ray_mask[1], ray_mask[3], S, Sf, want_weights=not fused or bool(part), cnt=counts[2:3])
+            if not front:
+                flat = ops.flat_rays(ray_mask[1], ray_mask[3], S, Sf, want_weights=not fused or bool(part), cnt=counts[2:3])
             view = self.view_constants(rays_d, skts, cam_idx, flat["ray_list"], flat["ray_count"])
         else:
             view = self.view_constants(rays_d, skts, cam_idx)
diff --git a/danbo-pytorch_amd/csrc/flat_rows.hpp b/danbo-pytorch_amd/csrc/flat_rows.hpp
--- /dev/null
+++ b/danbo-pytorch_amd/csrc/flat_rows.hpp
@@ -0,0 +1,87 @@
+#pragma once
+#include <stdint.h>
+
+#ifndef DANBO_HD
+#if defined(__HIPCC__)
+#define DANBO_HD __host__ __device__ __forceinline__
+#else
+#define DANBO_HD inline
+#endif
+#endif
+
+namespace danbo {
+
+DANBO_HD int rows_piece_offset(const void* base, uint64_t first_word) { return (int)((((uintptr_t)base >> 2) + first_word) & 3u); }
+DANBO_HD int rows_pieces(int off, int n_rows, int W) { return (off + n_rows * W + 3) >> 2; }
+
+struct RowsCursor { int q, rem; };
+DANBO_HD RowsCursor rows_cursor(int piece, int off, int W) {
+    const int l = 4 * piece - off + 4 * W;
+    RowsCursor c;
+    c.q = l / W - 4;
+    c.rem = l % W;
+    return c;
+}
+DANBO_HD RowsCursor rows_advance(RowsCursor c, int dq, int drem, int W) {
+    c.q += dq;
+    c.rem += drem;
+    if (c.rem >= W) { c.rem -= W; ++c.q; }
+    return c;
+}
+DANBO_HD bool rows_flat(const int* flat, int q, int n_rows) { return q >= 0 && q < n_rows && flat[q] != 0; }
+DANBO_HD unsigned rows_piece_mask(RowsCursor c, int W, int n_rows, const int* flat) {
+    if (c.rem + 4 <= W) return rows_flat(flat, c.q, n_rows) ? 15u : 0u;
+    unsigned m = 0u;
+    for (int e = 0; e < 4; ++e) {
+        if (rows_flat(flat, c.q, n_rows)) m |= 1u << e;
+        if (++c.rem == W) { c.rem = 0; ++c.q; }
+    }
+    return m;
+}
+
+template <class Store16, class Store4>
+DANBO_HD void zero_flat_rows(int tid, int nthreads, int off, int W, int n_rows, const int* flat, int n_flat, Store16 store16,
+                             Store4 store4) {
+    if (n_flat == 0) return;
+    const int np = rows_pieces(off, n_rows, W);
+    if (n_flat == n_rows) {
+        const int total = n_rows * W;
+        for (int p = tid; p < np; p += nthreads) {
+            const int l = 4 * p - off;
+            if (l >= 0 && l + 4 <= total) {
+                store16(l);
+            } else {
+                for (int e = 0; e < 4; ++e)
+                    if (l + e >= 0 && l + e < total) store4(l + e);
+            }
+        }
+        return;
+    }
+    if (off == 0 && (W & 3) == 0) {
+        const int per_row = W >> 2;
+        const int dq = nthreads / per_row, dj = nthreads % per_row;
+        int q = tid / per_row, j = tid % per_row;
+        for (int p = tid; p < np; p += nthreads) {
+            if (flat[q] != 0) store16(4 * p);
+            q += dq;
+            j += dj;
+            if (j >= per_row) { j -= per_row; ++q; }
+        }
+        return;
+    }
+    const int dq = (4 * nthreads) / W, drem = (4 * nthreads) % W;
+    RowsCursor c = rows_cursor(tid, off, W);
+    for (int p = tid; p < np; p += nthreads) {
+        const unsigned m = rows_piece_mask(c, W, n_rows, flat);
+        const int l = 4 * p - off;
+        if (m == 15u) {
+            store16(l);
+        } else if (m != 0u) {
+            for (int e = 0; e < 4; ++e)
+                if ((m >> e) & 1u) store4(l + e);
+        }
+        c = rows_advance(c, dq, drem, W);
+    }
+}
+
+}
diff --git a/danbo-pytorch_amd/csrc/k_frame.hip b/danbo-pytorch_amd/csrc/k_frame.hip
--- a/danbo-pytorch_amd/csrc/k_frame.hip
+++ b/danbo-pytorch_amd/csrc/k_frame.hip
@@ -1,5 +1,6 @@
 #include "common.hpp"
 #include "../../include/danbo_cull.h"
+#include "../../include/danbo_ray_front.h"
 
 using namespace danbo;
 
@@ -58,31 +59,31 @@
     DANBO_CHECK_ARG(workspace_bytes >= danbo_render_frame_workspace(R, G, S, Sf, r->chunk, m->graph_width));
     Carver c(workspace);
     const FrameBuffers b = carve(c, R, G, S, Sf, r->chunk, m->graph_width);
-    hipStream_t st = (hipStream_t)stream;
 
-    DANBO_TRY(danbo_near_far_cylinder(r->rays_o, r->rays_d, r->cyls, R, G, 0.f, 1.f, r->near_in, r->far_in, r->chunk, b.cyl_scratch,
-                                      b.near, b.far, stream));
+    DANBO_TRY(danbo_near_far_cylinder_clear(r->rays_o, r->rays_d, r->cyls, R, G, 0.f, 1.f, r->near_in, r->far_in, r->chunk, b.cyl_scratch,
+                                            b.near, b.far, reinterpret_cast<uint32_t*>(b.count), 4, stream));
     if (m->use_volume_near_far)
         DANBO_TRY(danbo_near_far_boxes(r->rays_o, r->rays_d, r->skts, m->align, m->axis_scale, R, G, b.near, b.far, stream));
     const bool listed_cull = flat_rays && G == 1;
     if (!listed_cull) DANBO_TRY(danbo_coarse_samples(b.near, b.far, R, S, nullptr, b.z, stream));
-    DANBO_TRY(danbo_ray_bone_mask(r->rays_o, r->rays_d, b.near, b.far, R, G, r->skts, m->align, m->axis_scale, b.ray_mask,
-                                  flat_rays ? b.ray_flat : nullptr, stream));
+    const int32_t *ray_list = nullptr, *ray_count = nullptr;
+    if (flat_rays) {
+        DANBO_TRY(danbo_ray_front(r->rays_o, r->rays_d, b.near, b.far, R, G, r->skts, m->align, m->axis_scale, S, Sf, b.ray_mask, nullptr,
+                                  o->rgb0, o->disp0, o->acc0, b.weights0, o->alpha0, listed_cull ? nullptr : b.z_fine, o->rgb_map,
+                                  o->disp_map, o->acc_map, o->weights, o->alpha, b.ray_list, b.count + 3, stream));
+        ray_list = b.ray_list;
+        ray_count = b.count + 3;
+    } else {
+        DANBO_TRY(danbo_ray_bone_mask(r->rays_o, r->rays_d, b.near, b.far, R, G, r->skts, m->align, m->axis_scale, b.ray_mask, nullptr,
+                                      stream));
+    }
     DANBO_TRY(danbo_pose_volumes_fwd(r->bones, G, m->L_graph, m->graph_width, m->g_w0, m->g_adjw0, m->g_b0, m->g_w1, m->g_adjw1, m->g_b1,
                                      m->g_w2, m->g_b2, m->g_w3, m->g_b3, b.vol_scratch, b.volumes, stream));
-    zero_words(b.count, 4, nullptr, 0, st);
     auto view_consts = [&](const int32_t* ray_list, const int32_t* ray_count) -> int {
         return danbo_view_consts(r->rays_d, r->skts, R, G, m->ray_mode, m->normalise, m->L_view, m->framecodes, m->n_codes, m->code_size,
                                  m->mean_code, r->cam_idx, m->views_w_ray_t, m->views_b_eff, m->rgb_w, m->rgb_b, m->empty_consts, 2,
                                  m->code_table, ray_list, ray_count, b.cview, b.raw_empty, stream);
     };
-    const int32_t *ray_list = nullptr, *ray_count = nullptr;
-    if (flat_rays) {
-        DANBO_TRY(danbo_flat_rays(b.near, b.ray_flat, R, S, Sf, o->rgb0, o->disp0, o->acc0, b.weights0, o->alpha0, b.z_fine, o->rgb_map,
-                                  o->disp_map, o->acc_map, o->weights, o->alpha, b.ray_list, b.count + 3, 3, stream));
-        ray_list = b.ray_list;
-        ray_count = b.count + 3;
-    }
     DANBO_TRY(view_consts(ray_list, ray_count));
     auto cull = [&](float* zz, int s, uint32_t* bits, int32_t* count) -> int {
         if (listed_cull) {
diff --git a/danbo-pytorch_amd/csrc/k_ray_front.hip b/danbo-pytorch_amd/csrc/k_ray_front.hip
--- /dev/null
+++ b/danbo-pytorch_amd/csrc/k_ray_front.hip
@@ -0,0 +1,140 @@
+#include "common.hpp"
+#include "../../include/danbo_ray_front.h"
+#include "ray_mask.hpp"
+#include "flat_rows.hpp"
+
+namespace danbo {
+
+constexpr int FRONT_BLOCK = 256;
+static_assert(FRONT_BLOCK == 4 * 64, "k_ray_front sums the listed counts of four wavefronts");
+constexpr int FRONT_MAX_W = 1 << 20;
+
+__device__ __forceinline__ void front_zero_rows(float* __restrict__ arr, int W, int r_a, int n_rows, const int* s_flag, int n_flat) {
+    if (arr == nullptr) return;
+    float* base = arr + (size_t)r_a * W;
+    const int off = rows_piece_offset(arr, (uint64_t)r_a * (uint64_t)W);
+    zero_flat_rows((int)threadIdx.x, FRONT_BLOCK, off, W, n_rows, s_flag, n_flat,
+                   [&](int l) { *reinterpret_cast<u32x4*>(base + l) = u32x4{0u, 0u, 0u, 0u}; },
+                   [&](int l) { base[l] = 0.f; });
+}
+
+template <bool POSES_IN_LDS>
+__global__ __launch_bounds__(FRONT_BLOCK) void k_ray_front(const float* __restrict__ rays_o, const float* __restrict__ rays_d,
+                                                           const float* __restrict__ t_lo, const float* __restrict__ t_hi,
+                                                           const float* __restrict__ skts, const float* __restrict__ align,
+                                                           const float* __restrict__ axis_scale, int R, int G, int S, int Sf,
+                                                           uint32_t* __restrict__ ray_mask, uint32_t* __restrict__ ray_flat,
+                                                           float* __restrict__ rgb0, float* __restrict__ disp0, float* __restrict__ acc0,
+                                                           float* __restrict__ weights0, float* __restrict__ alpha0,
+                                                           float* __restrict__ z_fine, float* __restrict__ rgb_map,
+                                                           float* __restrict__ disp, float* __restrict__ acc_out,
+                                                           float* __restrict__ weights, float* __restrict__ alpha_out,
+                                                           int32_t* __restrict__ ray_list, int32_t* __restrict__ ray_count) {
+    extern __shared__ __attribute__((aligned(16))) float smem[];
+    __shared__ int s_flag[FRONT_BLOCK];
+    __shared__ int s_cnt[FRONT_BLOCK / 64];
+    __shared__ int s_base;
+    float* s_align = smem;
+    float* s_scale = smem + J * 16;
+    float* s_skt = smem + J * 16 + J * 4;
+    const int tid = threadIdx.x, lane = tid & 63, wave = tid >> 6;
+    const int rays_per_pose = R / G;
+    const int r_a = blockIdx.x * FRONT_BLOCK, r_b = min(r_a + FRONT_BLOCK - 1, R - 1);
+    const int n_rows = r_b - r_a + 1;
+    const int g0 = min(r_a / rays_per_pose, G - 1), g1 = min(r_b / rays_per_pose, G - 1);
+    const int r = min(r_a + tid, R - 1);
+    const bool in = r_a + tid < R;
+    const float o[3] = {rays_o[3 * r], rays_o[3 * r + 1], rays_o[3 * r + 2]};
+    const float d[3] = {rays_d[3 * r], rays_d[3 * r + 1], rays_d[3 * r + 2]};
+    const float zl = t_lo[r], zh = t_hi[r];
+    stage_ray_poses<POSES_IN_LDS>(skts, align, axis_scale, g0, g1, s_align, s_scale, s_skt);
+    __syncthreads();
+    const int g = min(r / rays_per_pose, G - 1);
+    uint32_t bits = 0u;
+    if (POSES_IN_LDS) {
+        const float* sk = s_skt + (size_t)(g - g0) * J * 16;
+#pragma unroll 2
+        for (int j = 0; j < J; ++j)
+            bits |= segment_misses_bone(sk + 16 * j, s_align + 16 * j, s_scale + 4 * j, o, d, zl, zh) ? 0u : 1u << j;
+    } else {
+        for (int j = 0; j < J; ++j) {
+            float sk[12];
+            const float* src = skts + ((size_t)g * J + j) * 16;
+#pragma unroll
+            for (int i = 0; i < 12; ++i) sk[i] = src[i];
+            bits |= segment_misses_bone(sk, s_align + 16 * j, s_scale + 4 * j, o, d, zl, zh) ? 0u : 1u << j;
+        }
+    }
+    const float* m0 = POSES_IN_LDS ? s_skt + (size_t)(g - g0) * J * 16 : skts + (size_t)g * J * 16;
+    const bool flat = in && ray_of_constants(bits, d, zl, zh, m0);
+    if (in) {
+        ray_mask[r] = bits;
+        if (ray_flat != nullptr) ray_flat[r] = flat ? 1u : 0u;
+    }
+    s_flag[tid] = flat ? 1 : 0;
+    if (flat) {
+        rgb0[3 * r] = 0.f; rgb0[3 * r + 1] = 0.f; rgb0[3 * r + 2] = 0.f;
+        disp0[r] = 0.f;
+        acc0[r] = 0.f;
+        rgb_map[3 * r] = 0.f; rgb_map[3 * r + 1] = 0.f; rgb_map[3 * r + 2] = 0.f;
+        disp[r] = 0.f;
+        acc_out[r] = 0.f;
+    }
+    const unsigned long long listed = __ballot(in && !flat);
+    if (lane == 0) s_cnt[wave] = (int)__popcll(listed);
+    __syncthreads();
+    if (tid == 0) {
+        int run = 0;
+        for (int w = 0; w < FRONT_BLOCK / 64; ++w) run += s_cnt[w];
+        s_base = run > 0 ? atomicAdd(ray_count, run) : 0;
+    }
+    const int St = S + Sf;
+    const int n_flat = n_rows - (s_cnt[0] + s_cnt[1] + s_cnt[2] + s_cnt[3]);
+    front_zero_rows(alpha0, S, r_a, n_rows, s_flag, n_flat);
+    front_zero_rows(weights0, S, r_a, n_rows, s_flag, n_flat);
+    front_zero_rows(weights, St, r_a, n_rows, s_flag, n_flat);
+    front_zero_rows(alpha_out, St, r_a, n_rows, s_flag, n_flat);
+    if (z_fine != nullptr) {
+        unsigned long long rows = __ballot(flat);
+        while (rows != 0ull) {
+            const int b = (int)__builtin_ctzll(rows);
+            rows &= rows - 1ull;
+            const size_t rr = (size_t)(r_a + wave * 64 + b);
+            const float lo_b = __builtin_bit_cast(float, __builtin_amdgcn_readlane(__builtin_bit_cast(int, zl), b));
+            for (int c = lane; c < Sf; c += 64) z_fine[rr * Sf + c] = lo_b;
+        }
+    }
+    __syncthreads();
+    if (in && !flat) {
+        int before = 0;
+        for (int w = 0; w < wave; ++w) before += s_cnt[w];
+        ray_list[s_base + before + (int)__popcll(listed & ((1ull << lane) - 1ull))] = r;
+    }
+}
+
+}
+
+using namespace danbo;
+
+extern "C" int danbo_ray_front(const float* rays_o, const float* rays_d, const float* t_lo, const float* t_hi, int R, int G,
+                               const float* skts, const float* align, const float* axis_scale, int S, int Sf, uint32_t* ray_mask,
+                               uint32_t* ray_flat, float* rgb0, float* disp0, float* acc0, float* weights0, float* alpha0, float* z_fine,
+                               float* rgb_map, float* disp, float* acc, float* weights, float* alpha, int32_t* ray_list,
+                               int32_t* ray_count, void* stream) {
+    DANBO_CHECK_ARG(rays_o && rays_d && t_lo && t_hi && skts && align && axis_scale && ray_mask && poses_ok(R, G));
+    DANBO_CHECK_ARG(S >= 3 && Sf > 0 && S <= FRONT_MAX_W - Sf);
+    DANBO_CHECK_ARG(rgb0 && disp0 && acc0 && rgb_map && disp && acc && ray_list && ray_count);
+    const long np = 256 / (R / G) + 2 < G ? 256 / (R / G) + 2 : G;
+    const bool in_lds = np <= 8;
+    const size_t lds = sizeof(float) * (J * 16 + J * 4 + (in_lds ? np * J * 16 : 0));
+    const dim3 grid(ceil_div(R, FRONT_BLOCK)), block(FRONT_BLOCK);
+    if (in_lds)
+        hipLaunchKernelGGL(k_ray_front<true>, grid, block, lds, (hipStream_t)stream, rays_o, rays_d, t_lo, t_hi, skts, align, axis_scale, R,
+                           G, S, Sf, ray_mask, ray_flat, rgb0, disp0, acc0, weights0, alpha0, z_fine, rgb_map, disp, acc, weights, alpha,
+                           ray_list, ray_count);
+    else
+        hipLaunchKernelGGL(k_ray_front<false>, grid, block, lds, (hipStream_t)stream, rays_o, rays_d, t_lo, t_hi, skts, align, axis_scale, R,
+                           G, S, Sf, ray_mask, ray_flat, rgb0, disp0, acc0, weights0, alpha0, z_fine, rgb_map, disp, acc, weights, alpha,
+                           ray_list, ray_count);
+    DANBO_LAUNCH_RET();
+}
diff --git a/danbo-pytorch_amd/csrc/k_sample.hip b/danbo-pytorch_amd/csrc/k_sample.hip
--- a/danbo-pytorch_amd/csrc/k_sample.hip
+++ b/danbo-pytorch_amd/csrc/k_sample.hip
@@ -1,5 +1,7 @@
 #include "common.hpp"
 #include "cull_math.hpp"
+#include "ray_mask.hpp"
+#include "../../include/danbo_ray_front.h"
 
 namespace danbo {
 
@@ -74,9 +76,12 @@
 __global__ __launch_bounds__(CYL_BLOCK) DANBO_NO_PK_F32 void k_cylinder_chunk(const float* __restrict__ rays_o, const float* __restrict__ rays_d,
                                                               const float* __restrict__ cyl, int R, int G, float near0, float far0,
                                                               const float* __restrict__ near_in, const float* __restrict__ far_in,
-                                                              int chunk, float* __restrict__ near_out, float* __restrict__ far_out) {
+                                                              int chunk, float* __restrict__ near_out, float* __restrict__ far_out,
+                                                              uint32_t* __restrict__ clear, int n_clear) {
     __shared__ double s_part[CYL_BLOCK / 64][3];
     __shared__ double s_sum[3];
+    if (clear != nullptr && blockIdx.x == 0)
+        for (int i = threadIdx.x; i < n_clear; i += CYL_BLOCK) clear[i] = 0u;
     const int rays_per_pose = R / G;
     const int r_begin = blockIdx.x * chunk, r_end = min(r_begin + chunk, R);
     constexpr int PER = CYL_FUSED_MAX / CYL_BLOCK;
@@ -208,30 +213,6 @@
 }
 
 
-__device__ __forceinline__ bool segment_misses_bone(const float* sk, const float* al, const float* sc ,
-                                                    const float* o, const float* d, float zl, float zh) {
-    float ol[3], dl[3], t[3];
-    bone_local(sk, al, o, ol);
-    for (int k = 0; k < 3; ++k) t[k] = sk[4 * k] * d[0] + sk[4 * k + 1] * d[1] + sk[4 * k + 2] * d[2];
-    for (int k = 0; k < 3; ++k) dl[k] = al[4 * k] * t[0] + al[4 * k + 1] * t[1] + al[4 * k + 2] * t[2];
-    const float pad = 1e-4f * fmaxf(fabsf(zl), fabsf(zh)) + 1e-5f;
-    float tmin = zl - pad, tmax = zh + pad;
-    bool miss = false;
-    for (int k = 0; k < 3; ++k) {
-        const float s = sc[k] * 1.001f + 1e-4f;
-        if (fabsf(dl[k]) < 1e-12f) {
-            miss = miss || fabsf(ol[k]) > s;
-        } else {
-            const float inv = 1.0f / dl[k];
-            const float t1 = (-s - ol[k]) * inv, t2 = (s - ol[k]) * inv;
-            tmin = fmaxf(tmin, fminf(t1, t2));
-            tmax = fminf(tmax, fmaxf(t1, t2));
-        }
-    }
-    return miss || tmin > tmax;
-}
-
-constexpr float RAY_FLAT_VMAX = DANBO_RAY_FLAT_VMAX;
 
 template <bool POSES_IN_LDS>
 __global__ __launch_bounds__(256) void k_ray_bone_mask(const float* __restrict__ rays_o, const float* __restrict__ rays_d,
@@ -250,9 +231,7 @@
     const float o[3] = {rays_o[3 * r], rays_o[3 * r + 1], rays_o[3 * r + 2]};
     const float d[3] = {rays_d[3 * r], rays_d[3 * r + 1], rays_d[3 * r + 2]};
     const float zl = t_lo[r], zh = t_hi[r];
-    stage_bone_tables<256>(align, axis_scale, s_align, s_scale, 0.f);
-    if (POSES_IN_LDS)
-        for (int i = threadIdx.x; i < (g1 - g0 + 1) * J * 16; i += 256) s_skt[i] = skts[(size_t)g0 * J * 16 + i];
+    stage_ray_poses<POSES_IN_LDS>(skts, align, axis_scale, g0, g1, s_align, s_scale, s_skt);
     __syncthreads();
     const int g = min(r / rays_per_pose, G - 1);
     uint32_t bits = 0u;
@@ -273,16 +252,8 @@
     if (r_a + (int)threadIdx.x < R) {
         ray_mask[r] = bits;
         if (ray_flat != nullptr) {
-            const float dn = norm3_torch(d[0], d[1], d[2]);
-            const float span = mul_rn(add_rn(sub_rn(zh, zl), mul_rn(1e-3f, fmaxf(fabsf(zl), fabsf(zh)))), dn);
-            const float tail = mul_rn(1e10f, dn);
             const float* m0 = POSES_IN_LDS ? s_skt + (size_t)(g - g0) * J * 16 : skts + (size_t)g * J * 16;
-            float msum = 0.f;
-            for (int a = 0; a < 3; ++a)
-                for (int k = 0; k < 3; ++k) msum = add_rn(msum, fabsf(m0[4 * a + k]));
-            const float vin = mul_rn(dn, fmaxf(1.0f, msum));
-            const bool fin = zl <= zh && sub_rn(span, span) == 0.f && sub_rn(tail, tail) == 0.f && vin <= RAY_FLAT_VMAX;
-            ray_flat[r] = (bits == 0u && fin) ? 1u : 0u;
+            ray_flat[r] = ray_of_constants(bits, d, zl, zh, m0) ? 1u : 0u;
         }
     }
 }
@@ -704,6 +675,8 @@
     }
 }
 
+__device__ __forceinline__ int search_steps(int n) { return 32 - __builtin_clz((unsigned)(n > 0 ? n : 1)); }
+
 template <bool DET, bool TWO = false>
 __device__ __forceinline__ void importance_wave(float zi, float wi, int r, int S, int Sf, const float* __restrict__ u,
                                                 int lane, float* __restrict__ z_fine, float* __restrict__ z_sorted,
@@ -722,8 +695,7 @@
     const bool fact = lane < Sf;
     const float uk = DET ? linspace01(fact ? lane : 0, Sf) : (fact ? u[(size_t)r * Sf + lane] : 0.f);
     int lo = 0, hi = ncdf;
-#pragma unroll
-    for (int it = 0; it < 7; ++it) {
+    for (int it = search_steps(ncdf); it > 0; --it) {
         const int mid = (lo + hi) >> 1;
         const float cm = __shfl(cdf, mid < ncdf ? mid : ncdf - 1, 64);
         if (lo < hi) {
@@ -742,12 +714,14 @@
     const bool ascending = __all(!(lane < S - 1) || z1 >= zi);
     if (DET && ascending) {
         int l0 = 0, h0 = Sf, l1 = 0, h1 = S;
-#pragma unroll
-        for (int it = 0; it < 7; ++it) {
-            const int m0 = (l0 + h0) >> 1, m1 = (l1 + h1) >> 1;
+        for (int it = search_steps(Sf); it > 0; --it) {
+            const int m0 = (l0 + h0) >> 1;
             const float f = __shfl(zf, m0 < 63 ? m0 : 63, 64);
+            if (l0 < h0) { if (f < zi) l0 = m0 + 1; else h0 = m0; }
+        }
+        for (int it = search_steps(S); it > 0; --it) {
+            const int m1 = (l1 + h1) >> 1;
             const float c = __shfl(zi, m1 < 63 ? m1 : 63, 64);
-            if (l0 < h0) { if (f < zi) l0 = m0 + 1; else h0 = m0; }
             if (l1 < h1) { if (c <= zf) l1 = m1 + 1; else h1 = m1; }
         }
         rank_c += l0;
@@ -850,8 +824,7 @@
         const bool fact = lane < Sf;
         const float uk = DET ? linspace01(fact ? lane : 0, Sf) : (fact ? u[(size_t)r * Sf + lane] : 0.f);
         int lo = 0, hi = ncdf;
-#pragma unroll
-        for (int it = 0; it < 9; ++it) {
+        for (int it = search_steps(ncdf); it > 0; --it) {
             const int mid = (lo + hi) >> 1;
             const float cm = s_w[mid < ncdf ? mid : ncdf - 1];
             if (lo < hi) {
@@ -870,8 +843,7 @@
         const size_t oo = (size_t)r * (S + Sf);
         if (DET && ascending) {
             int l1 = 0, h1 = S;
-#pragma unroll
-            for (int it = 0; it < 9; ++it) {
+            for (int it = search_steps(S); it > 0; --it) {
                 const int m1 = (l1 + h1) >> 1;
                 const float cz = s_z[m1 < S ? m1 : S - 1];
                 if (l1 < h1) { if (cz <= zf) l1 = m1 + 1; else h1 = m1; }
@@ -881,8 +853,7 @@
                 const int s0 = 64 * c + lane;
                 const float zi = s_z[s0 < S ? s0 : S - 1];
                 int l0 = 0, h0 = Sf;
-#pragma unroll
-                for (int it = 0; it < 7; ++it) {
+                for (int it = search_steps(Sf); it > 0; --it) {
                     const int m0 = (l0 + h0) >> 1;
                     const float fz = s_f[m0 < 63 ? m0 : 63];
                     if (l0 < h0) { if (fz < zi) l0 = m0 + 1; else h0 = m0; }
@@ -1050,15 +1021,24 @@
 extern "C" int danbo_near_far_cylinder(const float* rays_o, const float* rays_d, const float* cyl, int R, int G,
                                         float near0, float far0, const float* near_in, const float* far_in, int chunk,
                                         float* scratch, float* near_out, float* far_out, void* stream) {
+    return danbo_near_far_cylinder_clear(rays_o, rays_d, cyl, R, G, near0, far0, near_in, far_in, chunk, scratch, near_out, far_out, nullptr,
+                                         0, stream);
+}
+
+extern "C" int danbo_near_far_cylinder_clear(const float* rays_o, const float* rays_d, const float* cyl, int R, int G,
+                                              float near0, float far0, const float* near_in, const float* far_in, int chunk,
+                                              float* scratch, float* near_out, float* far_out, uint32_t* clear_words, int n_clear,
+                                              void* stream) {
     DANBO_CHECK_ARG(chunk > 0 && scratch != nullptr && poses_ok(R, G));
+    DANBO_CHECK_ARG(n_clear >= 0 && n_clear <= 1024 && (clear_words != nullptr || n_clear == 0));
     hipStream_t st = (hipStream_t)stream;
     const int nchunk = ceil_div(R, chunk);
     if (chunk <= CYL_FUSED_MAX) {
         hipLaunchKernelGGL(k_cylinder_chunk, dim3(nchunk), dim3(CYL_BLOCK), 0, st, rays_o, rays_d, cyl, R, G, near0, far0, near_in,
-                           far_in, chunk, near_out, far_out);
+                           far_in, chunk, near_out, far_out, clear_words, n_clear);
         DANBO_LAUNCH_RET();
     }
-    zero_words(scratch, 8L * nchunk, nullptr, 0, st);
+    zero_words(scratch, 8L * nchunk, clear_words, n_clear, st);
     const int grid = stream_grid(R, 256);
     hipLaunchKernelGGL(k_cylinder_pass1, dim3(grid), dim3(256), 0, st, rays_o, rays_d, cyl, R, G, near0, far0, near_in,
                        far_in, chunk, reinterpret_cast<double*>(scratch), near_out, far_out);
diff --git a/danbo-pytorch_amd/csrc/ray_mask.hpp b/danbo-pytorch_amd/csrc/ray_mask.hpp
--- /dev/null
+++ b/danbo-pytorch_amd/csrc/ray_mask.hpp
@@ -0,0 +1,52 @@
+#pragma once
+#include "common.hpp"
+
+namespace danbo {
+
+__device__ __forceinline__ bool segment_misses_bone(const float* sk, const float* al, const float* sc ,
+                                                    const float* o, const float* d, float zl, float zh) {
+    float ol[3], dl[3], t[3];
+    bone_local(sk, al, o, ol);
+    for (int k = 0; k < 3; ++k) t[k] = sk[4 * k] * d[0] + sk[4 * k + 1] * d[1] + sk[4 * k + 2] * d[2];
+    for (int k = 0; k < 3; ++k) dl[k] = al[4 * k] * t[0] + al[4 * k + 1] * t[1] + al[4 * k + 2] * t[2];
+    const float pad = 1e-4f * fmaxf(fabsf(zl), fabsf(zh)) + 1e-5f;
+    float tmin = zl - pad, tmax = zh + pad;
+    bool miss = false;
+    for (int k = 0; k < 3; ++k) {
+        const float s = sc[k] * 1.001f + 1e-4f;
+        if (fabsf(dl[k]) < 1e-12f) {
+            miss = miss || fabsf(ol[k]) > s;
+        } else {
+            const float inv = 1.0f / dl[k];
+            const float t1 = (-s - ol[k]) * inv, t2 = (s - ol[k]) * inv;
+            tmin = fmaxf(tmin, fminf(t1, t2));
+            tmax = fminf(tmax, fmaxf(t1, t2));
+        }
+    }
+    return miss || tmin > tmax;
+}
+
+constexpr float RAY_FLAT_VMAX = DANBO_RAY_FLAT_VMAX;
+
+template <bool POSES_IN_LDS>
+__device__ __forceinline__ void stage_ray_poses(const float* __restrict__ skts, const float* __restrict__ align,
+                                                const float* __restrict__ axis_scale, int g0, int g1, float* s_align, float* s_scale,
+                                                float* s_skt) {
+    stage_bone_tables<256>(align, axis_scale, s_align, s_scale, 0.f);
+    if (POSES_IN_LDS)
+        for (int i = threadIdx.x; i < (g1 - g0 + 1) * J * 16; i += 256) s_skt[i] = skts[(size_t)g0 * J * 16 + i];
+}
+
+__device__ __forceinline__ bool ray_of_constants(uint32_t bits, const float* d, float zl, float zh, const float* m0) {
+    const float dn = norm3_torch(d[0], d[1], d[2]);
+    const float span = mul_rn(add_rn(sub_rn(zh, zl), mul_rn(1e-3f, fmaxf(fabsf(zl), fabsf(zh)))), dn);
+    const float tail = mul_rn(1e10f, dn);
+    float msum = 0.f;
+    for (int a = 0; a < 3; ++a)
+        for (int k = 0; k < 3; ++k) msum = add_rn(msum, fabsf(m0[4 * a + k]));
+    const float vin = mul_rn(dn, fmaxf(1.0f, msum));
+    const bool fin = zl <= zh && sub_rn(span, span) == 0.f && sub_rn(tail, tail) == 0.f && vin <= RAY_FLAT_VMAX;
+    return bits == 0u && fin;
+}
+
+}
diff --git a/include/danbo_ray_front.h b/include/danbo_ray_front.h
--- /dev/null
+++ b/include/danbo_ray_front.h
@@ -0,0 +1,26 @@
+#ifndef DANBO_RAY_FRONT_H
+#define DANBO_RAY_FRONT_H
+
+#include <stddef.h>
+#include <stdint.h>
+
+#ifdef __cplusplus
+extern "C" {
+#endif
+
+int danbo_ray_front(const float* rays_o, const float* rays_d, const float* t_lo , const float* t_hi , int R, int G,
+                    const float* skts , const float* align , const float* axis_scale , int S,
+                    int Sf, uint32_t* ray_mask , uint32_t* ray_flat , float* rgb0, float* disp0, float* acc0,
+                    float* weights0 , float* alpha0 , float* z_fine , float* rgb_map, float* disp,
+                    float* acc, float* weights , float* alpha , int32_t* ray_list ,
+                    int32_t* ray_count , void* stream);
+
+int danbo_near_far_cylinder_clear(const float* rays_o, const float* rays_d, const float* cyl, int R, int G, float near0, float far0,
+                                  const float* near_in, const float* far_in, int chunk, float* scratch, float* near_out,
+                                  float* far_out, uint32_t* clear_words , int n_clear, void* stream);
+
+#ifdef __cplusplus
+}
+#endif
+
+#endif
```

After: 3.994 billion ray-samples/s, median of 6. Within noise of the previous version (+0.8%).
